# Malfoy/BGREAT

Measured on AMD Instinct MI355X. Metric: Mreads/s aligned (k=31, 150bp, m=2), higher is better.
Workload: dtype u64; 1 GPU; BASELINE configs[2]: synthetic 5170.0M x 150 bp reads per GPU (1034 steps x 5000000), k=31, m=2, effort=2, greedy, graph of 98935 unitigs (genome 4600000 bp, 2 alleles every ~140 bp); reads resident in HBM as ASCII before the timed region, results left in HBM; read_len=150, k=31, m=2, effort=2, distinct_batches=20, parallelism=reads sharded over 1 GPU(s); graph blob broadcast once

## Files before the change

bgreat_amd/__init__.py:

```python
import ctypes as C
import importlib.util
import os
import subprocess
import sys

import numpy as np

_HERE = os.path.dirname(os.path.abspath(__file__))
LIB_PATH = os.environ.get("BGR_LIB_PATH") or os.path.join(_HERE, "lib", "libbgreat_gpu.so")
CLI_PATH = os.path.join(_HERE, "bin", "bgreat")

MODE_GREEDY, MODE_EXHAUSTIVE, MODE_ANCHORS = 0, 1, 2
ST_NOANCHOR, ST_FAILED, ST_ALIGNED, ST_MASK, ST_RC = 0, 1, 2, 3, 4
BUILD_ANCHORS = 1
BUILD_NO_EVICTIONS = 2

SYMBOLS = [
    "bgr_last_error", "bgr_device_count", "bgr_graph_build", "bgr_graph_build_from_fasta", "bgr_graph_blob",
    "bgr_graph_from_blob", "bgr_graph_info", "bgr_graph_destroy", "bgr_graph_upload", "bgr_graph_device_blob",
    "bgr_graph_adopt_device_blob", "bgr_aligner_create", "bgr_aligner_destroy", "bgr_align_batch", "bgr_align_device", "bgr_aligner_path_stats",
    "bgr_aligner_sync", "bgr_aligner_device_results", "bgr_aligner_arena_ints", "bgr_aligner_fetch", "bgr_aligner_counters",
    "bgr_aligner_reset_counters", "bgr_aligner_kernel_time", "bgr_aligner_reset_kernel_time", "bgr_aligner_launch_info",
    "bgr_aligner_configure", "bgr_readset_load", "bgr_readset_count", "bgr_readset_view", "bgr_readset_destroy",
    "bgr_write_records", "bgr_graph_unitigs", "bgr_readset_load_parallel", "bgr_align_all", "bgr_host_alloc", "bgr_host_free",
    "bgr_set_build_threads", "bgr_graph_build_ex", "bgr_graph_build_from_fasta_ex", "bgr_graph_anchor_lookup", "bgr_graph_key_lookup", "bgr_graph_key_lookup_wide",
    "bgr_aligner_set_knob", "bgr_aligner_pass_counts", "bgr_aligner_last_pass_runs", "bgr_set_option", "bgr_get_option", "bgr_option_name", "bgr_plan_launch", "bgr_aligner_kernel_times", "bgr_devices_init", "bgr_devices_method", "bgr_packed_plane_words", "bgr_pack_reads", "bgr_align_batch_packed",
    "bgr_align_fasta_text", "bgr_aligner_fetch_text", "bgr_host_cache_release", "bgr_device_local_cpus", "bgr_text_stage_create", "bgr_text_stage_destroy", "bgr_text_stage_upload",
    "bgr_align_batch_begin", "bgr_align_batch_test", "bgr_align_batch_wait", "bgr_text_stage_device", "bgr_text_stage_upload_parts",
    "bgr_device_alloc", "bgr_device_free", "bgr_device_upload", "bgr_device_download",
    "bgr_aligner_abundance_enable", "bgr_aligner_abundance", "bgr_aligner_reset_abundance", "bgr_aligner_abundance_plan", "bgr_plan_abundance", "bgr_graph_abundance", "bgr_write_abundance",
    "bgr_aligner_links_enable", "bgr_aligner_links", "bgr_aligner_reset_links", "bgr_aligner_links_info", "bgr_aligner_links_plan", "bgr_plan_links", "bgr_graph_links_bound",
    "bgr_graph_links_enable", "bgr_graph_links", "bgr_write_gfa", "bgr_link_canonical", "bgr_graph_links_enabled",
    "bgr_links_bubbles", "bgr_aligner_bubbles", "bgr_aligner_bubbles_times", "bgr_graph_bubbles_enable", "bgr_graph_bubbles_enabled", "bgr_graph_bubbles", "bgr_write_bubbles",
    "bgr_aligner_triples_enable", "bgr_aligner_triples", "bgr_aligner_reset_triples", "bgr_aligner_triples_info", "bgr_triple_canonical", "bgr_graph_triples_bound",
    "bgr_graph_triples_enable", "bgr_graph_triples_enabled", "bgr_graph_triples", "bgr_write_triples",
    "bgr_bubbles_phase", "bgr_graph_phase_enable", "bgr_graph_phase_enabled", "bgr_graph_phase", "bgr_write_phase",
    "bgr_phase_blocks", "bgr_phase_blocks_times", "bgr_graph_blocks_enable", "bgr_graph_blocks_enabled", "bgr_graph_blocks", "bgr_write_blocks",
    "bgr_blocks_haplotypes", "bgr_blocks_haplotypes_times", "bgr_graph_haplotypes_enable", "bgr_graph_haplotypes_enabled", "bgr_graph_haplotypes", "bgr_write_haplotypes",
    "bgr_aligner_pileup_enable", "bgr_aligner_pileup", "bgr_aligner_reset_pileup", "bgr_graph_pileup_enable", "bgr_graph_pileup_enabled", "bgr_graph_pileup",
    "bgr_write_pileup", "bgr_write_depth",
    "bgr_aligner_pileup_sites", "bgr_aligner_pileup_sites_times", "bgr_aligner_pileup_add", "bgr_graph_variants_enable", "bgr_graph_variants_enabled", "bgr_graph_variants",
    "bgr_graph_variants_params", "bgr_write_vcf", "bgr_parse_af_ppm",
    "bgr_aligner_pileup_strands_enable", "bgr_aligner_pileup_forward", "bgr_aligner_pileup_strand_sites", "bgr_graph_pileup_strands_enable", "bgr_graph_pileup_strands_enabled",
    "bgr_graph_pileup_forward", "bgr_graph_variants_strands_enable", "bgr_graph_variant_strand_sites", "bgr_write_pileup_strands", "bgr_write_vcf_strands", "bgr_parse_min_alt_strand",
]
KNOB_EXH_FRAME_CAP, KNOB_EXH_SEARCH, KNOB_BATCH_SPLIT_LIMIT, KNOB_DEBUG_STOP, KNOB_GREEDY_FAST, KNOB_EXH_FAST, KNOB_ANCHORS_FAST, KNOB_BATCH_OVERLAP, KNOB_EXH_MEMO_CAP, KNOB_GREEDY_PREPASS, KNOB_KERNEL_EVENTS = 1, 2, 3, 4, 5, 6, 7, 8, 9, 10, 11
KNOB_ABUNDANCE_FORM = 12
ABUNDANCE_AUTO, ABUNDANCE_GLOBAL, ABUNDANCE_LDS = 0, 1, 2
KNOB_LINKS_FORM = 13
LINKS_AUTO, LINKS_GLOBAL, LINKS_LDS = 0, 1, 2
KNOB_DEVICE_OVERLAP = 14
SEARCH_AUTO, SEARCH_DEPTH_FIRST, SEARCH_BY_LEVEL = 0, 1, 2


class _Borrowed(np.ndarray):
    _owner = None


class PlanInput(C.Structure):
    _fields_ = [("k", C.c_uint32), ("slot_fill_x100", C.c_uint32), ("table_bytes", C.c_uint32), ("has_exceptions", C.c_uint32), ("anchors", C.c_uint32), ("anchor_levels", C.c_uint32),
                ("graph_bases", C.c_uint64), ("n_unitigs", C.c_uint64), ("max_unitig_len", C.c_uint64),
                ("num_cus", C.c_uint32), ("resident_waves", C.c_uint32 * 7), ("lds_per_cu", C.c_uint64),
                ("cfg_waves", C.c_uint32), ("cfg_blocks_per_cu", C.c_uint32), ("cfg_lds_mphf", C.c_uint32),
                ("mode", C.c_uint32), ("max_mismatch", C.c_uint32), ("partial", C.c_uint32), ("max_read_len", C.c_uint32),
                ("n_reads", C.c_uint64), ("total_bases", C.c_uint64), ("wide_keys", C.c_uint32), ("reserved0", C.c_uint32)]


class PlanPass(C.Structure):
    _fields_ = [("used", C.c_uint32), ("blocks", C.c_uint32), ("waves_per_block", C.c_uint32), ("lds_bytes", C.c_uint32), ("table_staged", C.c_uint32)]


class PlanOutput(C.Structure):
    _fields_ = [("pass_", PlanPass * 6), ("level_search", C.c_uint32), ("deep_only", C.c_uint32), ("x4_levels", C.c_uint32), ("memo_cap", C.c_uint32),
                ("deep_scratch_bytes", C.c_uint64), ("arena_ints", C.c_uint64)]


class BgrError(RuntimeError):
    pass


class Params(C.Structure):
    _fields_ = [("mode", C.c_uint32), ("max_mismatch", C.c_uint32), ("effort", C.c_uint32), ("partial", C.c_uint32)]


class RunOptions(C.Structure):
    _fields_ = [("struct_size", C.c_uint64), ("n_gpus", C.c_uint32), ("threads", C.c_uint32), ("batch_reads", C.c_uint64), ("chunk_bytes", C.c_uint64),
                ("fastq", C.c_uint32), ("write_exhaustive", C.c_uint32), ("echo_files", C.c_uint32), ("correction", C.c_uint32),
                ("no_overlap_file", C.c_char_p), ("first_device", C.c_uint32), ("route", C.c_uint32), ("numa", C.c_uint32), ("split_output", C.c_uint32), ("gaf", C.c_uint32),
                ("abundance", C.c_uint32)]


class UnitigAbundance(C.Structure):
    _fields_ = [("reads", C.c_uint64), ("bases", C.c_uint64), ("kmers", C.c_uint64)]


class Link(C.Structure):
    _fields_ = [("from_", C.c_int32), ("to", C.c_int32), ("count", C.c_uint64)]


LINK_DTYPE = np.dtype([("from", np.int32), ("to", np.int32), ("count", np.uint64)])


class Bubble(C.Structure):
    _fields_ = [("source", C.c_int32), ("sink", C.c_int32), ("branch", C.c_int32 * 2), ("count", C.c_uint64 * 4)]


BUBBLE_DTYPE = np.dtype([("source", np.int32), ("sink", np.int32), ("branch", np.int32, (2,)), ("count", np.uint64, (4,))])
BUBBLES_TILE = 1024


class Triple(C.Structure):
    _fields_ = [("from_", C.c_int32), ("via", C.c_int32), ("to", C.c_int32), ("reserved", C.c_int32), ("count", C.c_uint64)]


TRIPLE_DTYPE = np.dtype([("from", np.int32), ("via", np.int32), ("to", np.int32), ("reserved", np.int32), ("count", np.uint64)])


class Phase(C.Structure):
    _fields_ = [("via", C.c_int32), ("source", C.c_int32), ("in_", C.c_int32 * 2), ("out", C.c_int32 * 2), ("sink", C.c_int32), ("reserved", C.c_int32), ("count", C.c_uint64 * 4)]


PHASE_DTYPE = np.dtype([("via", np.int32), ("source", np.int32), ("in", np.int32, (2,)), ("out", np.int32, (2,)), ("sink", np.int32), ("reserved", np.int32),
                        ("count", np.uint64, (4,))])


class BlockEntry(C.Structure):
    _fields_ = [("block", C.c_uint32), ("index", C.c_uint32), ("size", C.c_uint32), ("bubble", C.c_uint32), ("flags", C.c_uint32), ("reserved", C.c_uint32)]


BLOCK_DTYPE = np.dtype([("block", np.uint32), ("index", np.uint32), ("size", np.uint32), ("bubble", np.uint32), ("flags", np.uint32), ("reserved", np.uint32)])
BLOCK_REVERSED, BLOCK_HAP, BLOCK_CIRCULAR, BLOCK_CONFLICT = 1, 2, 4, 8
BLOCKS_TILE = 1024


class Haplotype(C.Structure):
    _fields_ = [("block", C.c_uint32), ("hap", C.c_uint32), ("size", C.c_uint32), ("flags", C.c_uint32), ("offset", C.c_uint64), ("length", C.c_uint64)]


HAPLOTYPE_DTYPE = np.dtype([("block", np.uint32), ("hap", np.uint32), ("size", np.uint32), ("flags", np.uint32), ("offset", np.uint64), ("length", np.uint64)])


class PathStat(C.Structure):
    _fields_ = [("path_len", C.c_uint64), ("path_start", C.c_uint64), ("aligned", C.c_uint32), ("mismatches", C.c_uint32)]


PATH_STAT_NO_WALK = 0x80000000


class Ticket(C.Structure):
    _fields_ = [("aligner", C.c_void_p), ("n_reads", C.c_uint64), ("serial", C.c_uint64)]


class TextBatch(C.Structure):
    _fields_ = [("struct_size", C.c_uint64), ("text", C.c_void_p), ("text_bytes", C.c_uint64), ("want_output", C.c_uint32), ("irregular", C.c_uint32), ("paths_out", C.c_void_p),
                ("paths_cap", C.c_uint64), ("notaligned_out", C.c_void_p), ("notaligned_cap", C.c_uint64), ("n_records", C.c_uint64),
                ("n_accepted", C.c_uint64), ("paths_bytes", C.c_uint64), ("notaligned_bytes", C.c_uint64), ("stage", C.c_void_p),
                ("fastq", C.c_uint32), ("reserved", C.c_uint32), ("record_info_out", C.c_void_p), ("record_info_cap", C.c_uint64)]


class PackedReads(C.Structure):
    _fields_ = [("read_offsets", C.c_void_p), ("fw3", C.c_void_p), ("hasn", C.c_void_p), ("nm_index", C.c_void_p), ("nm_value", C.c_void_p),
                ("nm_count", C.c_uint64), ("max_read_len", C.c_uint32)]


class GraphInfo(C.Structure):
    _fields_ = [("k", C.c_uint32), ("n_levels", C.c_uint32), ("n_unitigs", C.c_uint64), ("n_keys", C.c_uint64),
                ("n_left_keys", C.c_uint64), ("n_right_keys", C.c_uint64), ("n_fallback", C.c_uint64),
                ("total_bases", C.c_uint64), ("blob_bytes", C.c_uint64), ("mphf_bytes", C.c_uint64),
                ("max_unitig_len", C.c_uint64), ("has_exceptions", C.c_uint32), ("has_anchors", C.c_uint32),
                ("gamma", C.c_double)]


_lib = None


def build(force=False):
    if force:
        subprocess.check_call(["make", "-C", _HERE, "clean"])
    subprocess.check_call(["make", "-s", "-C", _HERE, "all"])


def _pin_hip_runtime():
    if "torch" in sys.modules or os.environ.get("BGREAT_SYSTEM_HIP"):
        return
    try:
        spec = importlib.util.find_spec("torch")
    except (ImportError, ValueError):
        spec = None
    if spec and spec.submodule_search_locations:
        p = os.path.join(list(spec.submodule_search_locations)[0], "lib", "libamdhip64.so")
        if os.path.exists(p):
            C.CDLL(p, mode=C.RTLD_GLOBAL)


def lib():
    global _lib
    if _lib is not None:
        return _lib
    _pin_hip_runtime()
    if not os.path.exists(LIB_PATH):
        raise BgrError("libbgreat_gpu.so is not built (%s); run `make -C bgreat_amd` -- there is no fallback path" % LIB_PATH)
    L = C.CDLL(LIB_PATH)
    vp, u64, u32, i32 = C.c_void_p, C.c_uint64, C.c_uint32, C.c_int
    L.bgr_last_error.restype = C.c_char_p
    L.bgr_set_build_threads.restype = None
    L.bgr_set_build_threads.argtypes = [C.c_uint32]
    L.bgr_device_count.restype = i32
    L.bgr_graph_build.argtypes = [u32, u64, vp, vp, C.c_double, C.POINTER(vp)]
    L.bgr_graph_build_from_fasta.argtypes = [C.c_char_p, u32, C.c_double, C.POINTER(vp)]
    L.bgr_graph_build_ex.argtypes = [u32, u64, vp, vp, C.c_double, u32, C.POINTER(vp)]
    L.bgr_graph_build_from_fasta_ex.argtypes = [C.c_char_p, u32, C.c_double, u32, C.POINTER(vp)]
    L.bgr_graph_anchor_lookup.argtypes = [vp, u64, C.POINTER(u64), C.POINTER(u64)]
    L.bgr_graph_key_lookup.argtypes = [vp, u64, C.POINTER(C.c_uint32)]
    L.bgr_graph_key_lookup_wide.argtypes = [vp, u64, u64, C.POINTER(C.c_uint32)]
    L.bgr_graph_blob.restype = vp
    L.bgr_graph_blob.argtypes = [vp, C.POINTER(u64)]
    L.bgr_graph_from_blob.argtypes = [vp, u64, C.POINTER(vp)]
    L.bgr_graph_info.argtypes = [vp, C.POINTER(GraphInfo)]
    L.bgr_graph_unitigs.argtypes = [vp, C.POINTER(vp), C.POINTER(vp), C.POINTER(u64)]
    L.bgr_graph_destroy.argtypes = [vp]
    L.bgr_graph_destroy.restype = None
    L.bgr_graph_upload.argtypes = [vp, i32]
    L.bgr_graph_device_blob.restype = vp
    L.bgr_graph_device_blob.argtypes = [vp, i32]
    L.bgr_graph_adopt_device_blob.argtypes = [i32, vp, u64, C.POINTER(vp)]
    L.bgr_devices_init.argtypes = [vp, i32, u32, u32]
    L.bgr_devices_method.argtypes = [vp]
    L.bgr_devices_method.restype = u32
    L.bgr_aligner_create.argtypes = [vp, i32, C.POINTER(vp)]
    L.bgr_aligner_destroy.argtypes = [vp]
    L.bgr_aligner_destroy.restype = None
    L.bgr_align_batch.argtypes = [vp, C.POINTER(Params), vp, vp, u64, vp, u64, vp, vp]
    L.bgr_align_device.argtypes = [vp, C.POINTER(Params), vp, vp, u64, u64, u32]
    L.bgr_packed_plane_words.argtypes = [u64, u64]
    L.bgr_packed_plane_words.restype = u64
    L.bgr_pack_reads.argtypes = [vp, vp, u64, vp, vp, vp, vp, u64, C.POINTER(u64), C.POINTER(u32)]
    L.bgr_align_batch_packed.argtypes = [vp, C.POINTER(Params), C.POINTER(PackedReads), u64, vp, u64, vp, vp]
    L.bgr_align_fasta_text.argtypes = [vp, C.POINTER(Params), C.POINTER(TextBatch)]
    L.bgr_align_batch_begin.argtypes = [vp, C.POINTER(Params), vp, vp, u64, C.POINTER(Ticket)]
    L.bgr_align_batch_test.argtypes = [C.POINTER(Ticket)]
    L.bgr_align_batch_wait.argtypes = [C.POINTER(Ticket), vp, u64, vp, vp]
    L.bgr_aligner_fetch_text.argtypes = [vp, C.POINTER(TextBatch)]
    L.bgr_text_stage_create.argtypes = [C.c_int, C.POINTER(vp)]
    L.bgr_text_stage_destroy.argtypes = [vp]
    L.bgr_text_stage_destroy.restype = None
    L.bgr_text_stage_upload.argtypes = [vp, vp, u64]
    L.bgr_aligner_sync.argtypes = [vp]
    L.bgr_aligner_device_results.argtypes = [vp, C.POINTER(vp), C.POINTER(vp), C.POINTER(vp)]
    L.bgr_aligner_arena_ints.argtypes = [vp, vp]
    L.bgr_aligner_fetch.argtypes = [vp, u64, vp, u64, vp, vp]
    L.bgr_aligner_path_stats.argtypes = [vp, vp, vp, u64, vp]
    L.bgr_aligner_counters.argtypes = [vp, vp]
    L.bgr_aligner_reset_counters.argtypes = [vp]
# ... 220 lines not shown
    if isinstance(a, (bytes, bytearray)):
        a = np.frombuffer(a, dtype=np.uint8)
    return np.ascontiguousarray(a, dtype=np.uint8)


def pack_reads(reads, offsets):
    reads = _as_u8(reads)
    offsets = np.ascontiguousarray(offsets, dtype=np.uint64)
    n = len(offsets) - 1
    rel = offsets - offsets[0]
    total = int(rel[n])
    words = lib().bgr_packed_plane_words(n, total)
    fw3 = np.zeros(words, dtype=np.uint64)
    hasn = np.zeros((n + 31) // 32 + 1, dtype=np.uint32)
    cap = max(64, total // 16 + 64)
    nm_index = np.zeros(cap, dtype=np.uint32)
    nm_value = np.zeros(cap, dtype=np.uint64)
    cnt, mx = C.c_uint64(), C.c_uint32()
    _check(lib().bgr_pack_reads(reads.ctypes.data, offsets.ctypes.data, n, fw3.ctypes.data, hasn.ctypes.data, nm_index.ctypes.data,
                                nm_value.ctypes.data, cap, C.byref(cnt), C.byref(mx)))
    return {"read_offsets": rel, "fw3": fw3, "hasn": hasn, "nm_index": nm_index[: cnt.value].copy(), "nm_value": nm_value[: cnt.value].copy(),
            "max_read_len": mx.value, "n": n}


class Graph:

    def __init__(self, handle):
        self.h = handle

    @classmethod
    def build(cls, k, seqs, offsets, gamma=0.0, anchors=False, no_evictions=False):
        seqs = _as_u8(seqs)
        offsets = np.ascontiguousarray(offsets, dtype=np.uint64)
        h = C.c_void_p()
        _check(lib().bgr_graph_build_ex(k, len(offsets) - 1, seqs.ctypes.data, offsets.ctypes.data, gamma,
                                        (BUILD_ANCHORS if anchors else 0) | (BUILD_NO_EVICTIONS if no_evictions else 0), C.byref(h)))
        return cls(h)

    @classmethod
    def from_fasta(cls, path, k, gamma=0.0, anchors=False):
        h = C.c_void_p()
        _check(lib().bgr_graph_build_from_fasta_ex(path.encode(), k, gamma, BUILD_ANCHORS if anchors else 0, C.byref(h)))
        return cls(h)

    def key_lookup(self, key):
        key = int(key)
        if key < 0:
            raise ValueError("key_lookup: a (k-1)-mer is a non-negative integer")
        if key >> 128:
            return None
        slot = C.c_uint32()
        _check(lib().bgr_graph_key_lookup_wide(self.h, key >> 64, key & 0xFFFFFFFFFFFFFFFF, C.byref(slot)))
        return None if slot.value == 0xFFFFFFFF else int(slot.value)

    def anchor_lookup(self, kmer):
        idx, pos = C.c_uint64(), C.c_uint64()
        _check(lib().bgr_graph_anchor_lookup(self.h, int(kmer), C.byref(idx), C.byref(pos)))
        if idx.value == 0xFFFFFFFFFFFFFFFF:
            return None, 0, 0
        return idx.value, pos.value >> 32, pos.value & 0xFFFFFFFF

    @classmethod
    def from_blob(cls, blob):
        blob = _as_u8(blob)
        h = C.c_void_p()
        _check(lib().bgr_graph_from_blob(blob.ctypes.data, blob.size, C.byref(h)))
        return cls(h)

    @classmethod
    def adopt_device_blob(cls, device, dev_ptr, nbytes):
        h = C.c_void_p()
        _check(lib().bgr_graph_adopt_device_blob(device, dev_ptr, nbytes, C.byref(h)))
        return cls(h)

    def blob(self):
        n = C.c_uint64()
        p = lib().bgr_graph_blob(self.h, C.byref(n))
        if not p:
            return np.zeros(0, dtype=np.uint8)
        v = np.ctypeslib.as_array(C.cast(p, C.POINTER(C.c_uint8)), shape=(n.value,)).view(_Borrowed)
        v._owner = self
        return v

    def info(self):
        gi = GraphInfo()
        _check(lib().bgr_graph_info(self.h, C.byref(gi)))
        return {f[0]: getattr(gi, f[0]) for f in GraphInfo._fields_ if f[0] != "reserved"}

    def upload(self, device=0):
        _check(lib().bgr_graph_upload(self.h, device))

    def devices_init(self, first_device=0, n_devices=1, how=0):
        _check(lib().bgr_devices_init(self.h, first_device, n_devices, how))
        return lib().bgr_devices_method(self.h)

    def device_blob(self, device=0):
        return lib().bgr_graph_device_blob(self.h, device)

    def abundance(self):
        n = self.info()["n_unitigs"]
        out = np.zeros((n, 3), dtype=np.uint64)
        _check(lib().bgr_graph_abundance(self.h, out.ctypes.data, n))
        return out

    def links_enable(self, on=True):
        _check(lib().bgr_graph_links_enable(self.h, int(bool(on))))

    def links_enabled(self):
        return bool(lib().bgr_graph_links_enabled(self.h))

    def bubbles_enable(self, on=True, min_link=1):
        _check(lib().bgr_graph_bubbles_enable(self.h, int(bool(on)), int(min_link)))

    def bubbles_enabled(self):
        return bool(lib().bgr_graph_bubbles_enabled(self.h))

    def bubbles(self):
        return _fetch_bubbles(lambda out, cap, n: lib().bgr_graph_bubbles(self.h, out, cap, n))

    def links(self):
        return _fetch_links(lib().bgr_graph_links, self.h)

    def pileup_enable(self, on=True):
        _check(lib().bgr_graph_pileup_enable(self.h, int(bool(on))))

    def pileup_enabled(self):
        return bool(lib().bgr_graph_pileup_enabled(self.h))

    def pileup(self):
        return _fetch_pileup(lib().bgr_graph_pileup, self)

    def write_pileup(self, path):
        _check(lib().bgr_write_pileup(path.encode(), self.h))

    def write_depth(self, path):
        _check(lib().bgr_write_depth(path.encode(), self.h))

    def variants_enable(self, min_depth=2, min_alt=2, min_af_ppm=200000, on=True):
        prm = VariantParams(int(min_depth), int(min_alt), int(min_af_ppm))
        _check(lib().bgr_graph_variants_enable(self.h, C.byref(prm) if on else None))

    def variants_enabled(self):
        return bool(lib().bgr_graph_variants_enabled(self.h))

    def variants(self):
        return _fetch_sites(lambda out, cap, n: lib().bgr_graph_variants(self.h, out, cap, n))

    def variants_params(self):
        prm = VariantParams()
        _check(lib().bgr_graph_variants_params(self.h, C.byref(prm)))
        return int(prm.min_depth), int(prm.min_alt), int(prm.min_af_ppm)

    def write_vcf(self, path, sites=None, params=None):
        if sites is None:
            sites = self.variants()
        prm = VariantParams(*(self.variants_params() if params is None else params))
        sites = np.ascontiguousarray(sites, dtype=VARIANT_DTYPE)
        _check(lib().bgr_write_vcf(path.encode(), self.h, C.byref(prm), sites.ctypes.data if len(sites) else None, len(sites)))

    def pileup_strands_enable(self, on=True):
        _check(lib().bgr_graph_pileup_strands_enable(self.h, int(bool(on))))

    def pileup_strands_enabled(self):
        return bool(lib().bgr_graph_pileup_strands_enabled(self.h))

    def pileup_forward(self):
        return _fetch_forward(lib().bgr_graph_pileup_forward, self)

    def write_pileup_strands(self, path):
        _check(lib().bgr_write_pileup_strands(path.encode(), self.h))
# ... 628 lines not shown
```

bgreat_amd/csrc/capi.hip:

```cpp
#include <hip/hip_runtime.h>
#include <sys/mman.h>
#include <dlfcn.h>

#include <algorithm>
#include <chrono>
#include <condition_variable>
#include <cstdio>
#include <cstdlib>
#include <cstring>
#include <map>
#include <mutex>
#include <string>
#include <thread>
#include <vector>

#include "../../include/bgreat_gpu.h"
#include "abundance_kernels.h"
#include "align_kernels.h"
#include "fanout.h"
#include "fastx.h"
#include "anchor_index.h"
#include "graph_build.h"
#include "launch_plan.h"
#include "launch_taker.h"
#include "links_kernels.h"
#include "triples_kernels.h"
#include "pileup_kernels.h"
#include "read_pack.h"
#include "text_kernels.h"
#include "options.h"
#include "capi_internal.h"

namespace bgr {
static thread_local std::string tl_err;
int set_error(int code, const std::string& msg) { tl_err = msg; return code; }
}

namespace {

int drain_timers(bgr_aligner* a) {
    if (a->ev_used == 0) return BGR_OK;
    HIP_TRY(hipStreamSynchronize(a->stream));
    for (int i = 0; i < a->ev_used; ++i) {
        float ms = 0;
        HIP_TRY(hipEventElapsedTime(&ms, a->ev[i][0], a->ev[i][a->ev_marks[i]]));
        a->t_ms += ms;
        for (int j = 0; j < a->ev_marks[i]; ++j) {
            HIP_TRY(hipEventElapsedTime(&ms, a->ev[i][j], a->ev[i][j + 1]));
            a->t_slot_ms[j] += ms;
        }
        ++a->t_launches;
    }
    a->ev_used = 0;
    return BGR_OK;
}

void forget_launch(bgr_aligner* a) { a->last_n = 0; a->holder = nullptr; }

}

extern "C" {

const char* bgr_last_error(void) { return bgr::tl_err.c_str(); }

int bgr_set_option(const char* name, int64_t value) {
    bgr::Option* o = name ? bgr::find_option(name) : nullptr;
    if (!o) return fail(BGR_E_ARG, std::string("bgr_set_option: unknown option '") + (name ? name : "") + "'");
    if (value < o->lo || value > o->hi) return fail(BGR_E_ARG, std::string("bgr_set_option: value out of range for '") + name + "'");
    o->value.store(value, std::memory_order_relaxed);
    return BGR_OK;
}
int bgr_get_option(const char* name, int64_t* value) {
    bgr::Option* o = name ? bgr::find_option(name) : nullptr;
    if (!o || !value) return fail(BGR_E_ARG, std::string("bgr_get_option: unknown option '") + (name ? name : "") + "'");
    *value = o->value.load(std::memory_order_relaxed);
    return BGR_OK;
}
const char* bgr_option_name(uint32_t index, const char** what) {
    size_t n;
    bgr::Option* t = bgr::option_table(&n);
    if (index >= n) return nullptr;
    if (what) *what = t[index].what;
    return t[index].name;
}
void bgr_set_build_threads(uint32_t threads) { bgr::set_build_threads(threads); }

int bgr_device_count(void) {
    int n = 0;
    if (hipGetDeviceCount(&n) != hipSuccess) return 0;
    return n;
}

int bgr_graph_build(uint32_t k, uint64_t n_unitigs, const char* seqs, const uint64_t* offsets, double gamma, bgr_graph** out) {
    return bgr_graph_build_ex(k, n_unitigs, seqs, offsets, gamma, 0, out);
}

int bgr_graph_build_ex(uint32_t k, uint64_t n_unitigs, const char* seqs, const uint64_t* offsets, double gamma, uint32_t flags, bgr_graph** out) {
    if (!out || (n_unitigs && (!seqs || !offsets))) return fail(BGR_E_ARG, "bgr_graph_build: null argument");
    if (flags & ~(uint32_t)(BGR_BUILD_ANCHORS | BGR_BUILD_NO_EVICTIONS)) return fail(BGR_E_ARG, "bgr_graph_build: unknown flag");
    bgr_graph* g = new bgr_graph();
    std::string err;
    uint64_t zero[1] = {0};
    if (!bgr::build_graph(k, n_unitigs, seqs, n_unitigs ? offsets : zero, gamma > 0 ? gamma : 0.0, flags, g->host, err)) {
        delete g;
        return fail(BGR_E_ARG, err);
    }
    g->header = *g->host.header();
    const uint64_t nu = g->header.n_unitigs;
    g->ascii.assign(seqs + (nu ? offsets[0] : 0), seqs + (nu ? offsets[nu] : 0));
    g->ascii_offs.resize(nu + 1);
    for (uint64_t i = 0; i <= nu; ++i) g->ascii_offs[i] = nu ? offsets[i] - offsets[0] : 0;
    *out = g;
    return BGR_OK;
}

int bgr_graph_unitigs(const bgr_graph* g, const char** seqs, const uint64_t** offsets, uint64_t* n) {
    if (!g || !seqs || !offsets || !n) return fail(BGR_E_ARG, "bgr_graph_unitigs: null argument");
    if (g->ascii_offs.empty()) return fail(BGR_E_ARG, "bgr_graph_unitigs: this graph was created from a blob and carries no unitig characters");
    *seqs = g->ascii.data();
    *offsets = g->ascii_offs.data();
    *n = g->ascii_offs.size() - 1;
    return BGR_OK;
}

int bgr_graph_build_from_fasta(const char* path, uint32_t k, double gamma, bgr_graph** out) {
    return bgr_graph_build_from_fasta_ex(path, k, gamma, 0, out);
}

int bgr_graph_build_from_fasta_ex(const char* path, uint32_t k, double gamma, uint32_t flags, bgr_graph** out) {
    if (!path || !out) return fail(BGR_E_ARG, "bgr_graph_build_from_fasta: null argument");
    std::vector<char> seqs;
    std::vector<uint64_t> offs;
    std::string err;
    if (!bgr::read_unitig_fasta(path, k, seqs, offs, err)) return fail(BGR_E_IO, err);
    return bgr_graph_build_ex(k, offs.size() - 1, seqs.data(), offs.data(), gamma, flags, out);
}

int bgr_graph_anchor_lookup(const bgr_graph* g, uint64_t kmer, uint64_t* index_out, uint64_t* position_out) {
    if (!g || !index_out) return fail(BGR_E_ARG, "bgr_graph_anchor_lookup: null argument");
    if (g->host.blob.empty()) return fail(BGR_E_ARG, "bgr_graph_anchor_lookup: graph has no host blob");
    if (!g->header.anc_n) return fail(BGR_E_ARG, "bgr_graph_anchor_lookup: the graph was built without BGR_BUILD_ANCHORS");
    const uint64_t idx = bgr::anchor_lookup(g->host.header(), g->host.base(), kmer);
    *index_out = idx;
    if (position_out) *position_out = idx == ~0ULL ? 0 : reinterpret_cast<const uint64_t*>(g->host.base() + g->header.off_anc_pos)[idx];
    return BGR_OK;
}

int bgr_graph_key_lookup(const bgr_graph* g, uint64_t key, uint32_t* slot_out) {
    if (!g || !slot_out) return fail(BGR_E_ARG, "bgr_graph_key_lookup: null argument");
    if (g->host.blob.empty()) return fail(BGR_E_ARG, "bgr_graph_key_lookup: graph has no host blob");
    if (g->header.wide_keys) return fail(BGR_E_ARG, "bgr_graph_key_lookup: the graph has two-word keys (k > 32): use bgr_graph_key_lookup_wide");
    *slot_out = bgr::host_lookup(g->host.header(), g->host.base(), key);
    return BGR_OK;
}

int bgr_graph_key_lookup_wide(const bgr_graph* g, uint64_t key_hi, uint64_t key_lo, uint32_t* slot_out) {
    if (!g || !slot_out) return fail(BGR_E_ARG, "bgr_graph_key_lookup_wide: null argument");
    if (g->host.blob.empty()) return fail(BGR_E_ARG, "bgr_graph_key_lookup_wide: graph has no host blob");
    *slot_out = bgr::host_lookup_wide(g->host.header(), g->host.base(), key_hi, key_lo);
    return BGR_OK;
}

const void* bgr_graph_blob(const bgr_graph* g, uint64_t* bytes) {
    if (!g || g->host.blob.empty()) { if (bytes) *bytes = 0; return nullptr; }
    if (bytes) *bytes = g->header.blob_bytes;
    return g->host.blob.data();
}

int bgr_graph_from_blob(const void* blob, uint64_t bytes, bgr_graph** out) {
    if (!blob || !out) return fail(BGR_E_ARG, "bgr_graph_from_blob: null argument");
    std::string err;
    if (!bgr::validate_blob(blob, bytes, err)) return fail(BGR_E_ARG, err);
    bgr_graph* g = new bgr_graph();
    if (!g->host.blob.reset((bytes + 7) / 8)) { delete g; return fail(BGR_E_ARG, "bgr_graph_from_blob: out of memory"); }
    memcpy(g->host.blob.data(), blob, bytes);
    g->header = *g->host.header();
    *out = g;
    return BGR_OK;
}

int bgr_graph_info(const bgr_graph* g, bgr_graph_info_t* o) {
    if (!g || !o) return fail(BGR_E_ARG, "bgr_graph_info: null argument");
    const BgrBlobHeader& h = g->header;
    memset(o, 0, sizeof(*o));
    o->k = h.k; o->n_levels = 2; o->n_unitigs = h.n_unitigs; o->n_keys = h.n_placed + h.n_fallback;
    o->n_left_keys = h.n_left_keys; o->n_right_keys = h.n_right_keys; o->n_fallback = h.n_fallback;
    o->total_bases = h.total_bases; o->blob_bytes = h.blob_bytes; o->mphf_bytes = h.n_buckets * 4;
    o->max_unitig_len = h.max_unitig_len; o->has_exceptions = h.has_exc; o->has_anchors = h.anc_n ? 1 : 0; o->gamma = h.gamma;
    return BGR_OK;
}

void bgr_graph_destroy(bgr_graph* g) {
    if (!g) return;
    for (auto& kv : g->dev) {
        if (kv.second.owned && kv.second.ptr) {
            if (hipSetDevice(kv.first) == hipSuccess) (void)hipFree(kv.second.ptr);
        }
    }
    variants_run_free(g);
    delete g;
}

int bgr_graph_upload(bgr_graph* g, int device) {
    if (!g) return fail(BGR_E_ARG, "bgr_graph_upload: null graph");
    if (g->dev.count(device)) return BGR_OK;
    if (g->host.blob.empty()) return fail(BGR_E_ARG, "bgr_graph_upload: graph has no host blob (adopted graphs live on one device)");
    HIP_TRY(hipSetDevice(device));
    void* p = nullptr;
    HIP_TRY(hipMalloc(&p, g->header.blob_bytes));
    hipError_t e = hipMemcpy(p, g->host.blob.data(), g->header.blob_bytes, hipMemcpyHostToDevice);
    if (e == hipSuccess) e = hipStreamSynchronize(nullptr);
    if (e != hipSuccess) { (void)hipFree(p); return fail(BGR_E_HIP, std::string("blob H2D: ") + hipGetErrorString(e)); }
    g->dev[device] = {p, true};
    return BGR_OK;
}

namespace {

struct Rccl {
    typedef int (*CommInitAll_t)(void** comms, int n, const int* devs);
    typedef int (*Group_t)(void);
    typedef int (*Broadcast_t)(const void* send, void* recv, size_t count, int dtype, int root, void* comm, hipStream_t stream);
    typedef int (*CommDestroy_t)(void* comm);
    void* lib = nullptr;
    CommInitAll_t CommInitAll = nullptr;
    Group_t GroupStart = nullptr, GroupEnd = nullptr;
    Broadcast_t Broadcast = nullptr;
    CommDestroy_t CommDestroy = nullptr;
    bool load() {
        for (const char* name : {"librccl.so.1", "librccl.so"}) {
            lib = dlopen(name, RTLD_NOW | RTLD_LOCAL);
            if (lib) break;
        }
        if (!lib) return false;
        CommInitAll = reinterpret_cast<CommInitAll_t>(dlsym(lib, "ncclCommInitAll"));
        GroupStart = reinterpret_cast<Group_t>(dlsym(lib, "ncclGroupStart"));
        GroupEnd = reinterpret_cast<Group_t>(dlsym(lib, "ncclGroupEnd"));
        Broadcast = reinterpret_cast<Broadcast_t>(dlsym(lib, "ncclBroadcast"));
        CommDestroy = reinterpret_cast<CommDestroy_t>(dlsym(lib, "ncclCommDestroy"));
        return CommInitAll && GroupStart && GroupEnd && Broadcast && CommDestroy;
    }
};

bool fanout_rccl(const std::vector<int>& devs, const std::vector<void*>& ptr, uint64_t bytes, std::string& why) {
    Rccl r;
    if (!r.load()) { why = "librccl not loadable"; return false; }
    const int n = (int)devs.size();
    std::vector<void*> comms(n, nullptr);
    if (r.CommInitAll(comms.data(), n, devs.data()) != 0) { why = "ncclCommInitAll failed"; return false; }
    std::vector<hipStream_t> streams(n, nullptr);
    bool ok = true;
    for (int i = 0; i < n && ok; ++i) ok = hipSetDevice(devs[i]) == hipSuccess && hipStreamCreateWithFlags(&streams[i], hipStreamNonBlocking) == hipSuccess;
    if (ok) {
        ok = r.GroupStart() == 0;
        for (int i = 0; i < n && ok; ++i) {
            ok = hipSetDevice(devs[i]) == hipSuccess &&
                 r.Broadcast(ptr[i], ptr[i], (size_t)bytes,  0,  0, comms[i], streams[i]) == 0;
        }
        ok = r.GroupEnd() == 0 && ok;
    }
    for (int i = 0; i < n; ++i) {
        if (streams[i]) { if (hipSetDevice(devs[i]) == hipSuccess) { ok = hipStreamSynchronize(streams[i]) == hipSuccess && ok; (void)hipStreamDestroy(streams[i]); } }
    }
    for (void* c : comms) if (c) (void)r.CommDestroy(c);
    if (!ok) why = "RCCL broadcast failed";
    return ok;
}

bool peer_round(const std::vector<bgr::FanoutCopy>& round, uint64_t bytes, std::string& why) {
    std::vector<hipStream_t> streams;
    std::vector<int> sdev;
    bool ok = true;
    for (const bgr::FanoutCopy& c : round) {
        if (hipSetDevice(c.src_dev) != hipSuccess) { ok = false; why = "hipSetDevice failed"; break; }
        int can = 0;
        if (hipDeviceCanAccessPeer(&can, c.src_dev, c.dst_dev) == hipSuccess && can) {
            hipError_t pe = hipDeviceEnablePeerAccess(c.dst_dev, 0);
            if (pe != hipSuccess && pe != hipErrorPeerAccessAlreadyEnabled) (void)hipGetLastError();
        }
        hipStream_t st = nullptr;
        if (hipStreamCreateWithFlags(&st, hipStreamNonBlocking) != hipSuccess) { ok = false; why = "hipStreamCreate failed"; break; }
        streams.push_back(st);
        sdev.push_back(c.src_dev);
        hipError_t e = hipMemcpyPeerAsync(c.dst, c.dst_dev, c.src, c.src_dev, bytes, st);
        if (e != hipSuccess) { ok = false; why = std::string("hipMemcpyPeerAsync: ") + hipGetErrorString(e); break; }
    }
    for (size_t j = 0; j < streams.size(); ++j) {
        if (hipSetDevice(sdev[j]) == hipSuccess) {
            hipError_t e = hipStreamSynchronize(streams[j]);
            if (e != hipSuccess && ok) { ok = false; why = std::string("peer copy: ") + hipGetErrorString(e); }
            (void)hipStreamDestroy(streams[j]);
        }
    }
    return ok;
}

}

int bgr_devices_init(bgr_graph* g, int first_device, uint32_t n_devices, uint32_t how) {
    if (!g) return fail(BGR_E_ARG, "bgr_devices_init: null graph");
    if (n_devices == 0) n_devices = 1;
    if (how > BGR_FANOUT_PEER) return fail(BGR_E_ARG, "bgr_devices_init: unknown distribution method");
    int nd = 0;
    if (hipGetDeviceCount(&nd) != hipSuccess || nd == 0) return fail(BGR_E_HIP, "no HIP device available");
    if (first_device < 0 || (uint64_t)first_device + n_devices > (uint64_t)nd) return fail(BGR_E_ARG, "bgr_devices_init: device range outside the visible devices");
    int rc = bgr_graph_upload(g, first_device);
    if (rc != BGR_OK) return rc;
    const uint64_t bytes = g->header.blob_bytes;
    bgr::FanoutOps ops;
    ops.alloc = [bytes](int dev, void** out) { return hipSetDevice(dev) == hipSuccess && hipMalloc(out, bytes) == hipSuccess; };
    ops.release = [](int dev, void* p) { if (p && hipSetDevice(dev) == hipSuccess) (void)hipFree(p); };
    ops.broadcast = [bytes](const std::vector<int>& devs, const std::vector<void*>& ptr, std::string& why) { return fanout_rccl(devs, ptr, bytes, why); };
    ops.peer_round = [bytes](const std::vector<bgr::FanoutCopy>& round, std::string& why) { return peer_round(round, bytes, why); };
    std::map<int, void*> resident;
    for (auto& kv : g->dev) resident[kv.first] = kv.second.ptr;
    g->fanout_method = 0;
    const bgr::FanoutResult r = bgr::fanout_blob(first_device, n_devices, how, resident, ops);
    if (!r.error.empty()) return fail(r.hip_error ? BGR_E_HIP : BGR_E_ARG, "bgr_devices_init: " + r.error);
    for (auto& kv : resident) if (!g->dev.count(kv.first)) g->dev[kv.first] = {kv.second, true};
    g->fanout_method = (uint32_t)r.method;
    return BGR_OK;
}

uint32_t bgr_devices_method(const bgr_graph* g) { return g ? g->fanout_method : 0; }

const void* bgr_graph_device_blob(const bgr_graph* g, int device) {
    if (!g) return nullptr;
    auto it = g->dev.find(device);
    return it == g->dev.end() ? nullptr : it->second.ptr;
}

int bgr_graph_adopt_device_blob(int device, const void* dev_blob, uint64_t bytes, bgr_graph** out) {
    if (!dev_blob || !out || bytes < sizeof(BgrBlobHeader)) return fail(BGR_E_ARG, "bgr_graph_adopt_device_blob: bad argument");
    HIP_TRY(hipSetDevice(device));
    bgr_graph* g = new bgr_graph();
    hipError_t e = hipMemcpy(&g->header, dev_blob, sizeof(BgrBlobHeader), hipMemcpyDeviceToHost);
    if (e != hipSuccess) { delete g; return fail(BGR_E_HIP, std::string("header D2H: ") + hipGetErrorString(e)); }
    std::string verr;
    if (!bgr::validate_blob_header(&g->header, bytes, verr)) {
        delete g;
        return fail(BGR_E_ARG, "bgr_graph_adopt_device_blob: " + verr);
    }
    g->dev[device] = {const_cast<void*>(dev_blob), false};
    *out = g;
    return BGR_OK;
}

int bgr_aligner_create(bgr_graph* g, int device, bgr_aligner** out) {
    if (!g || !out) return fail(BGR_E_ARG, "bgr_aligner_create: null argument");
    int nd = 0;
    hipError_t e0 = hipGetDeviceCount(&nd);
    if (e0 != hipSuccess || nd == 0) return fail(BGR_E_HIP, "no HIP device available (this library has no CPU mapping path)");
    if (device < 0 || device >= nd) return fail(BGR_E_ARG, "bgr_aligner_create: device index out of range");
    int rc = bgr_graph_upload(g, device);
    if (rc != BGR_OK) return rc;
    HIP_TRY(hipSetDevice(device));
    bgr_aligner* a = new bgr_aligner();
    a->graph = g;
    a->device = device;
    hipDeviceProp_t prop;
    hipError_t e = hipGetDeviceProperties(&prop, device);
    if (e != hipSuccess) { delete a; return fail(BGR_E_HIP, hipGetErrorString(e)); }
    a->num_cus = prop.multiProcessorCount;
    a->lds_per_cu = prop.maxSharedMemoryPerMultiProcessor ? prop.maxSharedMemoryPerMultiProcessor : 65536;
    e = hipStreamCreateWithFlags(&a->stream, hipStreamNonBlocking);
    if (e != hipSuccess) { delete a; return fail(BGR_E_HIP, hipGetErrorString(e)); }
    for (int i = 0; i < kTimerRing; ++i) {
        for (int j = 0; j <= kTimerSlots; ++j) {
            if (hipEventCreate(&a->ev[i][j]) != hipSuccess) {
                delete a;
                return fail(BGR_E_HIP, "hipEventCreate failed");
            }
        }
    }
    if (a->blocking_sync && hipEventCreateWithFlags(&a->ev_wait, hipEventBlockingSync | hipEventDisableTiming) != hipSuccess) a->blocking_sync = false;
    bgr::resolve_device_graph(&g->header, g->dev[device].ptr, a->dg);
    e = a->small.ensure(bgr::kSmallBytes);
    if (e == hipSuccess) e = hipMemset(a->small.p, 0, a->small.cap);
    if (e == hipSuccess) e = hipStreamSynchronize(nullptr);
    if (e != hipSuccess) { delete a; return fail(BGR_E_HIP, hipGetErrorString(e)); }
    *out = a;
    return BGR_OK;
}

void bgr_aligner_destroy(bgr_aligner* a) {
    if (!a) return;
    if (a->tx_phase_s[4] > 0 && bgr::opt("timing"))
        fprintf(stderr, "bgreat: text calls %.0f on device %d: to record count %.3f s, records %.3f s, mapping + sizes %.3f s, streams out %.3f s\n", a->tx_phase_s[4], a->device,
                a->tx_phase_s[0], a->tx_phase_s[1], a->tx_phase_s[2], a->tx_phase_s[3]);
    if (a->twin) { bgr_aligner_destroy(a->twin); a->twin = nullptr; }
    if (hipSetDevice(a->device) == hipSuccess) {
        if (a->stream) (void)hipStreamSynchronize(a->stream);
        a->in_reads.release(); a->in_offs.release(); a->pk_fw3.release(); a->pk_nm.release(); a->pk_hasn.release(); a->results.release(); a->arena.release(); a->ovf.release(); a->ovf2.release(); a->lst.release(); a->deepbuf.release(); a->retry.release(); a->retry2.release(); a->small.release();
        a->csr_sums.release(); a->csr_poffs.release(); a->csr_status.release(); a->csr_paths.release(); a->wave_times.release(); a->abundance.release(); a->links.release(); a->triples.release(); a->pileup.release(); a->pileup_offs.release(); a->pileup_fwd.release(); a->var_scratch.release(); a->var_out.release(); a->var_stage.release();
        for (DevBuf* b : {&a->tx_in, &a->tx_sums, &a->tx_state, &a->tx_rec, &a->tx_idx, &a->tx_accrec, &a->tx_accsrc, &a->tx_offs,
                          &a->tx_psz, &a->tx_nsz, &a->tx_poff, &a->tx_noff, &a->tx_pout, &a->tx_nout, &a->tx_info, &a->tx_gaf, &a->path_stats}) b->release();
        for (int i = 0; i < kTimerRing; ++i) for (int j = 0; j <= kTimerSlots; ++j) (void)hipEventDestroy(a->ev[i][j]);
        if (a->ev_wait) (void)hipEventDestroy(a->ev_wait);
        if (a->stream) (void)hipStreamDestroy(a->stream);
    }
    delete a;
}

int bgr_aligner_configure(bgr_aligner* a, uint32_t waves_per_block, uint32_t blocks_per_cu, uint32_t lds_mphf) {
    if (!a || waves_per_block > 16 || lds_mphf > 2) return fail(BGR_E_ARG, "bgr_aligner_configure: bad argument");
    a->cfg_waves = waves_per_block;
    a->cfg_blocks_per_cu = blocks_per_cu;
    a->cfg_lds_mphf = lds_mphf;
    return BGR_OK;
}

int bgr_aligner_set_knob(bgr_aligner* a, uint32_t knob, uint64_t value) {
    if (!a) return fail(BGR_E_ARG, "bgr_aligner_set_knob: null aligner");
    switch (knob) {
        case BGR_KNOB_EXH_FRAME_CAP: a->knob_frame_cap = (uint32_t)std::min<uint64_t>(value, 1u << 20); return BGR_OK;
        case BGR_KNOB_EXH_SEARCH: if (value > 2) break; a->knob_search = (uint32_t)value; return BGR_OK;
        case BGR_KNOB_BATCH_SPLIT_LIMIT: a->knob_split_limit = value; return BGR_OK;
        case BGR_KNOB_DEBUG_STOP: a->knob_debug_stop = (uint32_t)value; return BGR_OK;
        case BGR_KNOB_BATCH_OVERLAP: a->knob_overlap = (uint32_t)value; return BGR_OK;
        case BGR_KNOB_DEVICE_OVERLAP: a->knob_device_overlap = (uint32_t)value; return BGR_OK;
        case BGR_KNOB_GREEDY_FAST: if (value > 1) break; a->knob_greedy_fast = (uint32_t)value; return BGR_OK;
        case BGR_KNOB_EXH_FAST: if (value > 1) break; a->knob_exh_fast = (uint32_t)value; return BGR_OK;
        case BGR_KNOB_ANCHORS_FAST: if (value > 1) break; a->knob_anc_fast = (uint32_t)value; return BGR_OK;
        case BGR_KNOB_GREEDY_PREPASS: if (value > 1) break; a->knob_prepass = (uint32_t)value; return BGR_OK;
        case BGR_KNOB_KERNEL_EVENTS: if (value > 1) break; a->knob_no_events = value ? 0u : 1u; return BGR_OK;
        case BGR_KNOB_ABUNDANCE_FORM: if (value > 2) break; a->knob_abundance_form = (uint32_t)value; for (bgr_aligner* tw = a->twin; tw; tw = tw->twin) tw->knob_abundance_form = (uint32_t)value; return BGR_OK;
        case BGR_KNOB_LINKS_FORM: if (value > 2) break; a->knob_links_form = (uint32_t)value; for (bgr_aligner* tw = a->twin; tw; tw = tw->twin) tw->knob_links_form = (uint32_t)value; return BGR_OK;
        case BGR_KNOB_EXH_MEMO_CAP: a->knob_memo_cap = (uint32_t)std::min<uint64_t>(value, 1u << 24); return BGR_OK;
        default: break;
    }
    return fail(BGR_E_ARG, "bgr_aligner_set_knob: unknown knob or value out of range");
}

static bgr::PlanGraph plan_graph_of(const BgrBlobHeader& h) {
    bgr::PlanGraph g;
    g.k = h.k; g.slot_fill_x100 = h.slot_fill_x100; g.table_bytes = (uint32_t)std::min<uint64_t>((uint64_t)h.n_buckets * 4, 0xFFFFFFFFull);
    g.total_bases = h.total_bases; g.n_unitigs = h.n_unitigs; g.n_buckets = h.n_buckets; g.max_unitig_len = h.max_unitig_len;
    g.anc_n = h.anc_n; g.anc_active_levels = h.anc_active_levels; g.has_exc = h.has_exc != 0; g.wide_keys = h.wide_keys != 0;
    return g;
}
static bgr::PlanTuning plan_tuning_of(const bgr_aligner* a) {
    bgr::PlanTuning t;
    t.cfg_waves = a->cfg_waves; t.cfg_blocks_per_cu = a->cfg_blocks_per_cu; t.cfg_lds_mphf = a->cfg_lds_mphf;
    t.frame_cap = a->knob_frame_cap; t.search = a->knob_search; t.memo_cap = a->knob_memo_cap;
    t.no_greedy_fast = a->knob_greedy_fast != 0; t.no_exh_fast = a->knob_exh_fast != 0; t.no_anc_fast = a->knob_anc_fast != 0;
    return t;
}

extern "C" int bgr_plan_launch(const bgr_plan_input* in, bgr_plan_output* out) {
    if (!in || !out) return fail(BGR_E_ARG, "bgr_plan_launch: null argument");
    bgr::PlanGraph g;
    g.k = in->k; g.slot_fill_x100 = in->slot_fill_x100; g.table_bytes = in->table_bytes; g.total_bases = in->graph_bases; g.n_unitigs = in->n_unitigs;
    g.n_buckets = in->table_bytes / 4; g.max_unitig_len = in->max_unitig_len; g.anc_n = in->anchors ? 1 : 0; g.anc_active_levels = in->anchor_levels; g.has_exc = in->has_exceptions != 0;
    g.wide_keys = in->wide_keys != 0;
    bgr::PlanDevice d;
    if (in->num_cus) d.num_cus = in->num_cus;
    if (in->lds_per_cu) d.lds_per_cu = in->lds_per_cu;
    for (uint32_t i = 0; i < bgr::kResidentKernels; ++i) if (in->resident_waves[i]) d.resident[i] = in->resident_waves[i];
    bgr::PlanTuning t;
    t.cfg_waves = in->cfg_waves; t.cfg_blocks_per_cu = in->cfg_blocks_per_cu; t.cfg_lds_mphf = in->cfg_lds_mphf;
    bgr::PlanBatch b;
    b.mode = in->mode; b.max_mismatch = in->max_mismatch; b.partial = in->partial; b.max_read_len = in->max_read_len; b.n_reads = in->n_reads; b.total_bases = in->total_bases;
    const bgr::LaunchPlan P = bgr::plan_launch(g, d, t, b);
    memset(out, 0, sizeof(*out));
    if (P.error) return fail(BGR_E_ARG, P.error);
    auto put = [out](int slot, const bgr::LaunchCfg& c) {
        out->pass[slot] = bgr_plan_pass{1, c.blocks, c.waves_per_block, c.lds_bytes, c.stage_mphf};
    };
    const uint32_t general = bgr::many_reads_per_wave(P.pass[0].kernel) ? 1 : 0;
    for (uint32_t i = 0; i < P.n_passes; ++i) {
        const bgr::Pass& ps = P.pass[i];
        if (i == general) put(0, ps.cfg);
        switch (ps.kernel) {
            case bgr::KernelId::kGreedyMulti: put(1, ps.cfg); break;
            case bgr::KernelId::kExhaustive4: put(2, ps.cfg); break;
            case bgr::KernelId::kAnchors4: put(3, ps.cfg); break;
            case bgr::KernelId::kExhaustive: if (i != general) put(4, ps.cfg); break;
            case bgr::KernelId::kExhaustiveLast: put(5, ps.cfg); break;
            default: break;
        }
    }
    out->level_search = P.level_search; out->deep_only = P.pass[0].kernel == bgr::KernelId::kExhaustiveLast; out->x4_levels = P.x4_levels; out->memo_cap = P.memo_cap;
    out->deep_scratch_bytes = P.deep_scratch_bytes;
    out->arena_ints = P.arena_cap;
    return BGR_OK;
}

static DevBuf* list_buf(bgr_aligner* a, bgr::List l) {
    switch (l) {
        case bgr::List::kSearch: return &a->ovf;
        case bgr::List::kDepthFirst: case bgr::List::kGeneral: return &a->ovf2;
        case bgr::List::kFirst: return &a->lst;
        case bgr::List::kRetry: return &a->retry;
        default: return nullptr;
    }
}

struct LaunchMarks {
    bgr_aligner* a;
    bool timed;
    int marks = 0;
    hipError_t operator()(const char* name) {
        if (!timed || marks >= kTimerSlots) return hipSuccess;
        a->t_slot_name[marks] = name;
        return hipEventRecord(a->ev[a->ev_used][++marks], a->stream);
    }
};
// ... 75 lines not shown
    HIP_TRY(a->arena.ensure(P.arena_cap * 4));
    a->last_arena_cap = P.arena_cap; a->last_total_bases = total_bases;
    for (uint32_t i = 0; i < P.n_passes; ++i) {
        const bgr::Pass& ps = P.pass[i];
        if (ps.appends != bgr::List::kNone) HIP_TRY(list_buf(a, ps.appends)->ensure(n_reads * 4));
        if (ps.kernel == bgr::KernelId::kGreedyMulti) HIP_TRY(a->ovf.ensure((uint64_t)ps.cfg.blocks * ps.cfg.waves_per_block * P.q_cap * 8));
    }
    a->last_launch[0] = first.cfg.blocks; a->last_launch[1] = first.cfg.waves_per_block * 64; a->last_launch[2] = first.cfg.lds_bytes;
    a->last_launch[3] = first.cfg.stage_mphf | (P.level_search && first.kernel != bgr::KernelId::kExhaustiveLast ? 2u : 0u) | (bgr::many_reads_per_wave(first.kernel) ? 4u : 0u);

    const bool inline_pack = (first.kernel == bgr::KernelId::kGreedyMulti || first.kernel == bgr::KernelId::kExhaustive4) && !planes_ready && d_reads && !a->knob_prepass;
    if (!reads_bytes) reads_bytes = total_bases;
    if (!inline_pack) {
        HIP_TRY(a->pk_fw3.ensure(P.plane_words * 8));
        HIP_TRY(a->pk_nm.ensure(P.plane_words * 8));
        HIP_TRY(a->pk_hasn.ensure((n_reads + 31) / 32 * 4 + 4));
    }
    bgr::BatchIO io{};
    io.ascii = inline_pack ? static_cast<const uint8_t*>(d_reads) : nullptr;
    io.ascii_src = inline_pack ? static_cast<const uint32_t*>(d_src_off) : nullptr;
    io.ascii_bytes = reads_bytes;
    io.fw3 = static_cast<const uint64_t*>(a->pk_fw3.p);
    io.nmw = static_cast<const uint64_t*>(a->pk_nm.p);
    io.hasn = static_cast<const uint32_t*>(a->pk_hasn.p);
    io.read_offs = static_cast<const uint64_t*>(d_read_offsets);
    io.results = static_cast<uint2*>(a->results.p);
    io.arena = static_cast<int32_t*>(a->arena.p);
    io.cursor = static_cast<uint32_t*>(a->small.p);
    io.n_reads = (uint32_t)n_reads;
    io.path_cap = P.path_cap;
    io.arena_cap = (uint32_t)P.arena_cap;
    io.arena_chunk = P.arena_chunk;
    io.arena_own = (uint32_t)P.arena_own;
    io.deep_stride = (uint32_t)P.deep_stride;
    io.deep_memo_cap = P.memo_cap;
    io.search_iters = P.search_iters;
    io.wide_scan = P.wide_scan ? 1u : 0u;
    io.task_ctr = bgr::kCurTasks;
    bgr::KernelParams kp = {p->max_mismatch, p->effort, p->partial, p->mode, a->knob_debug_stop};
    BgrDeviceGraph dgl = a->dg;
    if (p->mode == BGR_MODE_EXHAUSTIVE && !(dgl.filter_kind == BGR_FILTER_MINIMIZER && a->exh_filter)) dgl.bloom = nullptr;

    if (!cursor_is_zero) HIP_TRY(hipMemsetAsync(a->small.p, 0, bgr::kCurWords * 4, a->stream));
    const bool timed = !a->knob_no_events;
    LaunchMarks mark{a, timed};
    if (timed) HIP_TRY(hipEventRecord(a->ev[a->ev_used][0], a->stream));
    hipError_t e = hipSuccess;
    if (!planes_ready && !inline_pack) {
        HIP_TRY(hipMemsetAsync(a->pk_hasn.p, 0, (n_reads + 31) / 32 * 4, a->stream));
        e = d_src_off ? bgr::launch_pack_reads_at(static_cast<const uint8_t*>(d_reads), static_cast<const uint32_t*>(d_src_off), io.read_offs, io.n_reads, reads_bytes, total_bases,
                                                  static_cast<uint64_t*>(a->pk_fw3.p), static_cast<uint64_t*>(a->pk_nm.p), static_cast<uint32_t*>(a->pk_hasn.p), a->stream)
                      : bgr::launch_pack_reads(static_cast<const uint8_t*>(d_reads), io.read_offs, io.n_reads, total_bases, static_cast<uint64_t*>(a->pk_fw3.p),
                                               static_cast<uint64_t*>(a->pk_nm.p), static_cast<uint32_t*>(a->pk_hasn.p), a->stream);
        if (e != hipSuccess) return fail(BGR_E_HIP, std::string("pre-pass launch: ") + hipGetErrorString(e));
        HIP_TRY(mark("bgr_pack_reads_kernel"));
    }
    for (uint32_t i = 0; i < P.n_passes; ++i) {
        const bgr::Pass& ps = P.pass[i];
        bgr::BatchIO pio = io;
        pio.words_per_read = ps.words;
        pio.frames_per_wave = ps.frames;
        pio.subset = ps.maps == bgr::List::kNone ? nullptr : static_cast<const uint32_t*>(list_buf(a, ps.maps)->p);
        pio.subset_ctr = bgr::list_word(ps.maps);
        uint32_t* appends = ps.appends == bgr::List::kNone ? nullptr : static_cast<uint32_t*>(list_buf(a, ps.appends)->p);
        if (ps.kernel == bgr::KernelId::kGreedyMulti) {
            pio.queue = static_cast<uint2*>(a->ovf.p);
            pio.q_cap = P.q_cap;
            pio.gen_list = appends;
            pio.gen_ctr = bgr::list_word(ps.appends);
        } else {
            pio.ovf_list = appends;
            pio.ovf_ctr = bgr::list_word(ps.appends);
        }
        if (ps.kernel == bgr::KernelId::kExhaustiveLast) pio.deep_scratch = static_cast<uint32_t*>(a->deepbuf.p);
#ifdef BGR_PHASE_TIMING
        if (ps.kernel == bgr::KernelId::kGreedyMulti || ps.kernel == bgr::KernelId::kExhaustive4) {
            const uint64_t waves = (uint64_t)ps.cfg.blocks * ps.cfg.waves_per_block, bytes = waves * (ps.kernel == bgr::KernelId::kGreedyMulti ? 64 : 32);
            HIP_TRY(a->wave_times.ensure(bytes));
            if (ps.kernel == bgr::KernelId::kGreedyMulti) HIP_TRY(hipMemsetAsync(a->wave_times.p, 0, bytes, a->stream));
            pio.wave_times = static_cast<unsigned long long*>(a->wave_times.p);
            a->wave_times_n = waves;
        }
#endif
        e = bgr::launch_align(ps.kernel, ps.variant, dgl, pio, kp, ps.cfg, a->stream);
        if (e != hipSuccess) return fail(BGR_E_HIP, std::string("kernel launch (") + ps.name + "): " + hipGetErrorString(e));
        HIP_TRY(mark(ps.name));
        if (ps.kernel == bgr::KernelId::kExhaustiveLast) {
            a->deep.open = true;
            a->deep.pass = ps; a->deep.io = pio; a->deep.kp = kp; a->deep.dg = dgl;
            a->deep.per_wave_lds = bgr::deep_lds_bytes_per_wave(max_read_len);
            a->deep.path_cap = P.path_cap; a->deep.memo_cap = P.memo_cap;
            a->deep.runs = 1;
        }
    }
    {
        bgr::PileupReads pr;
        if (inline_pack) { pr.ascii = static_cast<const uint8_t*>(d_reads); pr.src_off = static_cast<const uint32_t*>(d_src_off); pr.ascii_bytes = reads_bytes; }
        else { pr.fw3 = io.fw3; pr.nmw = io.nmw; pr.hasn = io.hasn; }
        const int crc = queue_counting(a, P.arena_cap, io.read_offs, n_reads, total_bases, pr, mark);
        if (crc != BGR_OK) return crc;
    }
    if (timed) {
        a->ev_marks[a->ev_used] = mark.marks;
        ++a->ev_used;
    }
    return BGR_OK;
}

static int settle_launch(bgr_aligner* a, uint32_t* cur) {
    if (cur[bgr::kCurOverflow]) return fail(BGR_E_INTERNAL, "path arena overflow (internal sizing error)");
    if (!a->deep.open) return BGR_OK;
    const uint32_t kRetry = bgr::list_word(bgr::List::kRetry);
    while (cur[kRetry]) {
        const uint32_t n_retry = cur[kRetry];
        auto& D = a->deep;
        if (D.runs >= bgr::kDeepRuns || D.memo_cap >= (1u << 28))
            return fail(BGR_E_NOMEM, "exhaustive search: a read's table of remembered calls outgrew 2^28 entries per wave (8 GiB)");
        D.memo_cap *= 16;
        const uint64_t stride = bgr::deep_scratch_words(D.path_cap, D.pass.frames, D.memo_cap);
        if (stride > 0xFFFFFFFFull) return fail(BGR_E_NOMEM, "exhaustive search: a read's table of remembered calls outgrew the 16 GiB a wave can address");
        size_t free_b = 0, total_b = 0;
        HIP_TRY(hipMemGetInfo(&free_b, &total_b));
        const uint64_t room = (uint64_t)free_b + a->deepbuf.cap;
        uint64_t waves = std::min<uint64_t>(n_retry, (uint64_t)D.pass.cfg.blocks * D.pass.cfg.waves_per_block);
        waves = std::min<uint64_t>(waves, std::max<uint64_t>(1, room / 2 / (stride * 4)));
        if (stride * 4 > room - room / 8) return fail(BGR_E_NOMEM, "exhaustive search: not enough device memory for a read's table of remembered calls");
        HIP_TRY(a->deepbuf.ensure(waves * stride * 4));
        DevBuf& other = a->retry2;
        HIP_TRY(other.ensure((uint64_t)n_retry * 4));
        bgr::BatchIO io = D.io;
        io.subset = io.ovf_list;
        io.subset_ctr = bgr::kCurRetrySubset;
        io.ovf_list = static_cast<uint32_t*>(other.p);
        io.ovf_ctr = kRetry;
        io.deep_scratch = static_cast<uint32_t*>(a->deepbuf.p);
        io.deep_stride = (uint32_t)stride;
        io.deep_memo_cap = D.memo_cap;
        uint32_t ctr[2] = {0, n_retry};
        HIP_TRY(hipMemcpyAsync(static_cast<uint32_t*>(a->small.p) + kRetry, ctr, 8, hipMemcpyHostToDevice, a->stream));
        bgr::LaunchCfg cfg = D.pass.cfg;
        cfg.waves_per_block = (uint32_t)std::min<uint64_t>(cfg.waves_per_block, waves);
        cfg.blocks = (uint32_t)std::max<uint64_t>(1, waves / cfg.waves_per_block);
        cfg.lds_bytes = bgr::kLdsFixed + cfg.waves_per_block * D.per_wave_lds;
        hipError_t e = bgr::launch_align(D.pass.kernel, D.pass.variant, D.dg, io, D.kp, cfg, a->stream);
        if (e != hipSuccess) return fail(BGR_E_HIP, std::string("kernel launch (last pass, run again): ") + hipGetErrorString(e));
        HIP_TRY(hipMemcpyAsync(cur, a->small.p, bgr::kCurWords * 4, hipMemcpyDeviceToHost, a->stream));
        HIP_TRY(wait_stream(a));
        if (cur[bgr::kCurOverflow]) return fail(BGR_E_INTERNAL, "path arena overflow (internal sizing error)");
        std::swap(a->retry, a->retry2);
        D.io.ovf_list = io.ovf_list;
        ++D.runs;
    }
    a->deep.open = false;
    return BGR_OK;
}
static int settle_launch_sync(bgr_aligner* a) {
    if (!a->deep.open) return BGR_OK;
    uint32_t cur[bgr::kCurWords];
    HIP_TRY(hipMemcpyAsync(cur, a->small.p, sizeof(cur), hipMemcpyDeviceToHost, a->stream));
    HIP_TRY(wait_stream(a));
    return settle_launch(a, cur);
}

static int twins_setup(bgr_aligner* a, unsigned n_twins) {
    bgr_aligner* prev = a;
    for (unsigned t = 0; t < n_twins; ++t) {
        if (!prev->twin) {
            int rc = bgr_aligner_create(a->graph, a->device, &prev->twin);
            if (rc != BGR_OK) return rc;
            prev->twin->is_twin = true;
        }
        bgr_aligner* tw = prev->twin;
        tw->cfg_waves = a->cfg_waves; tw->cfg_blocks_per_cu = a->cfg_blocks_per_cu; tw->cfg_lds_mphf = a->cfg_lds_mphf;
        tw->knob_frame_cap = a->knob_frame_cap; tw->knob_search = a->knob_search; tw->knob_debug_stop = a->knob_debug_stop;
        tw->knob_greedy_fast = a->knob_greedy_fast; tw->knob_exh_fast = a->knob_exh_fast; tw->knob_anc_fast = a->knob_anc_fast; tw->knob_memo_cap = a->knob_memo_cap; tw->knob_prepass = a->knob_prepass; tw->knob_no_events = a->knob_no_events;
        tw->knob_abundance_form = a->knob_abundance_form;
        tw->knob_links_form = a->knob_links_form;
        if (tw->abundance_on != a->abundance_on) { const int rc = abundance_set(tw, a->abundance_on); if (rc != BGR_OK) return rc; }
        prev = tw;
    }
    pileup_share(a);
    links_share(a);
    triples_share(a);
    return BGR_OK;
}

static int stream_idle(bgr_aligner* a, bool* idle) {
    const hipError_t e = hipStreamQuery(a->stream);
    if (e != hipSuccess && e != hipErrorNotReady) return fail(BGR_E_HIP, std::string("hipStreamQuery: ") + hipGetErrorString(e));
    *idle = e == hipSuccess;
    return BGR_OK;
}

int bgr_align_device(bgr_aligner* a, const bgr_params* p, const void* d_reads, const void* d_read_offsets, uint64_t n_reads,
                     uint64_t total_bases, uint32_t max_read_len) {
    if (!a || !p) return fail(BGR_E_ARG, "bgr_align_device: null argument");
    bgr_aligner* taker = a;
    if (!a->is_twin && !a->knob_device_overlap && p->mode != BGR_MODE_EXHAUSTIVE && n_reads) {
        HIP_TRY(hipSetDevice(a->device));
        bool primary_idle = true, twin_idle = true;
        int rc = stream_idle(a, &primary_idle);
        if (rc == BGR_OK && !primary_idle && a->twin) rc = stream_idle(a->twin, &twin_idle);
        if (rc != BGR_OK) return rc;
        if (bgr::launch_taker(primary_idle, twin_idle, a->holder != nullptr) == bgr::Taker::kTwin) {
            rc = twins_setup(a, 1);
            if (rc != BGR_OK) return rc;
            taker = a->twin;
        }
    }
    const int rc = align_device_impl(taker, p, d_reads, d_read_offsets, n_reads, total_bases, max_read_len, false);
    if (rc == BGR_OK) a->holder = taker == a ? nullptr : taker;
    return rc;
}

uint64_t bgr_packed_plane_words(uint64_t n_reads, uint64_t total_bases) { return bgr::packed_plane_words(n_reads, total_bases); }

int bgr_pack_reads(const char* reads, const uint64_t* read_offsets, uint64_t n, uint64_t* fw3, uint32_t* hasn, uint32_t* nm_index, uint64_t* nm_value,
                   uint64_t nm_cap, uint64_t* nm_count, uint32_t* max_read_len) {
    if (!read_offsets || !fw3 || !hasn || !nm_count || (n && !reads)) return fail(BGR_E_ARG, "bgr_pack_reads: null argument");
    const uint64_t base = read_offsets[0];
    memset(hasn, 0, ((n + 31) / 32) * 4);
    uint64_t cnt = 0;
    uint32_t longest = 0;
    std::vector<uint64_t> nm;
    for (uint64_t r = 0; r < n; ++r) {
        const uint64_t off = read_offsets[r] - base, len64 = read_offsets[r + 1] - read_offsets[r];
        if (len64 > 0x7FFFFFFFull) return fail(BGR_E_ARG, "bgr_pack_reads: read longer than 2^31 bases");
        const uint32_t len = (uint32_t)len64, words = (len + 31) >> 5;
        longest = std::max(longest, len);
        if (nm.size() < words) nm.resize(words);
        const uint64_t w0 = bgr::packed_word_offset(off, r);
        if (bgr::pack_read(reads + read_offsets[r], len, fw3 + w0, nm.data())) {
            hasn[r >> 5] |= 1u << (r & 31);
            if (cnt + words > nm_cap || !nm_index || !nm_value) return fail(BGR_E_CAPACITY, "bgr_pack_reads: N-mask list too small");
            for (uint32_t j = 0; j < words; ++j) { nm_index[cnt] = (uint32_t)(w0 + j); nm_value[cnt] = nm[j]; ++cnt; }
        }
    }
    *nm_count = cnt;
    if (max_read_len) *max_read_len = longest;
    return BGR_OK;
}

int bgr_align_batch_packed(bgr_aligner* a, const bgr_params* p, const bgr_packed_reads* pk, uint64_t n, int32_t* paths_out, uint64_t paths_cap,
                           uint64_t* path_offsets, uint8_t* status) {
    if (!a || !p || !pk || !path_offsets || (n && (!pk->read_offsets || !pk->fw3 || !pk->hasn || !status))) return fail(BGR_E_ARG, "bgr_align_batch_packed: null argument");
    if (pk->nm_count && (!pk->nm_index || !pk->nm_value)) return fail(BGR_E_ARG, "bgr_align_batch_packed: null N-mask list");
    path_offsets[0] = 0;
    forget_launch(a);
    if (n == 0) return BGR_OK;
    if (pk->read_offsets[0] != 0) return fail(BGR_E_ARG, "bgr_align_batch_packed: read_offsets must start at 0 (they address the planes)");
    const uint64_t total = pk->read_offsets[n];
    if (n >= 0x7FFFFFFFull || 2 * (total + 16 * n) >= 0xFFFFFFFFull - (256ull << 20))
        return fail(BGR_E_ARG, "bgr_align_batch_packed: batch too large for one launch (2*(bases + 16*reads) must stay below 2^32 - 2^28); pack it in pieces");
    HIP_TRY(hipSetDevice(a->device));
    const uint64_t plane_words = bgr::packed_plane_words(n, total);
    HIP_TRY(a->in_offs.ensure((n + 1) * 8));
    HIP_TRY(a->pk_fw3.ensure(plane_words * 8));
    HIP_TRY(a->pk_nm.ensure(plane_words * 8));
// ... 851 lines not shown
```

bgreat_amd/csrc/capi_internal.h:

```cpp
#ifndef BGREAT_AMD_CAPI_INTERNAL_H
#define BGREAT_AMD_CAPI_INTERNAL_H

#include <hip/hip_runtime.h>

#include <map>
#include <mutex>
#include <string>
#include <utility>
#include <vector>

#include "../../include/bgreat_gpu.h"
#include "abundance_kernels.h"
#include "align_kernels.h"
#include "graph_build.h"
#include "launch_plan.h"
#include "options.h"

namespace bgr {
int set_error(int code, const std::string& msg);
}

#pragma GCC visibility push(hidden)

inline int fail(int code, const std::string& msg) { return bgr::set_error(code, msg); }
// ... 51 lines not shown
    std::vector<uint32_t> pileup_fwd_words;
    std::vector<bgr_variant_strand_site> variants_strand_sites;
};

struct DevBuf {
    void* p = nullptr;
    size_t cap = 0;
    hipError_t ensure(size_t bytes) {
        if (bytes <= cap) return hipSuccess;
        if (p) { hipError_t e = hipFree(p); if (e != hipSuccess) return e; p = nullptr; cap = 0; }
        size_t want = bytes + bytes / 8 + 256;
        hipError_t e = hipMalloc(&p, want);
        if (e == hipSuccess) cap = want;
        const bool poison = bgr::opt("poison_device_buffers") != 0;
        if (e == hipSuccess && poison) { e = hipMemset(p, 0xA5, want); if (e == hipSuccess) e = hipDeviceSynchronize(); }
        return e;
    }
    void release() { if (p) (void)hipFree(p); p = nullptr; cap = 0; }
};

struct VariantsRun {
    int device = 0, num_cus = 0;
    hipStream_t stream = nullptr;
    BgrDeviceGraph dg;
    DevBuf table, offs, stage, table_fwd;
};

struct bgr_text_stage {
    int device = 0;
    hipStream_t stream = nullptr;
    hipEvent_t ev = nullptr, ev0 = nullptr;
    DevBuf buf;
    uint64_t bytes = 0;
    bool timing = false, pending = false;
    double copy_ms = 0, copy_bytes = 0;
    void settle() {
        if (!timing || !pending) return;
        float ms = 0;
        if (hipEventElapsedTime(&ms, ev0, ev) == hipSuccess) { copy_ms += ms; copy_bytes += (double)bytes; }
        pending = false;
    }
};

struct bgr_aligner {
    bgr_graph* graph = nullptr;
    int device = 0;
    hipStream_t stream = nullptr;
    BgrDeviceGraph dg;
    DevBuf tx_in, tx_sums, tx_state, tx_rec, tx_idx, tx_accrec, tx_accsrc, tx_offs, tx_psz, tx_nsz, tx_poff, tx_noff, tx_pout, tx_nout, tx_info, tx_gaf, path_stats;
    uint64_t tx_n_acc = 0, tx_pbytes = 0, tx_nbytes = 0;
    bool blocking_sync = bgr::opt("blocking_sync") != 0;
    hipEvent_t ev_wait = nullptr;
    const uint8_t* tx_text = nullptr;
    uint32_t tx_flip = 0;
    uint32_t tx_epoch = 0, tx_ticket[2] = {0, 0};
    bool tx_written = false;
    uint32_t tx_want = 0;
    double tx_phase_s[5] = {0, 0, 0, 0, 0};

    DevBuf in_reads, in_offs, pk_fw3, pk_nm, pk_hasn, results, arena, ovf, ovf2, lst, deepbuf, retry, retry2, small, csr_sums, csr_poffs, csr_status, csr_paths;
    struct DeepRun {
        bool open = false;
        bgr::Pass pass;
        bgr::BatchIO io;
        bgr::KernelParams kp;
        BgrDeviceGraph dg;
        uint32_t per_wave_lds = 0, path_cap = 0, memo_cap = 0, runs = 0;
    } deep;
    bgr::PlanDevice plan_dev;
    bool plan_dev_known = false;
    uint64_t last_n = 0;
    uint32_t last_mode = 0;
    uint64_t last_arena_cap = 0, last_total_bases = 0;
    DevBuf wave_times;
    uint64_t wave_times_n = 0;
    uint64_t ticket_serial = 0;
    bool ticket_open = false;
    std::vector<uint64_t> ticket_offs;
    uint32_t last_launch[4] = {0, 0, 0, 0};
    uint32_t cfg_waves = 0, cfg_blocks_per_cu = 0, cfg_lds_mphf = 0;
    bool exh_filter = bgr::opt("exh_filter") != 0;
    uint32_t knob_frame_cap = 0, knob_search = 0, knob_debug_stop = 0, knob_greedy_fast = 0, knob_exh_fast = 0, knob_anc_fast = 0, knob_memo_cap = 0, knob_prepass = 0, knob_no_events = 0;
    uint64_t knob_split_limit = 0;
    uint32_t knob_overlap = 0;
    uint32_t knob_abundance_form = 0;
    bool abundance_on = false;
    DevBuf abundance;
    uint32_t knob_links_form = 0;
    bool links_on = false;
    DevBuf links;
    unsigned long long* links_tab = nullptr;
    uint64_t links_cap = 0, links_bound = 0;
    bool triples_on = false;
    DevBuf triples;
    unsigned long long* triples_tab = nullptr;
    uint64_t triples_cap = 0, triples_bound = 0;
    bool pileup_on = false;
    DevBuf pileup, pileup_offs;
    uint32_t* pileup_tab = nullptr;
    const uint64_t* pileup_base_offs = nullptr;
    bool strands_on = false;
    DevBuf pileup_fwd;
    uint32_t* pileup_fwd_tab = nullptr;
    DevBuf var_scratch, var_out, var_stage;
    double var_ms[5] = {0, 0, 0, 0, 0};
    double bub_ms[4] = {0, 0, 0, 0};
    bgr_aligner* twin = nullptr;
    bool is_twin = false;
    uint32_t knob_device_overlap = 0;
    bgr_aligner* holder = nullptr;
    int num_cus = 0;
    size_t lds_per_cu = 0;
    hipEvent_t ev[kTimerRing][kTimerSlots + 1];
    int ev_marks[kTimerRing];
    int ev_used = 0;
    uint64_t t_launches = 0;
    double t_ms = 0, t_slot_ms[kTimerSlots] = {0, 0, 0, 0, 0, 0, 0, 0};
    const char* t_slot_name[kTimerSlots] = {nullptr, nullptr, nullptr, nullptr, nullptr, nullptr, nullptr, nullptr};
};

inline hipError_t wait_stream(bgr_aligner* a) {
    if (!a->blocking_sync) return hipStreamSynchronize(a->stream);
    hipError_t e = hipEventRecord(a->ev_wait, a->stream);
    return e == hipSuccess ? hipEventSynchronize(a->ev_wait) : e;
}
inline int sync_all(bgr_aligner* a) {
    HIP_TRY(hipSetDevice(a->device));
    for (bgr_aligner* x = a; x; x = x->twin) HIP_TRY(hipStreamSynchronize(x->stream));
    return BGR_OK;
}

inline bgr_aligner* holder_of(bgr_aligner* a) { return a->holder ? a->holder : a; }
inline const bgr_aligner* holder_of(const bgr_aligner* a) { return a->holder ? a->holder : a; }

int abundance_set(bgr_aligner* a, bool on);
bgr::AbundancePlan abundance_plan_of(const bgr_aligner* a, uint64_t n_reads, uint64_t total_bases);
void links_share(bgr_aligner* a);
int links_tail(bgr_aligner* a, const char* who, uint64_t* tail);
void run_links_begin(bgr_graph* g);
int run_links_collect(bgr_graph* g, bgr_aligner* a);
void run_links_end(bgr_graph* g, bool ok);
void triples_share(bgr_aligner* a);
void run_triples_begin(bgr_graph* g);
int run_triples_collect(bgr_graph* g, bgr_aligner* a);
void run_triples_end(bgr_graph* g, bool ok);
void run_phase_begin(bgr_graph* g);
int run_phase_end(bgr_graph* g, bool ok);
void run_blocks_begin(bgr_graph* g);
int run_blocks_end(bgr_graph* g, bool ok);
void run_haplotypes_begin(bgr_graph* g);
int run_haplotypes_end(bgr_graph* g, bool ok);
void run_bubbles_begin(bgr_graph* g);
void run_bubbles_collect(bgr_graph* g, bgr_aligner* a);
int run_bubbles_end(bgr_graph* g, bool ok);
void pileup_share(bgr_aligner* a);
int pileup_guard(const bgr_unitig_abundance* rows, uint64_t n, const char* who);
int guarded_sync(bgr_aligner* a, const char* who);
int graph_base_offs(bgr_graph* g, const char* who);
int pileup_refusal(const bgr_graph* g, const char* who);
void run_pileup_begin(bgr_graph* g);
int run_pileup_collect(bgr_graph* g, bgr_aligner* a);
int run_pileup_end(bgr_graph* g, bool ok);
int variants_collect(bgr_graph* g, bgr_aligner* a);
int variants_end(bgr_graph* g, bool ok);
void variants_run_free(bgr_graph* g);

// ... 4 lines not shown
```

bgreat_amd/csrc/graph_build.cpp:

```cpp
#include "graph_build.h"
#include "anchor_index.h"
#include "host_parallel.h"
#include "file_image.h"

#include <fcntl.h>
#include <sys/mman.h>
#include <sys/stat.h>
#include <unistd.h>

#include <algorithm>
#include <atomic>
#include <chrono>
#include <cmath>
#include <cstdio>
#include <cstdlib>
#include <cstring>
#include <thread>
#include "options.h"

namespace bgr {

namespace {

inline uint32_t code_of(char c) { return c == 'A' ? 0u : c == 'C' ? 1u : c == 'G' ? 2u : 3u; }

std::atomic<unsigned> g_build_threads{0};

inline void pack_strand(uint64_t* seq, uint64_t pos, const char* s, uint32_t len, bool rc) {
    uint32_t j = 0;
    while (j < len) {
        uint64_t w = (pos + j) >> 5;
        uint32_t o = (uint32_t)((pos + j) & 31), n = std::min<uint32_t>(32 - o, len - j);
        uint64_t x = 0;
        for (uint32_t i = 0; i < n; ++i) {
            uint32_t c = rc ? 3u - code_of(s[len - 1 - (j + i)]) : code_of(s[j + i]);
            x |= (uint64_t)c << (62 - 2 * (o + i));
        }
        if (n == 32) seq[w] = x;
        else __atomic_fetch_or(&seq[w], x, __ATOMIC_RELAXED);
        j += n;
    }
}
inline uint64_t window(const uint64_t* seq, uint64_t pos, uint32_t n) {
    uint64_t w = pos >> 5;
    uint32_t s = (uint32_t)(pos & 31) * 2;
    uint64_t x = s ? (seq[w] << s) | (seq[w + 1] >> (64 - s)) : seq[w];
    return x >> (64 - 2 * n);
}
inline uint64_t align256(uint64_t x) { return (x + 255) & ~(uint64_t)255; }

typedef unsigned __int128 u128;
inline uint64_t key_mix(uint64_t x) { return bgr_mix64(x); }
inline uint64_t key_mix(u128 x) { return bgr_mix_wide((uint64_t)(x >> 64), (uint64_t)x); }
inline uint64_t key_rcb(uint64_t x, uint32_t n) { return bgr_rcb(x, n); }
inline u128 key_rcb(u128 x, uint32_t n) {
    const u128 r = ((u128)~bgr_rev2((uint64_t)x) << 64) | (u128)~bgr_rev2((uint64_t)(x >> 64));
    return r >> (128 - 2 * n);
}

template <typename Key>
struct KeyTable {
    std::vector<uint32_t> buckets;
    std::vector<uint32_t> who;
    std::vector<Key> fallback;
    uint64_t n_placed = 0;
};

template <typename Key>
void build_key_table(const std::vector<Key>& keys, double slots_per_key, unsigned T, bool evictions, KeyTable<Key>& t) {
    const uint64_t n = keys.size();
    const uint32_t nb = (uint32_t)std::max<uint64_t>(1, (uint64_t)std::ceil(slots_per_key * (double)n / 4.0));
    t.buckets.assign(nb, 0);
    std::vector<uint64_t> mix(n);
    parallel_ranges(T, n, [&](uint64_t b, uint64_t e, unsigned) {
        for (uint64_t i = b; i < e; ++i) mix[i] = key_mix(keys[i]);
    });
    std::vector<uint32_t>& who = t.who;
    who.assign((size_t)nb * 4, BGR_NONE);
    uint8_t* fp = reinterpret_cast<uint8_t*>(t.buckets.data());
    auto try_place = [&](uint32_t bucket, uint32_t i) {
        for (uint32_t s = 0; s < 4; ++s) {
            const size_t slot = (size_t)bucket * 4 + s;
            if (!fp[slot]) { fp[slot] = (uint8_t)bgr_tab_fp(mix[i]); who[slot] = i; return true; }
        }
        return false;
    };
    const int kMaxKicks = evictions ? 4000 : 0;
    uint64_t rng = 0x9E3779B97F4A7C15ULL;
    for (uint64_t i0 = 0; i0 < n; ++i0) {
        uint32_t cur = (uint32_t)i0;
        uint32_t from = BGR_NONE;
        bool done = false;
        for (int kick = 0; kick <= kMaxKicks; ++kick) {
            const uint32_t b1 = bgr_tab_bucket((uint32_t)mix[cur], nb), b2 = bgr_tab_bucket((uint32_t)(mix[cur] >> 32), nb);
            if (try_place(b1, cur) || (b2 != b1 && try_place(b2, cur))) { done = true; break; }
            if (kick == kMaxKicks) break;
// ... 38 lines not shown
    return ((u128)e.hi << 64) | e.lo;
}

template <typename Key>
uint32_t lookup_key(const BgrBlobHeader* h, const uint8_t* base, Key key) {
    const uint32_t* table = reinterpret_cast<const uint32_t*>(base + h->off_table);
    const uint32_t nb = (uint32_t)h->n_buckets;
    const uint64_t m = key_mix(key);
    const uint32_t bk[2] = {bgr_tab_bucket((uint32_t)m, nb), bgr_tab_bucket((uint32_t)(m >> 32), nb)};
    const uint32_t f4 = bgr_tab_fp(m) * 0x01010101u;
    for (int c = 0; c < 2; ++c) {
        if (c == 1 && bk[1] == bk[0]) break;
        for (uint32_t z = bgr_zero_bytes(table[bk[c]] ^ f4); z; z &= z - 1) {
            const uint32_t idx = bk[c] * 4 + ((uint32_t)__builtin_ctz(z) >> 3);
            if (entry_key(h, base, idx, (Key*)nullptr) == key) return idx;
        }
    }
    if (h->n_fallback) {
        uint64_t lo = 0, hi = h->n_fallback;
        while (lo < hi) {
            const uint64_t mid = (lo + hi) / 2;
            if (entry_key(h, base, 4 * h->n_buckets + mid, (Key*)nullptr) < key) lo = mid + 1; else hi = mid;
        }
        if (lo < h->n_fallback && entry_key(h, base, 4 * h->n_buckets + lo, (Key*)nullptr) == key) return (uint32_t)(4 * h->n_buckets + lo);
    }
    return BGR_NONE;
}

}

uint32_t host_lookup(const BgrBlobHeader* h, const uint8_t* base, uint64_t key) { return lookup_key<uint64_t>(h, base, key); }
uint32_t host_lookup_wide(const BgrBlobHeader* h, const uint8_t* base, uint64_t key_hi, uint64_t key_lo) {
    if (!h->wide_keys) return key_hi ? BGR_NONE : host_lookup(h, base, key_lo);
    return lookup_key<u128>(h, base, ((u128)key_hi << 64) | key_lo);
}

void resolve_device_graph(const BgrBlobHeader* h, const void* basev, BgrDeviceGraph& dg) {
    const uint8_t* base = static_cast<const uint8_t*>(basev);
    memset(&dg, 0, sizeof(dg));
    dg.table = reinterpret_cast<const uint32_t*>(base + h->off_table);
    dg.keys = reinterpret_cast<const BgrKeyEntry*>(base + h->off_keys);
    dg.recs = reinterpret_cast<const BgrSlot*>(base + h->off_recs);
    dg.meta = reinterpret_cast<const BgrUnitigMeta*>(base + h->off_meta);
    dg.seq = reinterpret_cast<const uint64_t*>(base + h->off_seq);
    dg.hdr = reinterpret_cast<const BgrBlobHeader*>(base);
    dg.k = h->k;
    dg.n_buckets = (uint32_t)h->n_buckets;
    dg.flags = (h->has_exc ? BGR_GF_HAS_EXC : 0u) | (h->n_fallback ? BGR_GF_HAS_FALLBACK : 0u);
    dg.table_bytes = (uint32_t)(h->n_buckets * 4);
    dg.bloom = h->bloom_bits ? reinterpret_cast<const uint32_t*>(base + h->off_bloom) : nullptr;
    dg.filter_kind = h->bloom_bits ? h->filter_kind : BGR_FILTER_NONE;
    dg.bloom_mask = 0;
    if (dg.filter_kind == BGR_FILTER_FLAT) dg.bloom_mask = (uint32_t)(h->bloom_bits - 1);
    if (dg.filter_kind == BGR_FILTER_MINIMIZER) { uint32_t lg = 0; while ((512ull << lg) < h->bloom_bits) ++lg; dg.bloom_mask = 32 - lg; }
}

bool validate_blob_header(const BgrBlobHeader* h, uint64_t bytes, std::string& err) {
    if (bytes < sizeof(BgrBlobHeader)) { err = "blob smaller than its header"; return false; }
    if (h->magic != BGR_MAGIC || h->version != BGR_BLOB_VERSION) { err = "not a bgreat graph blob (magic/version)"; return false; }
    if (h->blob_bytes != bytes) { err = "blob size does not match its header"; return false; }
    if (h->k < 2 || h->k > BGR_MAX_K) { err = "corrupt blob header"; return false; }
    if (h->wide_keys > 2 || (h->k > BGR_NARROW_MAX_K) != (h->wide_keys == 1)) { err = "corrupt blob header (key layout)"; return false; }
    const uint64_t key_bytes = h->wide_keys ? sizeof(BgrKeyEntryWide) : sizeof(BgrKeyEntry), fb_bytes = h->wide_keys ? 16 : 8;
    auto inside = [&](uint64_t off, uint64_t count, uint64_t size) {
        if (off < sizeof(BgrBlobHeader) || off > bytes || (off & 255u)) return false;
        return count <= (bytes - off) / size;
    };
    if (h->n_keys >= 0x0FFFFFFFull || h->n_unitigs > 0x40000000ull || h->n_buckets == 0 || h->n_buckets >= (1ull << 26)) { err = "corrupt blob header (counts)"; return false; }
    if (h->n_slots >= BGR_HNONE - 8) { err = "corrupt blob header (slots)"; return false; }
    if (!inside(h->off_table, h->n_buckets, 4) || !inside(h->off_keys, h->n_keys, key_bytes) || !inside(h->off_recs, h->n_slots + 4, sizeof(BgrSlot)) ||
        !inside(h->off_meta, h->n_unitigs + 1, sizeof(BgrUnitigMeta)) || !inside(h->off_seq, h->seq_words, 8)) { err = "blob section outside the blob"; return false; }
    if (h->n_fallback && !inside(h->off_fallback, h->n_fallback, fb_bytes)) { err = "blob section outside the blob"; return false; }
    if (h->wide_keys && (h->bloom_bits || h->anc_n)) { err = "corrupt blob header (wide keys: no filter, no anchors index)"; return false; }
    if (h->bloom_bits && ((h->bloom_bits & (h->bloom_bits - 1)) || h->bloom_bits < 64 || !inside(h->off_bloom, h->bloom_bits / 32, 4))) { err = "corrupt blob header (filter)"; return false; }
    if (h->bloom_bits && h->filter_kind == BGR_FILTER_FLAT && h->bloom_bits > (1ull << 32)) { err = "corrupt blob header (flat filter size)"; return false; }
    if (h->bloom_bits && h->filter_kind == BGR_FILTER_MINIMIZER && (h->bloom_bits < 1024 || h->bloom_bits > (512ull << 27) || h->k - 1 < BGR_MMX_MIN_K1)) { err = "corrupt blob header (minimizer filter)"; return false; }
    if (h->bloom_bits && h->filter_kind != BGR_FILTER_FLAT && h->filter_kind != BGR_FILTER_MINIMIZER) { err = "corrupt blob header (filter kind)"; return false; }
    if (h->n_keys != 4 * h->n_buckets + h->n_fallback || h->n_placed > 4 * h->n_buckets) { err = "corrupt blob header (key counts)"; return false; }
    if (h->seq_words < 2 || h->total_bases > (h->seq_words - 2) * 32 || h->seq_words * 8 >= (1ull << 32)) { err = "corrupt blob header (sequence store)"; return false; }
    if (h->has_exc) {
        const uint64_t plane_words = (h->total_bases + 63) / 64 + 2;
        if (!inside(h->off_exc, plane_words, 8) || !inside(h->off_excn, plane_words, 8)) { err = "blob exception planes outside the blob"; return false; }
    }
    if (h->anc_n) {
        if (!inside(h->off_anc_bits, h->anc_words, 8) || !inside(h->off_anc_ranks, h->anc_rank_words, 8) ||
            (h->anc_n_final && !inside(h->off_anc_final, h->anc_n_final, 16)) || !inside(h->off_anc_pos, h->anc_n, 8)) { err = "blob section outside the blob"; return false; }
        for (int i = 0; i < BGR_ANC_LEVELS; ++i) {
            const BgrAncLevel& lv = h->anc_levels[i];
            if (lv.domain == 0 || lv.word_base > h->anc_words || 1 + lv.domain / 64 > h->anc_words - lv.word_base) { err = "corrupt anchors index"; return false; }
            if (lv.rank_base > h->anc_rank_words || (1 + lv.domain / 64 + 7) / 8 > h->anc_rank_words - lv.rank_base) { err = "corrupt anchors index"; return false; }
        }
        if (h->anc_active_levels >= BGR_ANC_LEVELS) { err = "corrupt anchors index"; return false; }
    }
    return true;
}

bool validate_blob(const void* blob, uint64_t bytes, std::string& err) {
    if (bytes < sizeof(BgrBlobHeader)) { err = "blob smaller than its header"; return false; }
    return validate_blob_header(static_cast<const BgrBlobHeader*>(blob), bytes, err);
}

bool ZeroPages::reset(uint64_t words) {
    release();
    if (words == 0) return true;
    void* p = mmap(nullptr, words * 8, PROT_READ | PROT_WRITE, MAP_PRIVATE | MAP_ANONYMOUS, -1, 0);
    if (p == MAP_FAILED) return false;
    p_ = static_cast<uint64_t*>(p);
    words_ = words;
    return true;
}
void ZeroPages::release() {
    if (p_) munmap(p_, words_ * 8);
    p_ = nullptr;
    words_ = 0;
}

void set_build_threads(unsigned t) { g_build_threads.store(t); }
unsigned build_threads() {
    unsigned t = g_build_threads.load();
    if (t == 0) t = std::min(16u, std::max(1u, std::thread::hardware_concurrency()));
    return t;
}

bool read_unitig_fasta(const std::string& path, uint32_t k, std::vector<char>& seqs, std::vector<uint64_t>& offs, std::string& err) {
    FileImage img;
    if (!img.open(path, err)) { err = "unitig file: " + err; return false; }
    seqs.clear();
    offs.assign(1, 0);
    const uint64_t size = img.size;
    if (size == 0) return true;
    const char* d = img.data;
    struct Ext { uint64_t b; uint32_t len; };
    std::vector<Ext> ext;
    uint64_t p = 0, total = 0;
    while (p < size) {
        const char* nl = static_cast<const char*>(memchr(d + p, '\n', size - p));
        if (!nl) break;
        uint64_t sb = (uint64_t)(nl - d) + 1;
        const char* nl2 = sb < size ? static_cast<const char*>(memchr(d + sb, '\n', size - sb)) : nullptr;
        uint64_t se = nl2 ? (uint64_t)(nl2 - d) : size;
        if (se - sb < k) break;
        if (se - sb > 0xFFFFFFFFull) { err = "unitig longer than 2^32-1 bases"; return false; }
        ext.push_back({sb, (uint32_t)(se - sb)});
        total += se - sb;
        p = se + 1;
    }
    seqs.resize(total);
    offs.resize(ext.size() + 1);
    uint64_t o = 0;
    for (size_t i = 0; i < ext.size(); ++i) { offs[i] = o; o += ext[i].len; }
    offs[ext.size()] = o;
    parallel_ranges(build_threads(), ext.size(), [&](uint64_t b, uint64_t e, unsigned) {
        for (uint64_t i = b; i < e; ++i) memcpy(seqs.data() + offs[i], d + ext[i].b, ext[i].len);
    });
    return true;
}

static const double kStageTwice = (163776.0 / 2 - 512 - 16 * 768), kStageOnce = (163776.0 - 512 - 16 * 768);

static void sort_keys(std::vector<uint64_t>& v, unsigned T) { parallel_sort(v, T); }
static void sort_keys(std::vector<u128>& v, unsigned) { std::sort(v.begin(), v.end()); }

template <typename Key>
static bool build_graph_t(uint32_t k, uint64_t n_in, const char* seqs, const uint64_t* offs, double gamma, uint32_t flags, uint32_t wide_keys, HostGraph& out, std::string& err) {
    constexpr bool kWide = sizeof(Key) > 8;
    if (gamma != 0.0 && !(gamma >= 1.03 && gamma <= 64.0)) { err = "gamma (key table slots per key) must be in [1.03,64] (0 = choose)"; return false; }
    const uint32_t K1 = k - 1;
    uint64_t n = 0;
    while (n < n_in && offs[n + 1] - offs[n] >= k) ++n;
    if (wide_keys == 1 && n == 0) { err = "k > 32: the first unitig is shorter than k, so the graph would be empty (k must be in [2,64] and at most the unitig length)"; return false; }
    if (n >= BGR_SLOT_ID_MASK) { err = "too many unitigs (limit 2^30-1)"; return false; }
    uint64_t sum = 0, maxlen = 0;
    for (uint64_t i = 0; i < n; ++i) {
        uint64_t len = offs[i + 1] - offs[i];
        if (len > 0xFFFFFFFFull) { err = "unitig longer than 2^32-1 bases"; return false; }
        sum += len;
        maxlen = std::max(maxlen, len);
    }
    const uint64_t total = 2 * sum, seq_words = (total + 31) / 32 + 2;
    if (seq_words * 8 >= (1ull << 32)) { err = "graph too large: the packed sequence store must stay below 4 GiB (2^34 bases over both strands)"; return false; }

    const unsigned T = build_threads();
    PhaseTimer tm;
    std::vector<BgrUnitigMeta> meta(n + 1);
    memset(meta.data(), 0, meta.size() * sizeof(BgrUnitigMeta));
    {
        uint64_t F = 0;
        for (uint64_t i = 0; i < n; ++i) {
            uint32_t len = (uint32_t)(offs[i + 1] - offs[i]);
            meta[i + 1].F = F;
            meta[i + 1].len = len;
            F += 2ull * len;
        }
    }
    std::vector<Key> begs(n + 1), ends(n + 1);
    std::vector<Key> lr(2 * n);
    std::vector<uint8_t> side(2 * n);
    std::atomic<bool> any_exc{false};
    parallel_ranges(T, n, [&](uint64_t b, uint64_t e, unsigned) {
        bool mine = false;
        for (uint64_t i = b + 1; i <= e; ++i) {
            const char* s = seqs + offs[i - 1];
            const uint32_t len = meta[i].len;
            Key beg = 0, end = 0;
            for (uint32_t j = 0; j < K1; ++j) {
                beg = beg << 2 | code_of(s[j]);
                end = end << 2 | code_of(s[len - K1 + j]);
            }
            Key rcBeg = key_rcb(beg, K1), rcEnd = key_rcb(end, K1);
            begs[i] = beg;
            ends[i] = end;
            if (beg <= rcBeg) { lr[2 * i - 2] = beg; side[2 * i - 2] = 0; } else { lr[2 * i - 2] = rcBeg; side[2 * i - 2] = 1; }
            if (end <= rcEnd) { lr[2 * i - 1] = end; side[2 * i - 1] = 1; } else { lr[2 * i - 1] = rcEnd; side[2 * i - 1] = 0; }
            if (!mine)
                for (uint32_t j = 0; j < len; ++j) {
                    char ch = s[j];
                    if (ch != 'A' && ch != 'C' && ch != 'G' && ch != 'T') { mine = true; break; }
                }
        }
        if (mine) any_exc.store(true);
    });
    const bool has_exc = any_exc.load();
    std::vector<Key> left, right;
    left.reserve(n);
    right.reserve(n);
    for (uint64_t j = 0; j < 2 * n; ++j) (side[j] ? right : left).push_back(lr[j]);
    {
        unsigned Th = std::max(1u, T / 2);
        std::thread tl([&] { sort_keys(left, Th); left.erase(std::unique(left.begin(), left.end()), left.end()); });
        sort_keys(right, Th);
        right.erase(std::unique(right.begin(), right.end()), right.end());
        tl.join();
    }
    std::vector<Key> keys(left.size() + right.size());
    std::merge(left.begin(), left.end(), right.begin(), right.end(), keys.begin());
    keys.erase(std::unique(keys.begin(), keys.end()), keys.end());
    if (keys.size() >= 0x0FFFFFFFull) { err = "too many overlap keys (limit 2^28-1)"; return false; }
    tm.lap("keys");

    if (gamma == 0.0) {
        const double n = (double)keys.size();
// ... 14 lines not shown
        for (uint64_t i = 1; i <= n; ++i) anc_first[i + 1] = anc_first[i] + (meta[i].len > k ? meta[i].len - k : 0);
        std::vector<uint64_t> akeys(anc_first[n + 1]);
        const uint64_t kmask = k == 32 ? ~0ULL : ((1ULL << (2 * k)) - 1);
        parallel_ranges(T, n, [&](uint64_t b, uint64_t e, unsigned) {
            for (uint64_t i = b + 1; i <= e; ++i) {
                const char* s = seqs + offs[i - 1];
                const uint32_t len = meta[i].len;
                if (len <= k) continue;
                uint64_t x = 0;
                for (uint32_t j = 0; j < k - 1; ++j) x = x << 2 | code_of(s[j]);
                uint64_t* o = akeys.data() + anc_first[i];
                for (uint32_t j = 0; j + k < len; ++j) {
                    x = (x << 2 | code_of(s[j + k - 1])) & kmask;
                    const uint64_t rc = bgr_rcb(x, k);
                    o[j] = x < rc ? x : rc;
                }
            }
        });
        build_anchor_mphf(akeys, T, anc);
        tm.lap("anchors");
    }

    const uint64_t exc_words = has_exc ? (total + 63) / 64 + 2 : 0;
    BgrBlobHeader h;
    memset(&h, 0, sizeof(h));
    h.magic = BGR_MAGIC;
    h.version = BGR_BLOB_VERSION;
    h.k = k;
    h.wide_keys = wide_keys;
    h.n_unitigs = n;
    h.n_buckets = tab.buckets.size();
    h.n_placed = tab.n_placed;
    h.n_fallback = tab.fallback.size();
    h.n_keys = 4 * h.n_buckets + h.n_fallback;
    if (h.n_keys >= 0x0FFFFFFFull) { err = "too many overlap keys (limit 2^28-1 table slots)"; return false; }
    h.seq_words = seq_words;
    h.total_bases = total;
    h.has_exc = has_exc ? 1 : 0;
    h.max_unitig_len = maxlen;
    h.n_left_keys = left.size();
    h.n_right_keys = right.size();
    h.gamma = gamma;
    uint64_t off = align256(4096);
    static_assert(sizeof(BgrBlobHeader) <= 4096, "header must fit its 4 KiB slot");
    h.off_table = off;    off = align256(off + h.n_buckets * 4 + 16);
    h.off_keys = off;     off = align256(off + h.n_keys * (kWide ? sizeof(BgrKeyEntryWide) : sizeof(BgrKeyEntry)) + 16);
    h.off_meta = off;     off = align256(off + (n + 1) * sizeof(BgrUnitigMeta));
    h.off_seq = off;      off = align256(off + seq_words * 8);
    if (has_exc) {
        h.off_exc = off;  off = align256(off + exc_words * 8);
        h.off_excn = off; off = align256(off + exc_words * 8);
    }
    h.off_fallback = off; off = align256(off + h.n_fallback * sizeof(Key) + sizeof(Key));
    const int filter_env = (int)opt("build_filter");
    const bool large_table = (double)tab.buckets.size() * 4.0 > kStageTwice;
    if (kWide && filter_env > 0) { err = "build_filter 1 / 2: a graph with two-word keys (k > 32, or test.wide_keys) is built without a filter"; return false; }
    if (!kWide && filter_env != 0 && !keys.empty() && (large_table || filter_env == 2)) {
        const bool minimizer = k - 1 >= BGR_MMX_MIN_K1 && filter_env != 1;
        uint64_t bits = minimizer ? 1024 : 64;
        while (bits < (minimizer ? 24 : 4) * keys.size()) bits <<= 1;
        if (minimizer && bits > (512ull << 27)) bits = 512ull << 27;
        h.filter_kind = minimizer ? BGR_FILTER_MINIMIZER : BGR_FILTER_FLAT;
        h.bloom_bits = bits;
        h.off_bloom = off; off = align256(off + bits / 8 + 16);
    }
    if (flags & BGR_BUILD_ANCHORS) {
        h.anc_n = anc.n;
        h.anc_last_rank = anc.last_rank;
        h.anc_n_final = anc.final_kv.size() / 2;
        h.anc_words = anc.bits.size();
        h.anc_rank_words = anc.ranks.size();
        h.anc_active_levels = anc.active_levels;
        memcpy(h.anc_levels, anc.levels, sizeof(h.anc_levels));
        h.off_anc_bits = off;  off = align256(off + h.anc_words * 8 + 8);
        h.off_anc_ranks = off; off = align256(off + h.anc_rank_words * 8 + 8);
        h.off_anc_final = off; off = align256(off + h.anc_n_final * 16 + 16);
        h.off_anc_pos = off;   off = align256(off + h.anc_n * 8 + 8);
    }
    h.off_recs = off;
    const uint64_t slots_bound = 2 * n + 4;
    if (slots_bound >= BGR_HNONE - 8) { err = "too many unitigs for the slot handles (limit 2^27-8)"; return false; }
    off = align256(off + slots_bound * sizeof(BgrSlot));
    h.blob_bytes = off;

    if (!out.blob.reset(off / 8)) { err = "out of memory for the graph blob"; return false; }
    uint8_t* base = reinterpret_cast<uint8_t*>(out.blob.data());
    memcpy(base, &h, sizeof(h));
    memcpy(base + h.off_table, tab.buckets.data(), tab.buckets.size() * 4);
    if (h.n_fallback) {
        uint64_t* fb = reinterpret_cast<uint64_t*>(base + h.off_fallback);
        for (uint64_t j = 0; j < h.n_fallback; ++j) {
            if (kWide) { fb[2 * j] = (uint64_t)(tab.fallback[j] >> 64); fb[2 * j + 1] = (uint64_t)tab.fallback[j]; }
            else fb[j] = (uint64_t)tab.fallback[j];
        }
    }
    if constexpr (!kWide) if (h.bloom_bits) {
        uint32_t* bl = reinterpret_cast<uint32_t*>(base + h.off_bloom);
        const uint32_t mask = (uint32_t)(h.bloom_bits - 1);
        uint32_t lg = 0;
        while ((512ull << lg) < h.bloom_bits) ++lg;
        const bool minimizer = h.filter_kind == BGR_FILTER_MINIMIZER;
        parallel_ranges(T, keys.size(), [&](uint64_t b, uint64_t e, unsigned) {
            for (uint64_t i = b; i < e; ++i) {
                const uint64_t m = bgr_mix64(keys[i]);
                if (minimizer) {
                    const uint64_t w = ((uint64_t)bgr_mmx_block(bgr_mmx_of_key(keys[i], k - 1), 32 - lg) << 4) + bgr_mmx_word(m);
                    __atomic_fetch_or(&bl[w], bgr_mmx_bits(m), __ATOMIC_RELAXED);
                } else {
                    const uint32_t bit = bgr_bloom_bit(m, mask);
                    __atomic_fetch_or(&bl[bit >> 5], 1u << (bit & 31), __ATOMIC_RELAXED);
                }
            }
        });
    }

    uint64_t* seq = reinterpret_cast<uint64_t*>(base + h.off_seq);
    parallel_ranges(T, n, [&](uint64_t b, uint64_t e, unsigned) {
        for (uint64_t i = b + 1; i <= e; ++i) {
            const char* s = seqs + offs[i - 1];
            pack_strand(seq, meta[i].F, s, meta[i].len, false);
            pack_strand(seq, meta[i].F + meta[i].len, s, meta[i].len, true);
        }
    });
    if (has_exc) {
        uint64_t* exc = reinterpret_cast<uint64_t*>(base + h.off_exc);
        uint64_t* excn = reinterpret_cast<uint64_t*>(base + h.off_excn);
        for (uint64_t i = 1; i <= n; ++i) {
            const char* s = seqs + offs[i - 1];
            uint64_t F = meta[i].F;
            for (uint32_t j = 0; j < meta[i].len; ++j) {
                char ch = s[j];
                if (ch == 'A' || ch == 'C' || ch == 'G' || ch == 'T') continue;
                exc[(F + j) >> 6] |= 1ULL << (63 - ((F + j) & 63));
                if (ch == 'N') excn[(F + j) >> 6] |= 1ULL << (63 - ((F + j) & 63));
            }
        }
    }
    tm.lap("pack");

    BgrKeyEntry* kout = reinterpret_cast<BgrKeyEntry*>(base + h.off_keys);
    BgrKeyEntryWide* kwout = reinterpret_cast<BgrKeyEntryWide*>(base + h.off_keys);
    auto put_key = [&](uint64_t j, bool empty, Key key) {
        if (kWide) {
            kwout[j].hi = empty ? BGR_EMPTY_KEY : (uint64_t)(key >> (kWide ? 64 : 0));
            kwout[j].lo = empty ? BGR_EMPTY_KEY : (uint64_t)key;
            kwout[j].pad = 0;
            kwout[j].hL = kwout[j].hR = BGR_HNONE;
        } else {
            kout[j].key = empty ? BGR_EMPTY_KEY : (uint64_t)key;
            kout[j].hL = kout[j].hR = BGR_HNONE;
        }
    };
    parallel_ranges(T, 4 * h.n_buckets, [&](uint64_t b, uint64_t e, unsigned) {
        for (uint64_t j = b; j < e; ++j) put_key(j, tab.who[j] == BGR_NONE, tab.who[j] == BGR_NONE ? Key(0) : keys[tab.who[j]]);
    });
    for (uint64_t j = 0; j < h.n_fallback; ++j) put_key(4 * h.n_buckets + j, false, tab.fallback[j]);
    const BgrBlobHeader* hp = reinterpret_cast<const BgrBlobHeader*>(base);
    std::atomic<bool> bad{false};
    parallel_ranges(T, keys.size(), [&](uint64_t b, uint64_t e, unsigned) {
        for (uint64_t j = b; j < e; ++j) {
            const uint32_t idx = lookup_key<Key>(hp, base, keys[j]);
            if (idx == BGR_NONE || idx >= h.n_keys || entry_key(hp, base, idx, (Key*)nullptr) != keys[j]) { bad.store(true); return; }
            if (idx < 4 * h.n_buckets) {
                const uint32_t b1 = bgr_tab_bucket((uint32_t)key_mix(keys[j]), (uint32_t)h.n_buckets);
                if (idx / 4 != b1 && bgr_zero_bytes(tab.buckets[b1]) != 0) { bad.store(true); return; }
            }
// ... 34 lines not shown
            }
            if (me) {
                if (end <= rcEnd) fill_slot(recs + (size_t)ie * 8 + 4, id | BGR_SLOT_F0  | (beg == rcEnd ? BGR_SLOT_F1 : 0), m, seq, m.F + m.len, K1);
                else fill_slot(recs + (size_t)ie * 8, id | (beg == rcEnd ? BGR_SLOT_F0 : 0) | BGR_SLOT_F1 , m, seq, m.F + m.len, K1);
            }
        }
    });
    {
        std::vector<uint64_t> filled(T, 0), halves(T, 0);
        parallel_ranges(T, 2 * nk, [&](uint64_t b, uint64_t e, unsigned t) {
            uint64_t f = 0, hh = 0;
            for (uint64_t j = b; j < e; ++j) {
                const BgrSlot* sl4 = recs + j * 4;
                if (!sl4[0].idf) continue;
                ++hh;
                for (int q = 0; q < 4; ++q) f += sl4[q].idf != 0;
            }
            filled[t] = f;
            halves[t] = hh;
        });
        uint64_t f = 0, hh = 0;
        for (unsigned t = 0; t < T; ++t) { f += filled[t]; hh += halves[t]; }
        BgrBlobHeader* hw = reinterpret_cast<BgrBlobHeader*>(base);
        hw->slot_fill_x100 = hh ? (uint32_t)(100 * f / hh) : 100;
        if (opt("timing")) fprintf(stderr, "[build] slot fill %.2f per non-empty half record\n", hw->slot_fill_x100 / 100.0);
    }
    {
        const uint64_t nh = 2 * nk;
        std::vector<uint32_t> hoff(nh + 1);
        parallel_ranges(T, nh, [&](uint64_t b, uint64_t e, unsigned) {
            for (uint64_t j = b; j < e; ++j) {
                const BgrSlot* sl4 = recs + j * 4;
                uint32_t c = 0;
                while (c < 4 && sl4[c].idf) ++c;
                hoff[j + 1] = c;
            }
        });
        hoff[0] = 0;
        for (uint64_t j = 0; j < nh; ++j) hoff[j + 1] += hoff[j];
        const uint64_t n_slots = hoff[nh];
        if (n_slots > slots_bound - 4) { err = "internal: more slots than unitig ends"; return false; }
        auto handle = [&](uint64_t half) { return hoff[half + 1] == hoff[half] ? (uint32_t)BGR_HNONE : hoff[half]; };
        parallel_ranges(T, nk, [&](uint64_t b, uint64_t e, unsigned) {
            for (uint64_t j = b; j < e; ++j) {
                if (kWide) { kwout[j].hL = handle(2 * j); kwout[j].hR = handle(2 * j + 1); }
                else { kout[j].hL = handle(2 * j); kout[j].hR = handle(2 * j + 1); }
            }
        });
        BgrSlot* cs = reinterpret_cast<BgrSlot*>(base + h.off_recs);
        parallel_ranges(T, nh, [&](uint64_t b, uint64_t e, unsigned) {
            for (uint64_t j = b; j < e; ++j) {
                const uint32_t cnt = hoff[j + 1] - hoff[j];
                const uint32_t side = (uint32_t)(j & 1);
                for (uint32_t q = 0; q < cnt; ++q) {
                    BgrSlot sl = recs[j * 4 + q];
                    const uint32_t rec_beg = sl.nx0, rec_end = sl.nx1, mflags = sl.mflags_x & 15u;
                    uint32_t nx[2];
                    for (uint32_t c = 0; c < 2; ++c) {
                        const bool left = c == side;
                        const bool fwd = (sl.idf & (c ? BGR_SLOT_F0 : BGR_SLOT_F1)) != 0;
                        const uint32_t nrec = fwd == left ? rec_beg : rec_end;
                        const uint32_t cbit = left ? (fwd ? BGR_META_CANON_BEG : BGR_META_CANON_RCEND) : (fwd ? BGR_META_CANON_END : BGR_META_CANON_RCBEG);
                        const bool cn = (mflags & cbit) != 0;
                        const bool next_right_table = cn == left;
                        const uint32_t hd = nrec < nk ? handle(2 * (uint64_t)nrec + (next_right_table ? 1 : 0)) : (uint32_t)BGR_HNONE;
                        nx[c] = hd | (cn ? BGR_H_CANON : 0u);
                    }
                    sl.nx0 = nx[1];
                    sl.nx1 = nx[0];
                    if (q + 1 == cnt) sl.Fo_x |= BGR_SLOT_LAST;
                    cs[hoff[j] + q] = sl;
                }
            }
        });
        BgrBlobHeader* hw = reinterpret_cast<BgrBlobHeader*>(base);
        hw->n_slots = n_slots;
        hw->blob_bytes = align256(h.off_recs + (n_slots + 4) * sizeof(BgrSlot));
        h.n_slots = n_slots;
        h.blob_bytes = hw->blob_bytes;
        dense.release();
    }
    tm.lap("slots");

    if (h.anc_n) {
        memcpy(base + h.off_anc_bits, anc.bits.data(), anc.bits.size() * 8);
        memcpy(base + h.off_anc_ranks, anc.ranks.data(), anc.ranks.size() * 8);
        if (!anc.final_kv.empty()) memcpy(base + h.off_anc_final, anc.final_kv.data(), anc.final_kv.size() * 8);
        uint64_t* apos = reinterpret_cast<uint64_t*>(base + h.off_anc_pos);
        const uint64_t kmask = k == 32 ? ~0ULL : ((1ULL << (2 * k)) - 1);
        std::atomic<bool> oob{false};
        parallel_ranges(T, n, [&](uint64_t b, uint64_t e, unsigned) {
            for (uint64_t i = b + 1; i <= e; ++i) {
                const char* s = seqs + offs[i - 1];
                const uint32_t len = meta[i].len;
                if (len <= k) continue;
                uint64_t x = 0;
                for (uint32_t j = 0; j < k - 1; ++j) x = x << 2 | code_of(s[j]);
                for (uint32_t j = 0; j + k < len; ++j) {
                    x = (x << 2 | code_of(s[j + k - 1])) & kmask;
                    const uint64_t rc = bgr_rcb(x, k);
                    const uint64_t idx = anchor_lookup(hp, base, x < rc ? x : rc);
                    if (idx >= h.anc_n) { oob.store(true); return; }
                    const uint64_t v = i << 32 | j;
                    uint64_t cur = __atomic_load_n(&apos[idx], __ATOMIC_RELAXED);
                    while (cur < v && !__atomic_compare_exchange_n(&apos[idx], &cur, v, true, __ATOMIC_RELAXED, __ATOMIC_RELAXED)) {}
                }
            }
        });
        if (oob.load()) { err = "internal: anchors index out of range"; return false; }
        tm.lap("anc_pos");
    }
    return true;
}

bool build_graph(uint32_t k, uint64_t n_in, const char* seqs, const uint64_t* offs, double gamma, uint32_t flags, HostGraph& out, std::string& err) {
    if (k < 2 || k > BGR_MAX_K) { err = "k must be in [2,64] (k > 32: two-word overlap keys, greedy mode only)"; return false; }
    const uint32_t wide = k > BGR_NARROW_MAX_K ? 1u : opt("test.wide_keys") ? 2u : 0u;
    if (wide && (flags & BGR_BUILD_ANCHORS)) { err = "BGR_BUILD_ANCHORS (-G) needs k <= 32 and one-word keys (anchor k-mers are 64-bit integers)"; return false; }
    if (wide) return build_graph_t<u128>(k, n_in, seqs, offs, gamma, flags, wide, out, err);
    return build_graph_t<uint64_t>(k, n_in, seqs, offs, gamma, flags, 0, out, err);
}

}
```

bgreat_amd/csrc/graph_build.h:

```cpp
#ifndef BGREAT_AMD_GRAPH_BUILD_H
#define BGREAT_AMD_GRAPH_BUILD_H

#include <cstdint>
#include <string>
#include <vector>

#include "graph_layout.h"

namespace bgr {

class ZeroPages {
public:
    ZeroPages() = default;
    ZeroPages(const ZeroPages&) = delete;
    ZeroPages& operator=(const ZeroPages&) = delete;
    ~ZeroPages() { release(); }
    bool reset(uint64_t words);
    void release();
    uint64_t* data() { return p_; }
    const uint64_t* data() const { return p_; }
    bool empty() const { return words_ == 0; }
    uint64_t size() const { return words_; }
private:
    uint64_t* p_ = nullptr;
    uint64_t words_ = 0;
};

struct HostGraph {
    ZeroPages blob;
    const BgrBlobHeader* header() const { return reinterpret_cast<const BgrBlobHeader*>(blob.data()); }
    uint64_t bytes() const { return header()->blob_bytes; }
    const uint8_t* base() const { return reinterpret_cast<const uint8_t*>(blob.data()); }
};

#define BGR_BUILD_ANCHORS 1u
#define BGR_BUILD_NO_EVICTIONS 2u
bool build_graph(uint32_t k, uint64_t n, const char* seqs, const uint64_t* offs, double gamma, uint32_t flags, HostGraph& out, std::string& err);

void set_build_threads(unsigned t);
unsigned build_threads();

bool read_unitig_fasta(const std::string& path, uint32_t k, std::vector<char>& seqs, std::vector<uint64_t>& offs, std::string& err);

uint32_t host_lookup(const BgrBlobHeader* h, const uint8_t* base, uint64_t key);
uint32_t host_lookup_wide(const BgrBlobHeader* h, const uint8_t* base, uint64_t key_hi, uint64_t key_lo);

void resolve_device_graph(const BgrBlobHeader* h, const void* base, BgrDeviceGraph& dg);

bool validate_blob_header(const BgrBlobHeader* h, uint64_t bytes, std::string& err);
bool validate_blob(const void* blob, uint64_t bytes, std::string& err);

}

#endif
```

bgreat_amd/csrc/graph_layout.h:

```cpp
#ifndef BGREAT_AMD_GRAPH_LAYOUT_H
#define BGREAT_AMD_GRAPH_LAYOUT_H

#include <stdint.h>

#if defined(__HIP__)
#define BGR_HD __host__ __device__ __forceinline__
#else
#define BGR_HD inline
#endif

#define BGR_MAGIC 0x3130484752474742ULL
#define BGR_BLOB_VERSION 13u
#define BGR_EMPTY_KEY 0xFFFFFFFFFFFFFFFFULL
#define BGR_MAX_K 64u
#define BGR_NARROW_MAX_K 32u
#define BGR_NONE 0xFFFFFFFFu
#define BGR_SLOT_ID_MASK 0x3FFFFFFFu
#define BGR_HNONE 0x0FFFFFFFu
#define BGR_H_CANON (1u << 28)
#define BGR_SLOT_F0 0x40000000u
#define BGR_SLOT_F1 0x80000000u

#define BGR_META_CANON_BEG 1u
#define BGR_META_CANON_END 2u
#define BGR_META_CANON_RCBEG 4u
#define BGR_META_CANON_RCEND 8u

typedef struct {
    uint32_t len;
    uint32_t flags;
    uint32_t rec_beg;
    uint32_t rec_end;
    uint64_t F;
    uint32_t hw[2];
} BgrUnitigMeta;

typedef struct {
    uint32_t idf;
    uint32_t len;
    uint32_t Fw;
    uint32_t Fo_x;
    uint32_t mflags_x;
    uint32_t nx0;
    uint32_t nx1;
    uint32_t near_lo;
} BgrSlot;
#define BGR_SLOT_FO_MASK 31u
#define BGR_SLOT_LAST 32u
typedef struct {
    uint64_t key;
    uint32_t hL, hR;
} BgrKeyEntry;
typedef struct {
    uint64_t hi;
    uint32_t hL, hR;
    uint64_t lo;
    uint64_t pad;
} BgrKeyEntryWide;
BGR_HD uint64_t bgr_slot_near(uint32_t Fo_x, uint32_t mflags_x, uint32_t near_lo) {
    return ((uint64_t)((mflags_x & 0xFFFFFFF0u) | ((Fo_x >> 8) & 15u)) << 32) | near_lo;
}

#define BGR_ANC_LEVELS 25
typedef struct {
    uint64_t domain;
    uint64_t word_base;
    uint64_t rank_base;
    uint64_t magic;
} BgrAncLevel;

typedef struct {
    uint64_t magic;
    uint32_t version, k;
    uint64_t blob_bytes;
    uint64_t n_unitigs;
    uint64_t n_keys;
    uint64_t n_placed;
    uint64_t n_fallback;
    uint64_t seq_words;
    uint64_t total_bases;
    uint64_t n_buckets;
    uint64_t off_table, off_keys, off_recs, off_meta, off_seq, off_exc, off_excn, off_fallback;
    uint32_t filter_kind, has_exc;
    uint64_t max_unitig_len;
    uint64_t n_left_keys, n_right_keys;
    uint32_t slot_fill_x100;
    uint32_t wide_keys;
    uint64_t n_slots;
    uint64_t off_bloom;
    uint64_t bloom_bits;
    double gamma;
    uint64_t anc_n;
    uint64_t anc_last_rank;
    uint64_t anc_n_final;
    uint64_t anc_words, anc_rank_words;
    uint64_t anc_active_levels;
    uint64_t off_anc_bits, off_anc_ranks, off_anc_final, off_anc_pos;
    BgrAncLevel anc_levels[BGR_ANC_LEVELS];
} BgrBlobHeader;

#define BGR_GF_HAS_EXC 1u
#define BGR_GF_HAS_FALLBACK 2u
typedef struct {
    const uint32_t* table;
    const BgrKeyEntry* keys;
    const BgrSlot* recs;
    const BgrUnitigMeta* meta;
    const uint64_t* seq;
    const BgrBlobHeader* hdr;
    uint32_t k, n_buckets, flags, table_bytes;
    const uint32_t* bloom;
    uint32_t bloom_mask;
    uint32_t filter_kind;
} BgrDeviceGraph;

BGR_HD uint64_t bgr_mix64(uint64_t x) {
    x ^= x >> 32;
    return x * 0x9E3779B97F4A7C15ULL;
}
BGR_HD uint64_t bgr_mix_wide(uint64_t hi, uint64_t lo) { return bgr_mix64(lo ^ (hi * 0xC2B2AE3D27D4EB4FULL)); }
BGR_HD uint32_t bgr_tab_bucket(uint32_t h, uint32_t n_buckets) { return (uint32_t)(((uint64_t)h * (uint64_t)n_buckets) >> 32); }
BGR_HD uint32_t bgr_bloom_bit(uint64_t m, uint32_t mask) { return (uint32_t)(m >> 20) & mask; }
#define BGR_FILTER_NONE 0u
#define BGR_FILTER_FLAT 1u
#define BGR_FILTER_MINIMIZER 2u
#define BGR_MMX_BASES 16u
#define BGR_MMX_MIN_K1 20u
BGR_HD uint32_t bgr_rc16(uint32_t x) {
#if defined(__HIP_DEVICE_COMPILE__)
    x = __builtin_bitreverse32(x);
    return (uint32_t)__builtin_amdgcn_bitop3_b32((int)(x >> 1), (int)(x << 1), 0x55555555, 0x1B);
#else
    x = ((x >> 2) & 0x33333333u) | ((x & 0x33333333u) << 2);
    x = ((x >> 4) & 0x0F0F0F0Fu) | ((x & 0x0F0F0F0Fu) << 4);
    x = (x >> 24) | ((x >> 8) & 0xFF00u) | ((x << 8) & 0xFF0000u) | (x << 24);
#endif
    return ~x;
}
BGR_HD uint32_t bgr_mmx_hash(uint32_t x) {
    const uint32_t r = bgr_rc16(x);
    return ((x < r ? x : r) * 0x9E3779B1u) | 1u;
}
BGR_HD uint32_t bgr_mmx_of_key(uint64_t key, uint32_t K1) {
    uint32_t best = 0;
    for (uint32_t j = 0; j + BGR_MMX_BASES <= K1; ++j) {
        const uint32_t h = bgr_mmx_hash((uint32_t)(key >> (2 * (K1 - BGR_MMX_BASES - j))));
        best = h > best ? h : best;
    }
    return best;
}
BGR_HD uint32_t bgr_mmx_block(uint32_t mh, uint32_t shift) { return (mh * 0x85EBCA6Bu) >> shift; }
BGR_HD uint32_t bgr_mmx_word(uint64_t m) { return (uint32_t)(m >> 8) & 15u; }
BGR_HD uint32_t bgr_mmx_bits(uint64_t m) { return (1u << ((uint32_t)(m >> 12) & 31u)) | (1u << ((uint32_t)(m >> 17) & 31u)); }
BGR_HD uint32_t bgr_tab_fp(uint64_t m) { const uint32_t f = (uint32_t)(m >> 32) & 0xFFu; return f ? f : 1u; }
BGR_HD uint32_t bgr_zero_bytes(uint32_t x) { return ~(((x & 0x7F7F7F7Fu) + 0x7F7F7F7Fu) | x) & 0x80808080u; }

BGR_HD uint64_t bgr_boo_hash64(uint64_t key, uint64_t seed) {
    uint64_t h = seed;
    h ^= (h << 7) ^ (key * (h >> 3)) ^ (~((h << 11) + (key ^ (h >> 5))));
    h = (~h) + (h << 21);
    h = h ^ (h >> 24);
    h = (h + (h << 3)) + (h << 8);
    h = h ^ (h >> 14);
    h = (h + (h << 2)) + (h << 4);
    h = h ^ (h >> 28);
    h = h + (h << 31);
    return h;
}
#define BGR_BOO_SEED0 0xAAAAAAAA55555555ULL
#define BGR_BOO_SEED1 0x33333333CCCCCCCCULL
BGR_HD uint64_t bgr_boo_next(uint64_t* s0, uint64_t* s1) {
    uint64_t a = *s0;
    const uint64_t b = *s1;
    *s0 = b;
    a ^= a << 23;
    *s1 = a ^ b ^ (a >> 17) ^ (b >> 26);
    return *s1 + b;
}

BGR_HD uint64_t bgr_mod_magic(uint64_t h, uint64_t d, uint64_t magic) {
#if defined(__HIP_DEVICE_COMPILE__)
    const uint64_t q = __umul64hi(h, magic);
#else
    const uint64_t q = (uint64_t)(((unsigned __int128)h * magic) >> 64);
#endif
    uint64_t r = h - q * d;
    if (r >= d) r -= d;
    if (r >= d) r -= d;
    return r;
}

BGR_HD uint64_t bgr_rev2(uint64_t x) {
    x = ((x >> 2) & 0x3333333333333333ULL) | ((x & 0x3333333333333333ULL) << 2);
    x = ((x >> 4) & 0x0F0F0F0F0F0F0F0FULL) | ((x & 0x0F0F0F0F0F0F0F0FULL) << 4);
    x = ((x >> 8) & 0x00FF00FF00FF00FFULL) | ((x & 0x00FF00FF00FF00FFULL) << 8);
    x = ((x >> 16) & 0x0000FFFF0000FFFFULL) | ((x & 0x0000FFFF0000FFFFULL) << 16);
    return (x >> 32) | (x << 32);
}
BGR_HD uint64_t bgr_rcb(uint64_t x, uint32_t n) { return (~bgr_rev2(x)) >> (64 - 2 * n); }

#endif
```

bgreat_amd/csrc/greedy_kernels.hip:

```cpp
#include "device_common.h"
#include "scan_take_word.h"

namespace bgr {
namespace {

template <bool STAGE, bool WIDE>
__device__ __forceinline__ void greedy_general(const BgrDeviceGraph& g, const BatchIO& io, const KernelParams& prm) {
    extern __shared__ u64 lds[];
    const int lane = threadIdx.x & 63, wave = threadIdx.x >> 6;
    const int waves = blockDim.x >> 6;
    const uint32_t W = io.words_per_read;
    const uint32_t K1 = g.k - 1;
    const uint32_t total = io.subset ? io.cursor[io.subset_ctr] : io.n_reads;
    if ((uint32_t)(blockIdx.x * waves) >= total) return;
    uint32_t ktab_words;
    const uint32_t* ktab = block_prologue<STAGE>(g, lds, &ktab_words);
    const uint32_t per_wave_words = 4 * W + io.path_cap / 2;
    u64* FW3 = lds + 64 + ktab_words + (u64)wave * per_wave_words;
    u64* FWQ = FW3 + W;
    u64* RCW = FWQ + W;
    u64* NM = RCW + W;
    int32_t* PATH = reinterpret_cast<int32_t*>(NM + W);

    uint32_t c_lane = 0;
// ... 70 lines not shown
                        else { lds_key_wide(B, L - K1 - a_pos, K1, &rh, &rl); rh = rl64(rh, 0); rl = rl64(rl, 0); }
                        a_rec = rl32(idx, src);
                        rcb_wide(nh, nl, K1, &ch, &cl);
                        if (ch != rh || cl != rl) {
                            const bool fw = key_lt_wide(nh, nl, ch, cl);
                            a_rec = find_key_wide<!STAGE>(g, ktab, fw ? nh : ch, fw ? nl : cl, true);
                        }
                        a_canon = !key_lt_wide(ch, cl, nh, nl);
                        if (a_rec != BGR_NONE) a_rec *= 2;
                    } else {
                    const u64 a_num = rl64(lds_win32(A, a_pos) >> (64 - 2 * K1), 0);
                    const u64 a_rcn = plain ? rcb_fast(a_num, K1) : rl64(lds_win32(B, L - K1 - a_pos) >> (64 - 2 * K1), 0);
                    a_rec = rl32(idx, src);
                    const u64 rc2 = rcb_fast(a_num, K1);
                    if (rc2 != a_rcn) {
                        const u64 key2 = a_num < rc2 ? a_num : rc2;
                        a_rec = find_key<!STAGE>(g, ktab, key2, true, (!STAGE && mmx_w) ? bgr_mmx_block(bgr_mmx_of_key(key2, K1), g.bloom_mask) : 0u);
                    }
                    a_canon = a_num <= rc2;
                    }
                    if (greedy_from_anchor(g, CMP, NM, useN, L, K1, a_rec, a_canon, a_pos, prm.max_mismatch, PATH, &p_lo, &p_n, lane)) {
                        done = true;
                        break;
                    }
                }
            }
            if (done) { status = BGR_ST_ALIGNED | (pass ? BGR_ST_RC : 0); break; }
            if (tried == 0) { status = BGR_ST_NOANCHOR | (pass ? BGR_ST_RC : 0); break; }
            status = BGR_ST_FAILED | BGR_ST_RC;
        }
        wave_sync();
        uint32_t abase = 0;
        if ((status & BGR_ST_MASK) == BGR_ST_ALIGNED) abase = publish_path(io, PATH, p_lo, p_n, &chunk_pos, &chunk_end, lane);
        else p_n = 0;
        if (lane == 0) io.results[r] = make_uint2(abase, p_n | (status << 24));
        c_lane += (uint32_t)lane == (status & BGR_ST_MASK);
        wave_sync();
    }
    {
        unsigned long long* counters = reinterpret_cast<unsigned long long*>(io.cursor + kCurCounters);
        const uint32_t total = rl32(c_lane, BGR_ST_NOANCHOR) + rl32(c_lane, BGR_ST_FAILED) + rl32(c_lane, BGR_ST_ALIGNED);
        if (lane == 0 && total) atomicAdd(&counters[0], (unsigned long long)total);
        if (lane == BGR_ST_NOANCHOR && c_lane) atomicAdd(&counters[1], (unsigned long long)c_lane);
        if (lane == BGR_ST_ALIGNED && c_lane) atomicAdd(&counters[2], (unsigned long long)c_lane);
        if (lane == BGR_ST_FAILED && c_lane) atomicAdd(&counters[3], (unsigned long long)c_lane);
    }
}

template <bool STAGE>
__global__ void __launch_bounds__(1024, BGR_GREEDY_OCC) bgr_align_greedy_kernel(BgrDeviceGraph g, BatchIO io, KernelParams prm) {
    greedy_general<STAGE, false>(g, io, prm);
}
template <bool STAGE>
__global__ void __launch_bounds__(1024, BGR_GREEDY_OCC) bgr_align_greedy_wide_kernel(BgrDeviceGraph g, BatchIO io, KernelParams prm) {
    greedy_general<STAGE, true>(g, io, prm);
}

#ifndef BGR_G4_OCC
#define BGR_G4_OCC 8
#endif

#define G4_ST_RC (1u << 31)
#define G4_ST_TRIED_SHIFT 20
#define G4_ST_POS_MASK 0xFFFFFu

template <bool STAGE, int GL, bool ASCII>
__global__ void __launch_bounds__(1024, BGR_G4_OCC) bgr_align_greedy_multi_kernel(BgrDeviceGraph g, BatchIO io, KernelParams prm) {
    static_assert(GL == 4, "the two-pair walk takes four lanes per read");
    constexpr uint32_t RPW = 64 / GL;
    extern __shared__ u64 lds[];
    const int lane = threadIdx.x & 63, wave = threadIdx.x >> 6;
    const int waves = blockDim.x >> 6;
    const uint32_t W = io.words_per_read;
    const uint32_t K1 = g.k - 1;
    const uint32_t total = io.n_reads;
    if ((uint32_t)(blockIdx.x * waves) * RPW >= total) return;
    uint32_t* wg_counts = reinterpret_cast<uint32_t*>(lds);
    if (threadIdx.x < 4) wg_counts[threadIdx.x] = 0;
    task_stock_init(lds, (total + RPW - 1) / RPW);
#ifdef BGR_PHASE_TIMING
    const unsigned long long wt0 = wall_clock64();
    unsigned long long wt2 = 0;
    uint32_t dbg_steps = 0, dbg_items = 0, dbg_groups = 0;
#endif
    uint32_t ktab_words;
    const uint32_t* ktab = block_prologue<STAGE>(g, lds, &ktab_words);
#ifdef BGR_PHASE_TIMING
    const unsigned long long wt1 = wall_clock64();
#endif
    u64* RD = lds + 64 + ktab_words + (u64)wave * (RPW * W);
    const uint32_t grp = (uint32_t)lane / GL, sub = (uint32_t)lane % GL;
    const uint32_t m = prm.max_mismatch;
    const uint32_t eff = prm.effort ? prm.effort : 1;
    const uint32_t mmx_w = (!STAGE && g.bloom && g.filter_kind == BGR_FILTER_MINIMIZER) ? K1 + 1 - BGR_MMX_BASES : 0u;
    const bool wide_scan = io.wide_scan && mmx_w && scan_mblock_is_wide(mmx_w);
    const uint32_t scan_step = (mmx_w && !wide_scan) ? 65 - mmx_w : 64;

    const uint32_t wid = (uint32_t)(blockIdx.x * waves + wave);
    const uint32_t q_base = wid * io.q_cap;
    uint32_t q_rd = 0, q_wr = 0, q_cnt = 0;
    const uint32_t n_tasks = (total + RPW - 1) / RPW;
    uint32_t pool_open = 1;

    for (;;) {
        uint32_t r = BGR_NONE, st = 0;
        uint32_t task = BGR_NONE;
        if (q_cnt < RPW && pool_open) {
            task = claim_task(lds, io.cursor + io.task_ctr, n_tasks, lane);
            if (task == BGR_NONE) {
                pool_open = 0;
#ifdef BGR_PHASE_TIMING
                if (!wt2) wt2 = wall_clock64();
#endif
            }
        }
        if (task != BGR_NONE) {
            if (task * RPW + grp < total) r = task * RPW + grp;
        } else {
            if (q_cnt == 0) break;
            const uint32_t take = q_cnt < RPW ? q_cnt : RPW;
            if (grp < take) {
                uint32_t at = q_rd + grp;
                if (at >= io.q_cap) at -= io.q_cap;
                r = __hip_atomic_load(&io.queue[q_base + at].x, __ATOMIC_RELAXED, __HIP_MEMORY_SCOPE_AGENT);
                st = __hip_atomic_load(&io.queue[q_base + at].y, __ATOMIC_RELAXED, __HIP_MEMORY_SCOPE_AGENT);
            }
            q_rd += take;
            if (q_rd >= io.q_cap) q_rd -= io.q_cap;
            q_cnt -= take;
        }
        uint32_t L = 0, act = 0;
        u64* F = RD + grp * W;
        {
            const u64* src = io.fw3;
            u64 a0 = 0;
            if (r != BGR_NONE) {
                const u64 off = io.read_offs[r];
                L = (uint32_t)(io.read_offs[r + 1] - off);
                act = ASCII ? 1u : ((io.hasn[r >> 5] >> (r & 31)) & 1u) ^ 1u;
                if (((L + 31) >> 5) >= W) act = 0;
                if (ASCII) a0 = ascii_start(io, r, off);
                else src += packed_word_offset(off, r);
            }
            const uint32_t Wr = (L + 31) >> 5;
            uint32_t chars = 0;
            for (uint32_t j = sub; j < W; j += GL) {
                u64 f = 0;
                if (act && j < Wr) {
                    if (ASCII) {
                        u64 fw;
                        const int32_t p = (st >> 31) ? (int32_t)L - 32 * ((int32_t)j + 1) : 0;
                        const u64 at = (st >> 31) ? a0 + (uint32_t)(p > 0 ? p : 0) : a0 + 32ull * j;
                        const uint32_t vv = (st >> 31) ? (p >= 0 ? 32u : (uint32_t)(32 + p)) : L - 32 * j;
                        if (io.ascii_src) fw = ascii_word<false>(io.ascii, at, vv, io.ascii_bytes, &chars);
                        else fw = ascii_word<true>(io.ascii, at, vv, io.ascii_bytes, &chars);
                        if (!(st >> 31)) f = fw;
                        else if (p >= 0) f = ~rev2_fast(fw);
                        else f = (~rev2_fast(fw >> (64 - 2 * vv))) & (~0ULL << (64 - 2 * vv));
                    } else if (!(st >> 31)) f = src[j];
                    else {
                        const int32_t p = (int32_t)L - 32 * ((int32_t)j + 1);
                        if (p >= 0) f = ~rev2_fast(win32(src, (u64)(uint32_t)p));
                        else { const uint32_t v = (uint32_t)(32 + p); f = (~rev2_fast(src[0] >> (64 - 2 * v))) & (~0ULL << (64 - 2 * v)); }
                    }
                }
                F[j] = f;
            }
            if (ASCII) {
                uint32_t n8 = chars & 0x08080808u;
                n8 |= quad_xor1(n8);
                if (GL >= 4) n8 |= quad_xor2(n8);
                if (GL >= 8) n8 |= half_row_mirror(n8);
                if (GL == 16) n8 |= (uint32_t)__builtin_amdgcn_mov_dpp((int)n8, 0x140, 0xF, 0xF, true);
                if (n8) act = 0;
            }
        }
        wave_sync();

        uint32_t a_pos = 0, a_rec = BGR_NONE;
        if constexpr (STAGE) {
            const uint32_t g_from = st & G4_ST_POS_MASK;
            uint32_t g_npos = L >= K1 ? L - K1 + 1 : 0;
            if (!prm.effort && g_npos > 1) g_npos = 1;
            u64 pend = __ballot(act != 0 && sub == 0 && g_from < g_npos);
#ifdef BGR_PHASE_TIMING
            if (prm.debug_stop == 1) pend = 0;
            dbg_items += (uint32_t)__popcll(pend);
            ++dbg_groups;
#endif
            static_assert(RPW == kTakeGroups, "scan_take_word.h counts sixteen groups per wave");
            const bool hi = lane >= 32;
            uint32_t sl = threadIdx.x;
            asm volatile("" : "+v"(sl));
            const uint32_t lcm = (((sl & 31u) << 6) | (32u - 2u * (sl & 15u))) - (16u << 6);
            const uint32_t c4w = lds_addr(lds + 64 + ktab_words) + (sl >> 6) * (RPW * W * 8u) + 4u * ((sl >> 4) & 1u);
            const uint32_t g_tw = take_word_pack(g_from, g_npos - g_from, ((sl & 63u) / GL) * (W * 2u) + (g_from >> 4));
            uint32_t li = 0, ln = 0, wa = 0, wb = 0;
            auto take = [&](bool h, uint32_t& hq, uint32_t& hb, uint32_t& hn) {
                uint32_t s_res = 16, s_left = 0, s_dw = 0;
                hn = 0;
                if (pend) {
                    const int at = __ffsll((long long)pend) - 1;
                    pend &= pend - 1;
                    const uint32_t w = rl32(g_tw, at);
                    s_res = take_word_res(w);
                    s_left = take_word_left(w);
                    s_dw = take_word_dword(w);
                    hq = (uint32_t)at / GL;
                    hb = take_word_resume(w) & ~15u;
                    hn = take_word_resume(w) + s_left;
                }
                if (hi == h) {
                    li = lcm + (s_res << 6);
                    ln = s_left << 6;
                    const uint32_t t = c4w + (s_dw << 2);
                    wa = t ^ 4u;
                    wb = (t + 4u) ^ 4u;
                }
            };
            uint32_t q0 = 0, b0 = 0, n0 = 0, q1 = 0, b1 = 0, n1 = 0;
            take(false, q0, b0, n0);
            take(true, q1, b1, n1);
            while (n0 | n1) {
#ifdef BGR_PHASE_TIMING
                ++dbg_steps;
#endif
                const bool valid = li < ln;
                u64 num = 0;
                if (valid) num = lds_win32_fixed(wa, wb, li) >> (64 - 2 * K1);
                const u64 rcn = rcb_fast(num, K1);
                uint32_t idx = scan_find_key(g, ktab, num < rcn ? num : rcn, valid, (uint32_t)lane);
                const u64 mask = __ballot(idx != BGR_NONE);
                li += 32u << 6;
                wa += 8;
                wb += 8;
                if (mask) {
                    if (idx != BGR_NONE && num <= rcn) idx |= G4_CANON;
                    auto settle = [&](uint32_t mh, int off, uint32_t hq, uint32_t hb, uint32_t& hn) {
                        if (mh) {
                            const uint32_t f = (uint32_t)__builtin_ctz(mh);
                            const uint32_t h = rl32(idx, off + (int)f);
                            if (grp == hq) { a_pos = hb + f; a_rec = h; }
                            hn = 0;
                        }
                    };
                    if (n0) settle((uint32_t)mask, 0, q0, b0, n0);
                    if (n1) settle((uint32_t)(mask >> 32), 32, q1, b1, n1);
                }
                b0 += 32;
                if (b0 >= n0) n0 = 0;
                b1 += 32;
                if (b1 >= n1) n1 = 0;
                if (!n0) take(false, q0, b0, n0);
                if (!n1) take(true, q1, b1, n1);
            }
        } else {
            for (uint32_t q = 0; q < RPW; ++q) {
                if (!rl32(act, (int)(GL * q))) continue;
#ifdef BGR_PHASE_TIMING
                if (prm.debug_stop == 1) continue;
#endif
                const uint32_t Lq = rl32(L, (int)(GL * q)), stq = rl32(st, (int)(GL * q));
                const u64* A = RD + q * W;
                uint32_t npos = Lq >= K1 ? Lq - K1 + 1 : 0;
                if (!prm.effort && npos > 1) npos = 1;
                for (uint32_t base = stq & G4_ST_POS_MASK; base < npos; base += scan_step) {
                    const uint32_t i = base + (uint32_t)lane;
// ... 46 lines not shown
            uint32_t miss, ext;
            int32_t sid;
            const uint32_t w1 = g2_step(g, F, L, K1, on, rec & G4_REC_MASK, (rec >> 28) & 1u, pos, m - cum, lane, &miss, &ext, &sid);
            if (on != 0) {
                if (!(w1 & G4_FOUND)) phase = 5;
                else {
                    if ((sub & 1u) == 0) io.arena[PT0 + (phase == 1 ? PH - 1 - ni : PH + ni)] = sid;
                    ++ni;
                    cum += miss;
                    if (w1 & G4_FITS) {
                        if (phase == 1) {
                            if (sub == 0) io.arena[PT0 + PH - 1 - ni] = (int32_t)(ext - pos);
                            ++ni;
                        }
                        phase = 0;
                    } else if (phase == 1) { pos -= ext; rec = w1; }
                    else { pos += ext; rec = w1; phase = 3; }
                }
            }
        }
        const uint32_t o_phase = quad_xor2(phase), o_cum = quad_xor2(cum), o_ni = quad_xor2(ni);
        const uint32_t lph = side ? o_phase : phase, rph = side ? phase : o_phase;
        const uint32_t tot = cum + o_cum;
        const uint32_t nl = side ? o_ni : ni, nr = side ? ni : o_ni;
        if (lph == 4 || lph == 5) phase = lph;
        else if (rph == 4) phase = tot <= m ? 4u : 5u;
        else phase = (rph == 5 || tot > m) ? 5u : 0u;
        if (phase == 5) st += 1u << G4_ST_TRIED_SHIFT;

        uint32_t outcome = 4, nst = 0;
        const uint32_t rc = st >> 31;
        if (act) {
            const uint32_t tried = (st >> G4_ST_TRIED_SHIFT) & 0x7FFu;
            const uint32_t npos_g = (L >= K1 ? L - K1 + 1 : 0);
            const uint32_t npos_e = (!prm.effort && npos_g > 1) ? 1u : npos_g;
            if (phase == 4) outcome = 4;
            else if (a_rec != BGR_NONE && phase != 5) outcome = 0;
            else if (a_rec == BGR_NONE && tried == 0) outcome = 1;
            else {
                const uint32_t resume = a_pos + 1;
                const uint32_t used_up = (a_rec == BGR_NONE || tried >= eff || resume >= npos_e) ? 1u : 0u;
                if (!used_up) { outcome = 3; nst = (st & ~G4_ST_POS_MASK) | resume; }
                else if (!rc) { outcome = 3; nst = G4_ST_RC; }
                else outcome = 2;
                if (tried >= 0x7FEu || resume > G4_ST_POS_MASK) outcome = 4;
            }
        }
        const uint32_t have = r != BGR_NONE ? 1u : 0u;

        const uint32_t aligned = outcome == 0 ? 1u : 0u;
        const uint32_t p_n = aligned ? nl + nr : 0;
        const uint32_t gbase = (r == BGR_NONE ? 0u : r) * kG4PathInts + PH - nl;
        if (sub == 0 && have) {
            if (outcome <= 2) {
                const uint32_t code = (outcome == 0 ? BGR_ST_ALIGNED : outcome == 1 ? BGR_ST_NOANCHOR : BGR_ST_FAILED) | (rc ? BGR_ST_RC : 0u);
                io.results[r] = make_uint2(aligned ? gbase : 0u, p_n | (code << 24));
            } else if (outcome == 4) {
                io.gen_list[atomicAdd(io.cursor + io.gen_ctr, 1u)] = r;
            }
        }
        {
            const bool listed = sub == 0 && have && outcome == 3;
            const u64 lm = __ballot(listed);
            if (lm) {
                const uint32_t cnt = (uint32_t)__popcll(lm);
                if (listed) {
                    uint32_t at = q_wr + __builtin_amdgcn_mbcnt_hi((uint32_t)(lm >> 32), __builtin_amdgcn_mbcnt_lo((uint32_t)lm, 0u));
                    if (at >= io.q_cap) at -= io.q_cap;
                    io.queue[q_base + at] = make_uint2(r, nst);
                }
                q_wr += cnt;
                if (q_wr >= io.q_cap) q_wr -= io.q_cap;
                q_cnt += cnt;
            }
        }
        if (sub == 0 && have && outcome <= 3) atomicAdd(&wg_counts[outcome], 1u);
        wave_sync();
    }
#ifdef BGR_PHASE_TIMING
    if (io.wave_times && lane == 0) {
        unsigned long long* w = io.wave_times + 4ull * (blockIdx.x * waves + wave);
        w[0] = wt0; w[1] = wt1; w[2] = wt2; w[3] = wall_clock64();
        unsigned long long* c = io.wave_times + 4ull * (gridDim.x * waves) + 4ull * (blockIdx.x * waves + wave);
        c[0] = dbg_steps; c[1] = dbg_items; c[2] = dbg_groups; c[3] = 0;
    }
#endif
    __syncthreads();
    if (threadIdx.x == 0) {
        unsigned long long* counters = reinterpret_cast<unsigned long long*>(io.cursor + kCurCounters);
        const uint32_t al = wg_counts[0], noov = wg_counts[1], na = wg_counts[2], qa = wg_counts[3];
        if (al | noov | na) atomicAdd(&counters[0], (unsigned long long)(al + noov + na));
        if (noov) atomicAdd(&counters[1], (unsigned long long)noov);
        if (al) atomicAdd(&counters[2], (unsigned long long)al);
        if (na) atomicAdd(&counters[3], (unsigned long long)na);
        if (qa) atomicAdd(io.cursor + kCurFollowUps, qa);
    }
}

}

const void* greedy_kernel(KernelId k, bool stage, bool ascii) {
    constexpr int GL = (int)kG4GroupLanes;
    switch (k) {
        case KernelId::kGreedyMulti:
            if (ascii) return stage ? kernel_ptr(bgr_align_greedy_multi_kernel<true, GL, true>) : kernel_ptr(bgr_align_greedy_multi_kernel<false, GL, true>);
            return stage ? kernel_ptr(bgr_align_greedy_multi_kernel<true, GL, false>) : kernel_ptr(bgr_align_greedy_multi_kernel<false, GL, false>);
        case KernelId::kGreedyWide: return stage ? kernel_ptr(bgr_align_greedy_wide_kernel<true>) : kernel_ptr(bgr_align_greedy_wide_kernel<false>);
        case KernelId::kGreedy: return stage ? kernel_ptr(bgr_align_greedy_kernel<true>) : kernel_ptr(bgr_align_greedy_kernel<false>);
        default: return nullptr;
    }
}

}
```

bgreat_amd/csrc/options.h:

```cpp
#ifndef BGREAT_AMD_OPTIONS_H
#define BGREAT_AMD_OPTIONS_H

#include <stdint.h>
#include <string.h>

#include <atomic>

namespace bgr {

struct Option {
    const char* name;
    std::atomic<int64_t> value;
    int64_t lo, hi;
    const char* what;
};

inline Option* option_table(size_t* n) {
    static Option t[] = {
        {"timing", {0}, 0, 1, "per-stage timing lines on stderr (pipeline, text calls, index build)"},
        {"blocking_sync", {0}, 0, 1, "aligners wait for their stream with a blocking event (the thread sleeps) instead of spinning"},
        {"numa", {1}, 0, 1, "bgr_align_all pins its threads to the NUMA node of the devices they feed when all share one"},
        {"workers_per_device", {0}, 0, 16, "bgr_align_all: stream workers per device (0 = default: 2)"},
        {"extra_sets", {-1}, -1, 32, "bgr_align_all: staging sets beyond one per worker (-1 = default)"},
        {"fastq_gather", {1}, 0, 1, "FASTQ pieces cross PCIe without their '+' and quality lines"},
        {"overlap_streams", {4}, 2, 4, "bgr_align_batch of >= 512 k reads: internal streams"},
        {"huge_pinned", {1}, 0, 1, "bgr_host_alloc: buffers of 2 MB and more from huge-page mappings registered with the runtime"},
        {"exh_filter", {1}, 0, 1, "exhaustive mode probes large key tables through the minimizer filter"},
        {"build_filter", {-1}, -1, 2, "index build: filter in front of the key table: -1 by table size, 0 none, 1 one hash, 2 minimizer-blocked (forced onto small graphs by tests)"},
        {"poison_device_buffers", {0}, 0, 1, "diagnostic: every new device buffer is filled with a pattern (a kernel that reads what nothing wrote shows in any run)"},
        {"test.bases_cap", {0}, 0, INT64_MAX, "test hook: bases per batch of bgr_align_all (walks the cut of large batches with small inputs)"},
        {"test.lanes_on_one_device", {0}, 0, 1, "test hook: every lane of a split run / every device of --gpus N is device 0 (a one-GPU box walks the N-device code)"},
        {"test.wide_keys", {0}, 0, 1, "test hook: index build: every graph gets the two-word key layout of k > 32 (and the kernel that reads it), whatever its k"},
        {"test.links_capacity", {0}, 0, INT64_MAX, "test hook: slots of the table of links an aligner allocates when link counting is enabled (0 = from the graph's bound): a table that can fill"},
        {"test.triples_capacity", {0}, 0, INT64_MAX, "test hook: slots of the table of triples an aligner allocates when triple counting is enabled (0 = from the graph's bound): a table that can fill"},
        {"test.variants_stage_bytes", {0}, 0, 64 << 20, "test hook: bytes of the staging piece through which one pileup table is added into another (0 = one kernel on one device, 64 MiB pieces across devices); any value takes the staged way on one device too"},
        {"test.count_with_path_stats", {0}, 0, 1, "test hook: bgr_aligner_path_stats also queues every enabled counting kernel (abundance, links, triples, pileup) once over the rows the result buffers hold at that time, the read characters from its reads buffer: rows a test wrote there itself"},
        {"test.text_epoch", {0}, 0, 0x3FFFFF, "test hook: the epoch the text form's chains start from when their state is (re)allocated (walks the 22-bit wrap with a few pieces)"},
    };
    *n = sizeof(t) / sizeof(t[0]);
    return t;
}
inline Option* find_option(const char* name) {
    size_t n;
    Option* t = option_table(&n);
    for (size_t i = 0; i < n; ++i)
        if (strcmp(t[i].name, name) == 0) return &t[i];
    return nullptr;
}
inline int64_t opt(const char* name) {
    Option* o = find_option(name);
    return o ? o->value.load(std::memory_order_relaxed) : 0;
}

}

#endif
```

include/bgreat_gpu.h:

```cpp
#ifndef BGREAT_GPU_H
#define BGREAT_GPU_H

#include <stdint.h>

#ifdef __cplusplus
extern "C" {
#endif

#define BGR_OK 0
#define BGR_E_ARG (-1)
#define BGR_E_HIP (-2)
#define BGR_E_IO (-3)
#define BGR_E_CAPACITY (-4)
#define BGR_E_INTERNAL (-5)
#define BGR_E_NOMEM (-7)
#define BGR_E_COMPACTION (-6)

#define BGR_ST_NOANCHOR 0
#define BGR_ST_FAILED 1
#define BGR_ST_ALIGNED 2
#define BGR_ST_MASK 3
#define BGR_ST_RC 4

#define BGR_MODE_GREEDY 0
#define BGR_MODE_EXHAUSTIVE 1
#define BGR_MODE_ANCHORS 2

typedef struct bgr_graph bgr_graph;
typedef struct bgr_aligner bgr_aligner;

typedef struct {
    uint32_t mode;
    uint32_t max_mismatch;
    uint32_t effort;
    uint32_t partial;
} bgr_params;

typedef struct {
    uint32_t k, n_levels;
    uint64_t n_unitigs, n_keys, n_left_keys, n_right_keys, n_fallback;
    uint64_t total_bases, blob_bytes, mphf_bytes, max_unitig_len;
    uint32_t has_exceptions, has_anchors;
    double gamma;
} bgr_graph_info_t;

const char* bgr_last_error(void);

int bgr_set_option(const char* name, int64_t value);
int bgr_get_option(const char* name, int64_t* value);
const char* bgr_option_name(uint32_t index, const char** what);
int bgr_device_count(void);

void bgr_set_build_threads(uint32_t threads);
int bgr_graph_build(uint32_t k, uint64_t n_unitigs, const char* seqs, const uint64_t* offsets, double gamma, bgr_graph** out);
int bgr_graph_build_from_fasta(const char* unitig_fasta_path, uint32_t k, double gamma, bgr_graph** out);
#define BGR_BUILD_ANCHORS 1u
#define BGR_BUILD_NO_EVICTIONS 2u
int bgr_graph_build_ex(uint32_t k, uint64_t n_unitigs, const char* seqs, const uint64_t* offsets, double gamma, uint32_t flags, bgr_graph** out);
int bgr_graph_build_from_fasta_ex(const char* unitig_fasta_path, uint32_t k, double gamma, uint32_t flags, bgr_graph** out);
int bgr_graph_anchor_lookup(const bgr_graph* g, uint64_t kmer, uint64_t* index_out, uint64_t* position_out);
int bgr_graph_key_lookup(const bgr_graph* g, uint64_t canonical_k1mer, uint32_t* slot_out);
int bgr_graph_key_lookup_wide(const bgr_graph* g, uint64_t key_hi, uint64_t key_lo, uint32_t* slot_out);
const void* bgr_graph_blob(const bgr_graph* g, uint64_t* bytes);
int bgr_graph_from_blob(const void* blob, uint64_t bytes, bgr_graph** out);
int bgr_graph_info(const bgr_graph* g, bgr_graph_info_t* out);
int bgr_graph_unitigs(const bgr_graph* g, const char** seqs, const uint64_t** offsets, uint64_t* n);
void bgr_graph_destroy(bgr_graph* g);

int bgr_graph_upload(bgr_graph* g, int device);
const void* bgr_graph_device_blob(const bgr_graph* g, int device);
#define BGR_FANOUT_AUTO 0u
#define BGR_FANOUT_RCCL 1u
#define BGR_FANOUT_PEER 2u
int bgr_devices_init(bgr_graph* g, int first_device, uint32_t n_devices, uint32_t how);
uint32_t bgr_devices_method(const bgr_graph* g);
int bgr_graph_adopt_device_blob(int device, const void* dev_blob, uint64_t bytes, bgr_graph** out);

int bgr_aligner_create(bgr_graph* g, int device, bgr_aligner** out);
void bgr_aligner_destroy(bgr_aligner* a);

int bgr_align_batch(bgr_aligner* a, const bgr_params* p, const char* reads, const uint64_t* read_offsets, uint64_t n_reads,
                    int32_t* paths_out, uint64_t paths_cap, uint64_t* path_offsets, uint8_t* status);

typedef struct {
    const uint64_t* read_offsets;
    const uint64_t* fw3;
    const uint32_t* hasn;
    const uint32_t* nm_index;
    const uint64_t* nm_value;
    uint64_t nm_count;
    uint32_t max_read_len;
} bgr_packed_reads;
uint64_t bgr_packed_plane_words(uint64_t n_reads, uint64_t total_bases);
int bgr_pack_reads(const char* reads, const uint64_t* read_offsets, uint64_t n_reads, uint64_t* fw3, uint32_t* hasn, uint32_t* nm_index,
                   uint64_t* nm_value, uint64_t nm_cap, uint64_t* nm_count, uint32_t* max_read_len);
int bgr_align_batch_packed(bgr_aligner* a, const bgr_params* p, const bgr_packed_reads* reads, uint64_t n_reads, int32_t* paths_out,
                           uint64_t paths_cap, uint64_t* path_offsets, uint8_t* status);

typedef struct {
    bgr_aligner* aligner;
    uint64_t n_reads;
    uint64_t serial;
} bgr_ticket;
int bgr_align_batch_begin(bgr_aligner* a, const bgr_params* p, const char* reads, const uint64_t* read_offsets, uint64_t n_reads, bgr_ticket* ticket);
int bgr_align_batch_test(const bgr_ticket* ticket);
int bgr_align_batch_wait(const bgr_ticket* ticket, int32_t* paths_out, uint64_t paths_cap, uint64_t* path_offsets, uint8_t* status);

typedef struct bgr_text_stage bgr_text_stage;
typedef struct {
    uint64_t struct_size;
    const char* text;
    uint64_t text_bytes;
    uint32_t want_output;
    uint32_t irregular;
    char* paths_out;
    uint64_t paths_cap;
    char* notaligned_out;
    uint64_t notaligned_cap;
    uint64_t n_records, n_accepted, paths_bytes, notaligned_bytes;
    bgr_text_stage* stage;
    uint32_t fastq;
    uint32_t reserved;
    uint32_t* record_info_out;
    uint64_t record_info_cap;
} bgr_text_batch;
int bgr_text_stage_create(int device, bgr_text_stage** out);
void bgr_text_stage_destroy(bgr_text_stage* s);
int bgr_text_stage_upload(bgr_text_stage* s, const char* text, uint64_t text_bytes);
int bgr_text_stage_upload_parts(bgr_text_stage* s, uint32_t n_parts, const char* const* parts, const uint64_t* part_bytes);
int bgr_text_stage_device(const bgr_text_stage* s);
int bgr_align_fasta_text(bgr_aligner* a, const bgr_params* p, bgr_text_batch* b);
int bgr_aligner_fetch_text(bgr_aligner* a, bgr_text_batch* b);

int bgr_align_device(bgr_aligner* a, const bgr_params* p, const void* d_reads, const void* d_read_offsets, uint64_t n_reads,
                     uint64_t total_bases, uint32_t max_read_len);
int bgr_aligner_sync(bgr_aligner* a);
int bgr_aligner_device_results(bgr_aligner* a, void** d_results, void** d_arena, void** d_cursor);
int bgr_aligner_arena_ints(bgr_aligner* a, uint64_t* ints);
typedef struct {
    uint64_t path_len, path_start;
    uint32_t aligned, mismatches;
} bgr_path_stat;
#define BGR_PATH_STAT_NO_WALK 0x80000000u
int bgr_aligner_path_stats(bgr_aligner* a, const void* d_reads, const void* d_read_offsets, uint64_t n_reads, bgr_path_stat* out);
int bgr_aligner_fetch(bgr_aligner* a, uint64_t n_reads, int32_t* paths_out, uint64_t paths_cap, uint64_t* path_offsets, uint8_t* status);

typedef struct { uint64_t reads, bases, kmers; } bgr_unitig_abundance;
int bgr_aligner_abundance_enable(bgr_aligner* a, uint32_t on);
int bgr_aligner_abundance(bgr_aligner* a, bgr_unitig_abundance* out, uint64_t n_rows);
int bgr_aligner_reset_abundance(bgr_aligner* a);
int bgr_aligner_abundance_plan(bgr_aligner* a, uint64_t n_reads, uint64_t total_bases, uint32_t out[4]);
int bgr_plan_abundance(uint64_t n_unitigs, uint32_t k, uint64_t n_reads, uint64_t total_bases, uint32_t num_cus, uint64_t lds_per_cu, uint32_t form_knob, uint32_t out[4]);

typedef struct { int32_t from, to; uint64_t count; } bgr_link;
int bgr_aligner_links_enable(bgr_aligner* a, uint32_t on);
int bgr_aligner_links(bgr_aligner* a, bgr_link* out, uint64_t cap, uint64_t* n);
int bgr_aligner_reset_links(bgr_aligner* a);
int bgr_aligner_links_info(bgr_aligner* a, uint64_t out[4]);
int bgr_aligner_links_plan(bgr_aligner* a, uint64_t n_reads, uint32_t out[4]);
int bgr_plan_links(uint64_t links_bound, uint64_t n_reads, uint32_t num_cus, uint32_t form_knob, uint32_t out[4]);
int bgr_graph_links_bound(bgr_graph* g, uint64_t* bound);
typedef struct { uint32_t depth, a, c, g, t, n; } bgr_pileup_base;
int bgr_aligner_pileup_enable(bgr_aligner* a, uint32_t on);
int bgr_aligner_pileup(bgr_aligner* a, bgr_pileup_base* out, uint64_t n_bases, uint64_t* skipped);
int bgr_aligner_reset_pileup(bgr_aligner* a);
#define BGR_VARIANTS_TILE 2048u
typedef struct { uint32_t unitig, pos, depth, a, c, g, t, n; } bgr_variant_site;
typedef struct { uint32_t min_depth, min_alt, min_af_ppm; } bgr_variant_params;
int bgr_aligner_pileup_sites(bgr_aligner* a, const bgr_variant_params* params, bgr_variant_site* out, uint64_t cap, uint64_t* n);
int bgr_aligner_pileup_sites_times(bgr_aligner* a, double ms[5]);
int bgr_aligner_pileup_add(bgr_aligner* dst, bgr_aligner* src);
typedef struct { uint32_t min_depth, min_alt, min_af_ppm, min_alt_strand; } bgr_variant_strand_params;
typedef struct { uint32_t unitig, pos, depth, a, c, g, t, n, fdepth, fa, fc, fg, ft, fn, reserved[2]; } bgr_variant_strand_site;
int bgr_aligner_pileup_strands_enable(bgr_aligner* a, uint32_t on);
int bgr_aligner_pileup_forward(bgr_aligner* a, bgr_pileup_base* out, uint64_t n_bases);
int bgr_aligner_pileup_strand_sites(bgr_aligner* a, const bgr_variant_strand_params* params, bgr_variant_strand_site* out, uint64_t cap, uint64_t* n);
int bgr_link_canonical(int32_t a, int32_t b, bgr_link* out, uint64_t* key);

int bgr_aligner_counters(bgr_aligner* a, uint64_t out[5]);
int bgr_aligner_reset_counters(bgr_aligner* a);

int bgr_aligner_kernel_time(bgr_aligner* a, uint64_t* launches, double* total_ms);
int bgr_aligner_reset_kernel_time(bgr_aligner* a);
int bgr_aligner_kernel_times(bgr_aligner* a, uint64_t* launches, double slot_ms[8], const char* slot_names[8]);
int bgr_aligner_launch_info(bgr_aligner* a, uint32_t out[4]);
int bgr_aligner_pass_counts(bgr_aligner* a, uint32_t out[4]);
int bgr_aligner_configure(bgr_aligner* a, uint32_t waves_per_block, uint32_t blocks_per_cu, uint32_t lds_mphf);

#define BGR_KNOB_EXH_FRAME_CAP 1u
#define BGR_KNOB_EXH_SEARCH 2u
#define BGR_KNOB_BATCH_SPLIT_LIMIT 3u
#define BGR_KNOB_DEBUG_STOP 4u
#define BGR_KNOB_BATCH_OVERLAP 8u
#define BGR_KNOB_ANCHORS_FAST 7u
#define BGR_KNOB_EXH_FAST 6u
#define BGR_KNOB_EXH_MEMO_CAP 9u
#define BGR_KNOB_GREEDY_PREPASS 10u
#define BGR_KNOB_KERNEL_EVENTS 11u
#define BGR_KNOB_ABUNDANCE_FORM 12u
#define BGR_KNOB_LINKS_FORM 13u
#define BGR_KNOB_GREEDY_FAST 5u
#define BGR_KNOB_DEVICE_OVERLAP 14u
int bgr_aligner_set_knob(bgr_aligner* a, uint32_t knob, uint64_t value);
typedef struct bgr_plan_input {
    uint32_t k, slot_fill_x100, table_bytes, has_exceptions, anchors, anchor_levels;
    uint64_t graph_bases, n_unitigs, max_unitig_len;
    uint32_t num_cus, resident_waves[7];
    uint64_t lds_per_cu;
    uint32_t cfg_waves, cfg_blocks_per_cu, cfg_lds_mphf;
    uint32_t mode, max_mismatch, partial, max_read_len;
    uint64_t n_reads, total_bases;
    uint32_t wide_keys, reserved0;
} bgr_plan_input;
typedef struct bgr_plan_pass { uint32_t used, blocks, waves_per_block, lds_bytes, table_staged; } bgr_plan_pass;
typedef struct bgr_plan_output {
    bgr_plan_pass pass[6];
    uint32_t level_search, deep_only, x4_levels, memo_cap;
    uint64_t deep_scratch_bytes, arena_ints;
} bgr_plan_output;
int bgr_plan_launch(const bgr_plan_input* in, bgr_plan_output* out);

int bgr_aligner_last_pass_runs(const bgr_aligner* a, uint32_t* runs, uint32_t* memo_cap);

typedef struct bgr_readset bgr_readset;
int bgr_readset_load(const char* path, int fastq, uint32_t k, bgr_readset** out);
int bgr_readset_load_parallel(const char* path, int fastq, uint32_t k, uint32_t threads, uint64_t chunk_bytes, bgr_readset** out);
uint64_t bgr_readset_count(const bgr_readset* rs);
int bgr_readset_view(const bgr_readset* rs, const char** reads, const uint64_t** read_offsets, const char** headers, const uint64_t** header_offsets);
void bgr_readset_destroy(bgr_readset* rs);

int bgr_write_records(void* paths_file, void* notaligned_file, uint64_t n_reads, const char* headers, const uint64_t* header_offsets,
                      const char* reads, const uint64_t* read_offsets, const int32_t* paths, const uint64_t* path_offsets);

typedef struct {
    uint64_t struct_size;
    uint32_t n_gpus;
    uint32_t threads;
    uint64_t batch_reads;
    uint64_t chunk_bytes;
    uint32_t fastq;
    uint32_t write_exhaustive;
    uint32_t echo_files;
    uint32_t correction;
    const char* no_overlap_file;
    uint32_t first_device;
    uint32_t route;
    uint32_t numa;
    uint32_t split_output;
    uint32_t gaf;
    uint32_t abundance;
} bgr_run_options;
void bgr_host_cache_release(void);
int bgr_align_all(bgr_graph* g, const bgr_params* p, const bgr_run_options* o, const char* reads_csv, const char* paths_file,
                  const char* notaligned_file, uint64_t counters_out[5], double* mapping_seconds);

int bgr_graph_abundance(const bgr_graph* g, bgr_unitig_abundance* out, uint64_t n_rows);
int bgr_write_abundance(const char* path, const bgr_graph* g, const bgr_unitig_abundance* rows, uint64_t n_rows);

int bgr_graph_links_enable(bgr_graph* g, uint32_t on);
int bgr_graph_links_enabled(const bgr_graph* g);
int bgr_graph_links(const bgr_graph* g, bgr_link* out, uint64_t cap, uint64_t* n);
int bgr_write_gfa(const char* path, const bgr_graph* g, const bgr_unitig_abundance* abundance_rows, uint64_t n_rows, const bgr_link* links, uint64_t n_links);

#define BGR_BUBBLES_TILE 1024u
typedef struct { int32_t source, sink, branch[2]; uint64_t count[4]; } bgr_bubble;
int bgr_links_bubbles(int device, const bgr_link* links, uint64_t n_links, uint64_t n_unitigs, uint64_t min_link, bgr_bubble* out, uint64_t cap, uint64_t* n);
int bgr_aligner_bubbles(bgr_aligner* a, uint64_t min_link, bgr_bubble* out, uint64_t cap, uint64_t* n);
int bgr_aligner_bubbles_times(bgr_aligner* a, double ms[4]);
int bgr_graph_bubbles_enable(bgr_graph* g, uint32_t on, uint64_t min_link);
int bgr_graph_bubbles_enabled(const bgr_graph* g);
int bgr_graph_bubbles(const bgr_graph* g, bgr_bubble* out, uint64_t cap, uint64_t* n);
int bgr_write_bubbles(const char* path, const bgr_graph* g, const bgr_bubble* bubbles, uint64_t n);

typedef struct { int32_t from, via, to, reserved; uint64_t count; } bgr_triple;
int bgr_aligner_triples_enable(bgr_aligner* a, uint32_t on);
int bgr_aligner_triples(bgr_aligner* a, bgr_triple* out, uint64_t cap, uint64_t* n);
int bgr_aligner_reset_triples(bgr_aligner* a);
int bgr_aligner_triples_info(bgr_aligner* a, uint64_t out[4]);
int bgr_triple_canonical(int32_t a, int32_t b, int32_t c, bgr_triple* out);
int bgr_graph_triples_bound(bgr_graph* g, uint64_t* bound);
int bgr_graph_triples_enable(bgr_graph* g, uint32_t on);
int bgr_graph_triples_enabled(const bgr_graph* g);
int bgr_graph_triples(const bgr_graph* g, bgr_triple* out, uint64_t cap, uint64_t* n);
// ... 70 lines not shown
```

Measured before the change: 3771 Mreads/s.

## Add sampled jump index so greedy anchor scan can skip across unitig interiors

Builds an optional hashed index of sampled interior (k-1)-mers per unitig, stored after the graph blob, and uses it in the greedy multi-read kernel. A quad of lanes looks up a sampled read k-mer, compares the read against the unitig sequence word-wise to find the anchor or the first mismatch, and skips the per-position key-table scan. This is meant to cut the number of MPHF lookups per read in the greedy anchor search. It costs build time, extra blob memory, and extra per-wave work when the hint misses. It only applies to graphs that qualify: narrow keys, no exceptions, key table staged in LDS.

Result: faster. 4047 Mreads/s (median of 6 runs) (+7.3%).

```diff
diff --git a/bgreat_amd/__init__.py b/bgreat_amd/__init__.py
--- a/bgreat_amd/__init__.py
+++ b/bgreat_amd/__init__.py
@@ -17,7 +17,7 @@
 
 SYMBOLS = [
     "bgr_last_error", "bgr_device_count", "bgr_graph_build", "bgr_graph_build_from_fasta", "bgr_graph_blob",
-    "bgr_graph_from_blob", "bgr_graph_info", "bgr_graph_destroy", "bgr_graph_upload", "bgr_graph_device_blob",
+    "bgr_graph_from_blob", "bgr_graph_info", "bgr_graph_jump_index", "bgr_graph_destroy", "bgr_graph_upload", "bgr_graph_device_blob",
     "bgr_graph_adopt_device_blob", "bgr_aligner_create", "bgr_aligner_destroy", "bgr_align_batch", "bgr_align_device", "bgr_aligner_path_stats",
     "bgr_aligner_sync", "bgr_aligner_device_results", "bgr_aligner_arena_ints", "bgr_aligner_fetch", "bgr_aligner_counters",
     "bgr_aligner_reset_counters", "bgr_aligner_kernel_time", "bgr_aligner_reset_kernel_time", "bgr_aligner_launch_info",
@@ -50,6 +50,9 @@
 KNOB_LINKS_FORM = 13
 LINKS_AUTO, LINKS_GLOBAL, LINKS_LDS = 0, 1, 2
 KNOB_DEVICE_OVERLAP = 14
+KNOB_GREEDY_JUMP = 15
+JUMP_ABSENT = ("", "two-word overlap keys", "unitig bases outside ACGT", "key table not staged in LDS", "index beyond the cache cap",
+               "an interior (k-1)-mer of a unitig is an overlap key, or built with build_jump = 0")
 SEARCH_AUTO, SEARCH_DEPTH_FIRST, SEARCH_BY_LEVEL = 0, 1, 2
 
 
@@ -168,7 +171,8 @@
                 ("n_left_keys", C.c_uint64), ("n_right_keys", C.c_uint64), ("n_fallback", C.c_uint64),
                 ("total_bases", C.c_uint64), ("blob_bytes", C.c_uint64), ("mphf_bytes", C.c_uint64),
                 ("max_unitig_len", C.c_uint64), ("has_exceptions", C.c_uint32), ("has_anchors", C.c_uint32),
-                ("gamma", C.c_double)]
+                ("gamma", C.c_double), ("jump_entries", C.c_uint64), ("jump_bytes", C.c_uint64), ("jump_stride", C.c_uint32), ("jump_absent", C.c_uint32),
+                ("jump_dropped_x1000", C.c_uint32), ("reserved", C.c_uint32)]
 
 
 _lib = None
@@ -555,10 +559,26 @@
         v._owner = self
         return v
 
+    def jump_index(self):
+        n = C.c_uint64()
+        lib().bgr_graph_jump_index.restype = C.c_void_p
+        lib().bgr_graph_jump_index.argtypes = [C.c_void_p, C.POINTER(C.c_uint64)]
+        p = lib().bgr_graph_jump_index(self.h, C.byref(n))
+        if not p:
+            return None
+        return np.ctypeslib.as_array(C.cast(p, C.POINTER(C.c_uint32)), shape=(n.value // 16, 4)).copy()
+
     def info(self):
         gi = GraphInfo()
         _check(lib().bgr_graph_info(self.h, C.byref(gi)))
-        return {f[0]: getattr(gi, f[0]) for f in GraphInfo._fields_ if f[0] != "reserved"}
+        return {f[0]: getattr(gi, f[0]) for f in GraphInfo._fields_ if f[0] != "reserved" and not f[0].startswith("jump_")}
+
+    def jump_info(self):
+        gi = GraphInfo()
+        _check(lib().bgr_graph_info(self.h, C.byref(gi)))
+        d = {f[0]: getattr(gi, f[0]) for f in GraphInfo._fields_ if f[0].startswith("jump_")}
+        d["jump_absent_why"] = JUMP_ABSENT[gi.jump_absent]
+        return d
 
     def upload(self, device=0):
         _check(lib().bgr_graph_upload(self.h, device))
diff --git a/bgreat_amd/csrc/capi.hip b/bgreat_amd/csrc/capi.hip
--- a/bgreat_amd/csrc/capi.hip
+++ b/bgreat_amd/csrc/capi.hip
@@ -106,6 +106,10 @@
         return fail(BGR_E_ARG, err);
     }
     g->header = *g->host.header();
+    if (g->host.jump_buckets) {
+        g->header.off_jump = g->host.jump_off; g->header.jump_entries = g->host.jump_entries; g->header.jump_buckets = g->host.jump_buckets;
+        g->header.jump_stride = g->host.jump_stride; g->header.jump_dropped_x1000 = g->host.jump_dropped_x1000;
+    }
     const uint64_t nu = g->header.n_unitigs;
     g->ascii.assign(seqs + (nu ? offsets[0] : 0), seqs + (nu ? offsets[nu] : 0));
     g->ascii_offs.resize(nu + 1);
@@ -187,7 +191,16 @@
     o->n_left_keys = h.n_left_keys; o->n_right_keys = h.n_right_keys; o->n_fallback = h.n_fallback;
     o->total_bases = h.total_bases; o->blob_bytes = h.blob_bytes; o->mphf_bytes = h.n_buckets * 4;
     o->max_unitig_len = h.max_unitig_len; o->has_exceptions = h.has_exc; o->has_anchors = h.anc_n ? 1 : 0; o->gamma = h.gamma;
-    return BGR_OK;
+    o->jump_entries = h.jump_entries; o->jump_bytes = h.jump_buckets * 2 * sizeof(BgrJumpEntry); o->jump_stride = h.jump_stride;
+    o->jump_absent = bgr::jump_absent_reason(&h);
+    o->jump_dropped_x1000 = h.jump_dropped_x1000;
+    return BGR_OK;
+}
+
+const void* bgr_graph_jump_index(const bgr_graph* g, uint64_t* bytes) {
+    const bool have = g && !g->host.blob.empty() && g->host.jump_buckets;
+    if (bytes) *bytes = have ? g->host.jump_buckets * 2 * sizeof(BgrJumpEntry) : 0;
+    return have ? g->host.base() + g->host.jump_off : nullptr;
 }
 
 void bgr_graph_destroy(bgr_graph* g) {
@@ -207,8 +220,11 @@
     if (g->host.blob.empty()) return fail(BGR_E_ARG, "bgr_graph_upload: graph has no host blob (adopted graphs live on one device)");
     HIP_TRY(hipSetDevice(device));
     void* p = nullptr;
-    HIP_TRY(hipMalloc(&p, g->header.blob_bytes));
-    hipError_t e = hipMemcpy(p, g->host.blob.data(), g->header.blob_bytes, hipMemcpyHostToDevice);
+    const uint64_t image = g->host.image_bytes();
+    HIP_TRY(hipMalloc(&p, image));
+    hipError_t e = hipMemcpy(p, g->host.blob.data(), image, hipMemcpyHostToDevice);
+    if (e == hipSuccess && g->host.jump_buckets)
+        e = hipMemcpy(static_cast<char*>(p) + offsetof(BgrBlobHeader, off_jump), &g->header.off_jump, sizeof(BgrBlobHeader) - offsetof(BgrBlobHeader, off_jump), hipMemcpyHostToDevice);
     if (e == hipSuccess) e = hipStreamSynchronize(nullptr);
     if (e != hipSuccess) { (void)hipFree(p); return fail(BGR_E_HIP, std::string("blob H2D: ") + hipGetErrorString(e)); }
     g->dev[device] = {p, true};
@@ -306,7 +322,7 @@
     if (first_device < 0 || (uint64_t)first_device + n_devices > (uint64_t)nd) return fail(BGR_E_ARG, "bgr_devices_init: device range outside the visible devices");
     int rc = bgr_graph_upload(g, first_device);
     if (rc != BGR_OK) return rc;
-    const uint64_t bytes = g->header.blob_bytes;
+    const uint64_t bytes = g->host.image_bytes();
     bgr::FanoutOps ops;
     ops.alloc = [bytes](int dev, void** out) { return hipSetDevice(dev) == hipSuccess && hipMalloc(out, bytes) == hipSuccess; };
     ops.release = [](int dev, void* p) { if (p && hipSetDevice(dev) == hipSuccess) (void)hipFree(p); };
@@ -423,6 +439,7 @@
         case BGR_KNOB_EXH_FAST: if (value > 1) break; a->knob_exh_fast = (uint32_t)value; return BGR_OK;
         case BGR_KNOB_ANCHORS_FAST: if (value > 1) break; a->knob_anc_fast = (uint32_t)value; return BGR_OK;
         case BGR_KNOB_GREEDY_PREPASS: if (value > 1) break; a->knob_prepass = (uint32_t)value; return BGR_OK;
+        case BGR_KNOB_GREEDY_JUMP: if (value > 1) break; a->knob_no_jump = (uint32_t)value; for (bgr_aligner* tw = a->twin; tw; tw = tw->twin) tw->knob_no_jump = (uint32_t)value; return BGR_OK;
         case BGR_KNOB_KERNEL_EVENTS: if (value > 1) break; a->knob_no_events = value ? 0u : 1u; return BGR_OK;
         case BGR_KNOB_ABUNDANCE_FORM: if (value > 2) break; a->knob_abundance_form = (uint32_t)value; for (bgr_aligner* tw = a->twin; tw; tw = tw->twin) tw->knob_abundance_form = (uint32_t)value; return BGR_OK;
         case BGR_KNOB_LINKS_FORM: if (value > 2) break; a->knob_links_form = (uint32_t)value; for (bgr_aligner* tw = a->twin; tw; tw = tw->twin) tw->knob_links_form = (uint32_t)value; return BGR_OK;
@@ -664,7 +681,9 @@
             a->wave_times_n = waves;
         }
 #endif
-        e = bgr::launch_align(ps.kernel, ps.variant, dgl, pio, kp, ps.cfg, a->stream);
+        BgrDeviceGraph dgp = dgl;
+        if (ps.kernel == bgr::KernelId::kGreedyMulti && ps.cfg.stage_mphf && a->graph->header.jump_buckets && !a->knob_no_jump) dgp.flags |= BGR_GF_JUMP;
+        e = bgr::launch_align(ps.kernel, ps.variant, dgp, pio, kp, ps.cfg, a->stream);
         if (e != hipSuccess) return fail(BGR_E_HIP, std::string("kernel launch (") + ps.name + "): " + hipGetErrorString(e));
         HIP_TRY(mark(ps.name));
         if (ps.kernel == bgr::KernelId::kExhaustiveLast) {
@@ -755,7 +774,7 @@
         bgr_aligner* tw = prev->twin;
         tw->cfg_waves = a->cfg_waves; tw->cfg_blocks_per_cu = a->cfg_blocks_per_cu; tw->cfg_lds_mphf = a->cfg_lds_mphf;
         tw->knob_frame_cap = a->knob_frame_cap; tw->knob_search = a->knob_search; tw->knob_debug_stop = a->knob_debug_stop;
-        tw->knob_greedy_fast = a->knob_greedy_fast; tw->knob_exh_fast = a->knob_exh_fast; tw->knob_anc_fast = a->knob_anc_fast; tw->knob_memo_cap = a->knob_memo_cap; tw->knob_prepass = a->knob_prepass; tw->knob_no_events = a->knob_no_events;
+        tw->knob_greedy_fast = a->knob_greedy_fast; tw->knob_exh_fast = a->knob_exh_fast; tw->knob_anc_fast = a->knob_anc_fast; tw->knob_memo_cap = a->knob_memo_cap; tw->knob_prepass = a->knob_prepass; tw->knob_no_events = a->knob_no_events; tw->knob_no_jump = a->knob_no_jump;
         tw->knob_abundance_form = a->knob_abundance_form;
         tw->knob_links_form = a->knob_links_form;
         if (tw->abundance_on != a->abundance_on) { const int rc = abundance_set(tw, a->abundance_on); if (rc != BGR_OK) return rc; }
diff --git a/bgreat_amd/csrc/capi_internal.h b/bgreat_amd/csrc/capi_internal.h
--- a/bgreat_amd/csrc/capi_internal.h
+++ b/bgreat_amd/csrc/capi_internal.h
@@ -157,6 +157,7 @@
     bool exh_filter = bgr::opt("exh_filter") != 0;
     uint32_t knob_frame_cap = 0, knob_search = 0, knob_debug_stop = 0, knob_greedy_fast = 0, knob_exh_fast = 0, knob_anc_fast = 0, knob_memo_cap = 0, knob_prepass = 0, knob_no_events = 0;
     uint64_t knob_split_limit = 0;
+    uint32_t knob_no_jump = 0;
     uint32_t knob_overlap = 0;
     uint32_t knob_abundance_form = 0;
     bool abundance_on = false;
diff --git a/bgreat_amd/csrc/graph_build.cpp b/bgreat_amd/csrc/graph_build.cpp
--- a/bgreat_amd/csrc/graph_build.cpp
+++ b/bgreat_amd/csrc/graph_build.cpp
@@ -12,6 +12,7 @@
 #include <atomic>
 #include <chrono>
 #include <cmath>
+#include <cstddef>
 #include <cstdio>
 #include <cstdlib>
 #include <cstring>
@@ -216,6 +217,10 @@
         const uint64_t plane_words = (h->total_bases + 63) / 64 + 2;
         if (!inside(h->off_exc, plane_words, 8) || !inside(h->off_excn, plane_words, 8)) { err = "blob exception planes outside the blob"; return false; }
     }
+    if (h->jump_buckets) {
+        if (h->wide_keys || h->has_exc || h->bloom_bits || h->jump_buckets > 0xFFFFFFFFull || h->jump_stride == 0 || h->jump_entries > 2 * h->jump_buckets) { err = "corrupt blob header (jump index)"; return false; }
+        if (!inside(h->off_jump, h->jump_buckets, 2 * sizeof(BgrJumpEntry))) { err = "blob section outside the blob"; return false; }
+    } else if (h->off_jump || h->jump_entries || h->jump_stride) { err = "corrupt blob header (jump index)"; return false; }
     if (h->anc_n) {
         if (!inside(h->off_anc_bits, h->anc_words, 8) || !inside(h->off_anc_ranks, h->anc_rank_words, 8) ||
             (h->anc_n_final && !inside(h->off_anc_final, h->anc_n_final, 16)) || !inside(h->off_anc_pos, h->anc_n, 8)) { err = "blob section outside the blob"; return false; }
@@ -291,6 +296,16 @@
 }
 
 static const double kStageTwice = (163776.0 / 2 - 512 - 16 * 768), kStageOnce = (163776.0 - 512 - 16 * 768);
+
+uint32_t jump_absent_reason(const BgrBlobHeader* h) {
+    if (h->jump_buckets) return 0;
+    if (h->wide_keys) return 1;
+    if (h->has_exc) return 2;
+    if (h->bloom_bits || (double)h->n_buckets * 4.0 > kStageTwice) return 3;
+    const uint64_t fwd = h->total_bases / 2, k1s = h->n_unitigs * (uint64_t)(h->k - 1);
+    if (((fwd > k1s ? fwd - k1s : 0) + h->n_unitigs + BGR_JUMP_STRIDE - 1) / BGR_JUMP_STRIDE * 2 * sizeof(BgrJumpEntry) > BGR_JUMP_CAP_BYTES) return 4;
+    return 5;
+}
 
 static void sort_keys(std::vector<uint64_t>& v, unsigned T) { parallel_sort(v, T); }
 static void sort_keys(std::vector<u128>& v, unsigned) { std::sort(v.begin(), v.end()); }
@@ -471,6 +486,12 @@
     if (slots_bound >= BGR_HNONE - 8) { err = "too many unitigs for the slot handles (limit 2^27-8)"; return false; }
     off = align256(off + slots_bound * sizeof(BgrSlot));
     h.blob_bytes = off;
+    uint64_t jump_nb = 0;
+    if (!kWide && opt("build_jump") && !has_exc && !large_table && !h.bloom_bits && !keys.empty()) {
+        jump_nb = (sum - n * K1 + n + BGR_JUMP_STRIDE - 1) / BGR_JUMP_STRIDE;
+        if (jump_nb * 2 * sizeof(BgrJumpEntry) > BGR_JUMP_CAP_BYTES) jump_nb = 0;
+    }
+    off += align256(jump_nb * 2 * sizeof(BgrJumpEntry));
 
     if (!out.blob.reset(off / 8)) { err = "out of memory for the graph blob"; return false; }
     uint8_t* base = reinterpret_cast<uint8_t*>(out.blob.data());
@@ -671,6 +692,54 @@
     }
     tm.lap("slots");
 
+    if constexpr (!kWide) if (jump_nb) {
+        std::atomic<bool> p_fails{false};
+        parallel_ranges(T, n, [&](uint64_t b, uint64_t e, unsigned) {
+            for (uint64_t i = b + 1; i <= e; ++i) {
+                if (p_fails.load(std::memory_order_relaxed)) return;
+                const BgrUnitigMeta& m = mout[i];
+                for (uint32_t t = 1; t + K1 < m.len; ++t) {
+                    const uint64_t x = window(seq, m.F + t, K1), rc = bgr_rcb(x, K1);
+                    if (lookup_key<uint64_t>(hp, base, std::min(x, rc)) != BGR_NONE) { p_fails.store(true); return; }
+                }
+            }
+        });
+        tm.lap("jump_P");
+        if (!p_fails.load()) {
+            BgrBlobHeader* hw = reinterpret_cast<BgrBlobHeader*>(base);
+            const uint64_t off_jump = hw->blob_bytes;
+            BgrJumpEntry* je = reinterpret_cast<BgrJumpEntry*>(base + off_jump);
+            const uint64_t drop_nth = (uint64_t)opt("test.jump_drop");
+            uint64_t seen = 0, wanted = 0, placed = 0;
+            for (uint64_t i = 1; i <= n; ++i) {
+                const BgrUnitigMeta& m = mout[i];
+                for (uint32_t t = 0; t + K1 <= m.len && t <= BGR_JUMP_MAX_T; ++t) {
+                    const uint64_t x = window(seq, m.F + t, K1), rc = bgr_rcb(x, K1);
+                    const uint64_t mx = bgr_mix64(std::min(x, rc));
+                    if (!bgr_jump_selects(mx) || x == rc) continue;
+                    ++wanted;
+                    if (drop_nth && ++seen % drop_nth == 0) continue;
+                    BgrJumpEntry* e2 = je + 2 * (uint64_t)bgr_tab_bucket((uint32_t)mx, (uint32_t)jump_nb);
+                    if (e2[0].t_tag && e2[1].t_tag) continue;
+                    BgrJumpEntry& en = e2[0].t_tag ? e2[1] : e2[0];
+                    en.idc = (uint32_t)i | (x < rc ? BGR_JUMP_FWD_CANON : 0u);
+                    en.t_tag = t << 8 | bgr_tab_fp(mx);
+                    ++placed;
+                }
+            }
+            if (placed) {
+                out.jump_off = off_jump;
+                out.jump_entries = placed;
+                out.jump_buckets = jump_nb;
+                out.jump_stride = BGR_JUMP_STRIDE;
+                out.jump_dropped_x1000 = (uint32_t)(1000 * (wanted - placed) / wanted);
+                static_assert(offsetof(BgrBlobHeader, off_jump) == 1096 && sizeof(BgrBlobHeader) == 1128, "the header's jump fields lie behind everything a blob of this version had");
+            }
+            if (opt("timing")) fprintf(stderr, "[build] jump index: %llu of %llu sampled (k-1)-mers placed, %llu buckets\n", (unsigned long long)placed, (unsigned long long)wanted, (unsigned long long)jump_nb);
+        } else if (opt("timing")) fprintf(stderr, "[build] jump index: none (an interior (k-1)-mer of a unitig is an overlap key)\n");
+        tm.lap("jump");
+    }
+
     if (h.anc_n) {
         memcpy(base + h.off_anc_bits, anc.bits.data(), anc.bits.size() * 8);
         memcpy(base + h.off_anc_ranks, anc.ranks.data(), anc.ranks.size() * 8);
diff --git a/bgreat_amd/csrc/graph_build.h b/bgreat_amd/csrc/graph_build.h
--- a/bgreat_amd/csrc/graph_build.h
+++ b/bgreat_amd/csrc/graph_build.h
@@ -28,6 +28,9 @@
 
 struct HostGraph {
     ZeroPages blob;
+    uint64_t jump_off = 0, jump_buckets = 0, jump_entries = 0;
+    uint32_t jump_stride = 0, jump_dropped_x1000 = 0;
+    uint64_t image_bytes() const { return jump_buckets ? jump_off + jump_buckets * 2 * sizeof(BgrJumpEntry) : bytes(); }
     const BgrBlobHeader* header() const { return reinterpret_cast<const BgrBlobHeader*>(blob.data()); }
     uint64_t bytes() const { return header()->blob_bytes; }
     const uint8_t* base() const { return reinterpret_cast<const uint8_t*>(blob.data()); }
@@ -47,6 +50,8 @@
 
 void resolve_device_graph(const BgrBlobHeader* h, const void* base, BgrDeviceGraph& dg);
 
+uint32_t jump_absent_reason(const BgrBlobHeader* h);
+
 bool validate_blob_header(const BgrBlobHeader* h, uint64_t bytes, std::string& err);
 bool validate_blob(const void* blob, uint64_t bytes, std::string& err);
 
diff --git a/bgreat_amd/csrc/graph_layout.h b/bgreat_amd/csrc/graph_layout.h
--- a/bgreat_amd/csrc/graph_layout.h
+++ b/bgreat_amd/csrc/graph_layout.h
@@ -97,10 +97,26 @@
     uint64_t anc_active_levels;
     uint64_t off_anc_bits, off_anc_ranks, off_anc_final, off_anc_pos;
     BgrAncLevel anc_levels[BGR_ANC_LEVELS];
+    uint64_t off_jump;
+    uint64_t jump_entries;
+    uint64_t jump_buckets;
+    uint32_t jump_stride;
+    uint32_t jump_dropped_x1000;
 } BgrBlobHeader;
+
+typedef struct {
+    uint32_t idc;
+    uint32_t t_tag;
+} BgrJumpEntry;
+#define BGR_JUMP_FWD_CANON 0x40000000u
+#define BGR_JUMP_MAX_T 0x00FFFFFFu
+#define BGR_JUMP_STRIDE 4u
+#define BGR_JUMP_WINDOWS 3u
+#define BGR_JUMP_CAP_BYTES (64ull << 20)
 
 #define BGR_GF_HAS_EXC 1u
 #define BGR_GF_HAS_FALLBACK 2u
+#define BGR_GF_JUMP 4u
 typedef struct {
     const uint32_t* table;
     const BgrKeyEntry* keys;
@@ -152,6 +168,7 @@
 BGR_HD uint32_t bgr_mmx_block(uint32_t mh, uint32_t shift) { return (mh * 0x85EBCA6Bu) >> shift; }
 BGR_HD uint32_t bgr_mmx_word(uint64_t m) { return (uint32_t)(m >> 8) & 15u; }
 BGR_HD uint32_t bgr_mmx_bits(uint64_t m) { return (1u << ((uint32_t)(m >> 12) & 31u)) | (1u << ((uint32_t)(m >> 17) & 31u)); }
+BGR_HD bool bgr_jump_selects(uint64_t m) { return (((uint32_t)(m >> 40)) & (BGR_JUMP_STRIDE - 1u)) == 0; }
 BGR_HD uint32_t bgr_tab_fp(uint64_t m) { const uint32_t f = (uint32_t)(m >> 32) & 0xFFu; return f ? f : 1u; }
 BGR_HD uint32_t bgr_zero_bytes(uint32_t x) { return ~(((x & 0x7F7F7F7Fu) + 0x7F7F7F7Fu) | x) & 0x80808080u; }
 
diff --git a/bgreat_amd/csrc/greedy_kernels.hip b/bgreat_amd/csrc/greedy_kernels.hip
--- a/bgreat_amd/csrc/greedy_kernels.hip
+++ b/bgreat_amd/csrc/greedy_kernels.hip
@@ -176,6 +176,7 @@
     const unsigned long long wt0 = wall_clock64();
     unsigned long long wt2 = 0;
     uint32_t dbg_steps = 0, dbg_items = 0, dbg_groups = 0;
+    uint32_t dbg_jumped = 0, dbg_raised = 0;
 #endif
     uint32_t ktab_words;
     const uint32_t* ktab = block_prologue<STAGE>(g, lds, &ktab_words);
@@ -273,10 +274,110 @@
 
         uint32_t a_pos = 0, a_rec = BGR_NONE;
         if constexpr (STAGE) {
-            const uint32_t g_from = st & G4_ST_POS_MASK;
+            uint32_t g_from = st & G4_ST_POS_MASK;
             uint32_t g_npos = L >= K1 ? L - K1 + 1 : 0;
             if (!prm.effort && g_npos > 1) g_npos = 1;
-            u64 pend = __ballot(act != 0 && sub == 0 && g_from < g_npos);
+            uint32_t to_scan = (act != 0 && g_from < g_npos) ? 1u : 0u;
+#ifdef BGR_PHASE_TIMING
+            if ((g.flags & BGR_GF_JUMP) && prm.debug_stop != 1) {
+#else
+            if (g.flags & BGR_GF_JUMP) {
+#endif
+                const BgrBlobHeader* jh = g.hdr;
+                asm volatile("" : "+s"(jh));
+                const uint4* jtab = reinterpret_cast<const uint4*>(reinterpret_cast<const char*>(jh) + jh->off_jump);
+                const BgrUnitigMeta* jmeta = reinterpret_cast<const BgrUnitigMeta*>(reinterpret_cast<const char*>(jh) + jh->off_meta);
+                const uint32_t jnb = (uint32_t)jh->jump_buckets;
+                uint32_t my_rel = 255u, my_bk = 0;
+#pragma unroll 1
+                for (uint32_t rel = sub; rel < GL * BGR_JUMP_WINDOWS; rel += GL) {
+                    if (to_scan && my_rel == 255u && g_from + rel < g_npos) {
+                        const u64 num = lds_win32(F, g_from + rel) >> (64 - 2 * K1);
+                        const u64 rcn = rcb_fast(num, K1);
+                        const u64 mx = bgr_mix64(num < rcn ? num : rcn);
+                        if (bgr_jump_selects(mx) && num != rcn) {
+                            my_rel = rel | (bgr_tab_fp(mx) << 8) | (num < rcn ? 0x80000000u : 0u);
+                            my_bk = __umulhi((uint32_t)mx, jnb);
+                        }
+                    }
+                }
+                uint32_t w_sub = my_rel & 255u;
+                { const uint32_t o = quad_xor1(w_sub); w_sub = o < w_sub ? o : w_sub; }
+                { const uint32_t o = quad_xor2(w_sub); w_sub = o < w_sub ? o : w_sub; }
+                uint32_t w_idc = 0, w_tt = 0;
+                if ((my_rel & 255u) == w_sub && w_sub != 255u) {
+                    const uint4 b = jtab[my_bk];
+                    const uint32_t tag = (my_rel >> 8) & 0xFFu;
+                    if ((b.y & 0xFFu) == tag) { w_idc = b.x; w_tt = b.y; }
+                    else if ((b.w & 0xFFu) == tag) { w_idc = b.z; w_tt = b.w; }
+                    if (w_tt) w_idc = (w_idc & 0x7FFFFFFFu) | (my_rel & 0x80000000u);
+                    else w_idc = 0;
+                }
+                w_tt |= quad_xor1(w_tt); w_tt |= quad_xor2(w_tt);
+                w_idc |= quad_xor1(w_idc); w_idc |= quad_xor2(w_idc);
+                uint32_t live = 0, ulen = 0, rcs = 0, u0 = 0, rb = 0, re = 0, mfl = 0, hi_p = 0;
+                uint32_t sw = 0, ss = 0;
+                if (w_tt) {
+                    const BgrUnitigMeta* mp = jmeta + (w_idc & BGR_SLOT_ID_MASK);
+                    const uint4 m0 = *reinterpret_cast<const uint4*>(mp);
+                    const u64 Fm = mp->F;
+                    ulen = m0.x; mfl = m0.y; rb = m0.z; re = m0.w;
+                    const uint32_t t = w_tt >> 8;
+                    rcs = ((w_idc >> 31) ^ (w_idc >> 30)) & 1u;
+                    if (t + K1 <= ulen) {
+                        const uint32_t u = rcs ? ulen - K1 - t : t;
+                        if (u >= w_sub) {
+                            u0 = u - w_sub;
+                            const u64 sbase = Fm + (rcs ? ulen : 0u) + u0;
+                            sw = (uint32_t)(sbase >> 5);
+                            ss = 2u * ((uint32_t)sbase & 31u);
+                            const uint32_t room = ulen - u0;
+                            hi_p = L - g_from < room ? L : g_from + room;
+                            live = 1;
+                        }
+                    }
+                }
+                uint32_t e = hi_p;
+                const uint32_t fs = 2u * (g_from & 31u);
+                for (uint32_t c0 = 0; __any(live != 0 && g_from + 64u * c0 < hi_p); c0 += GL) {
+                    const uint32_t rp = g_from + 64u * (c0 + sub);
+                    if (live && rp < hi_p) {
+                        const bool two = rp + 32u < hi_p;
+                        const u64* fp = F + (rp >> 5);
+                        const u64* sp = g.seq + sw + 2u * (c0 + sub);
+                        const u64 f0 = fp[0], f1 = fp[1], f2 = two ? fp[2] : 0;
+                        const u64 s0 = sp[0], s1 = sp[1], s2 = two ? sp[2] : 0;
+                        const u64 xa = ((f0 << fs) | ((f1 >> 1) >> (63 - fs))) ^ ((s0 << ss) | ((s1 >> 1) >> (63 - ss)));
+                        const u64 xb = two ? ((f1 << fs) | ((f2 >> 1) >> (63 - fs))) ^ ((s1 << ss) | ((s2 >> 1) >> (63 - ss))) : 0;
+                        const uint32_t q = xa ? rp + ((uint32_t)__builtin_clzll(xa) >> 1) : xb ? rp + 32u + ((uint32_t)__builtin_clzll(xb) >> 1) : e;
+                        e = q < e ? q : e;
+                    }
+                }
+                { const uint32_t o = quad_xor1(e); e = o < e ? o : e; }
+                { const uint32_t o = quad_xor2(e); e = o < e ? o : e; }
+                const int32_t last = (int32_t)e - (int32_t)K1;
+                uint32_t jumped = 0, raised = 0;
+                if (live && last >= (int32_t)g_from) {
+                    const uint32_t p1 = g_from + (ulen - K1 - u0);
+                    uint32_t found = 0, at_end = 0;
+                    if (u0 == 0) found = 1;
+                    else if ((int32_t)p1 <= last && p1 < g_npos) { found = 1; at_end = 1; }
+                    if (found) {
+                        a_pos = at_end ? p1 : g_from;
+                        const uint32_t cbit = at_end ? (rcs ? BGR_META_CANON_RCBEG : BGR_META_CANON_END) : (rcs ? BGR_META_CANON_RCEND : BGR_META_CANON_BEG);
+                        a_rec = ((at_end ^ rcs) ? re : rb) | ((mfl & cbit) ? G4_CANON : 0u);
+                        to_scan = 0;
+                        jumped = 1;
+                    } else if (last >= (int32_t)g_npos - 1) { to_scan = 0; jumped = 1; }
+                    else { g_from = (uint32_t)last + 1; raised = 1; }
+                }
+#ifdef BGR_PHASE_TIMING
+                dbg_jumped += (uint32_t)__popcll(__ballot(jumped != 0 && sub == 0));
+                dbg_raised += (uint32_t)__popcll(__ballot(raised != 0 && sub == 0));
+#endif
+                (void)jumped; (void)raised;
+            }
+            u64 pend = __ballot(to_scan != 0 && sub == 0);
 #ifdef BGR_PHASE_TIMING
             if (prm.debug_stop == 1) pend = 0;
             dbg_items += (uint32_t)__popcll(pend);
@@ -489,7 +590,7 @@
         unsigned long long* w = io.wave_times + 4ull * (blockIdx.x * waves + wave);
         w[0] = wt0; w[1] = wt1; w[2] = wt2; w[3] = wall_clock64();
         unsigned long long* c = io.wave_times + 4ull * (gridDim.x * waves) + 4ull * (blockIdx.x * waves + wave);
-        c[0] = dbg_steps; c[1] = dbg_items; c[2] = dbg_groups; c[3] = 0;
+        c[0] = dbg_steps; c[1] = dbg_items; c[2] = dbg_groups; c[3] = (unsigned long long)dbg_jumped | ((unsigned long long)dbg_raised << 32);
     }
 #endif
     __syncthreads();
diff --git a/bgreat_amd/csrc/options.h b/bgreat_amd/csrc/options.h
--- a/bgreat_amd/csrc/options.h
+++ b/bgreat_amd/csrc/options.h
@@ -27,6 +27,8 @@
         {"huge_pinned", {1}, 0, 1, "bgr_host_alloc: buffers of 2 MB and more from huge-page mappings registered with the runtime"},
         {"exh_filter", {1}, 0, 1, "exhaustive mode probes large key tables through the minimizer filter"},
         {"build_filter", {-1}, -1, 2, "index build: filter in front of the key table: -1 by table size, 0 none, 1 one hash, 2 minimizer-blocked (forced onto small graphs by tests)"},
+        {"build_jump", {1}, 0, 1, "index build: the jump index of the greedy anchor scan (graph_layout.h) where a graph qualifies: 1 = build it, 0 = none"},
+        {"test.jump_drop", {0}, 0, INT64_MAX, "test hook: index build: every N-th sampled (k-1)-mer is left out of the jump index (the index is a hint: results must not change)"},
         {"poison_device_buffers", {0}, 0, 1, "diagnostic: every new device buffer is filled with a pattern (a kernel that reads what nothing wrote shows in any run)"},
         {"test.bases_cap", {0}, 0, INT64_MAX, "test hook: bases per batch of bgr_align_all (walks the cut of large batches with small inputs)"},
         {"test.lanes_on_one_device", {0}, 0, 1, "test hook: every lane of a split run / every device of --gpus N is device 0 (a one-GPU box walks the N-device code)"},
diff --git a/include/bgreat_gpu.h b/include/bgreat_gpu.h
--- a/include/bgreat_gpu.h
+++ b/include/bgreat_gpu.h
@@ -42,7 +42,17 @@
     uint64_t total_bases, blob_bytes, mphf_bytes, max_unitig_len;
     uint32_t has_exceptions, has_anchors;
     double gamma;
+    uint64_t jump_entries, jump_bytes;
+    uint32_t jump_stride;
+    uint32_t jump_absent;
+    uint32_t jump_dropped_x1000, jump_reserved;
 } bgr_graph_info_t;
+#define BGR_JUMP_PRESENT 0u
+#define BGR_JUMP_WIDE_KEYS 1u
+#define BGR_JUMP_EXCEPTIONS 2u
+#define BGR_JUMP_NOT_STAGED 3u
+#define BGR_JUMP_OVER_CAP 4u
+#define BGR_JUMP_NOT_COMPACTED 5u
 
 const char* bgr_last_error(void);
 
@@ -64,6 +74,7 @@
 const void* bgr_graph_blob(const bgr_graph* g, uint64_t* bytes);
 int bgr_graph_from_blob(const void* blob, uint64_t bytes, bgr_graph** out);
 int bgr_graph_info(const bgr_graph* g, bgr_graph_info_t* out);
+const void* bgr_graph_jump_index(const bgr_graph* g, uint64_t* bytes);
 int bgr_graph_unitigs(const bgr_graph* g, const char** seqs, const uint64_t** offsets, uint64_t* n);
 void bgr_graph_destroy(bgr_graph* g);
 
@@ -199,6 +210,7 @@
 #define BGR_KNOB_KERNEL_EVENTS 11u
 #define BGR_KNOB_ABUNDANCE_FORM 12u
 #define BGR_KNOB_LINKS_FORM 13u
+#define BGR_KNOB_GREEDY_JUMP 15u
 #define BGR_KNOB_GREEDY_FAST 5u
 #define BGR_KNOB_DEVICE_OVERLAP 14u
 int bgr_aligner_set_knob(bgr_aligner* a, uint32_t knob, uint64_t value);
```
